# eriklindernoren/PyTorch-GAN

Measured on NVIDIA H100. Metric: DCGAN 64x64 images/sec (full G+D step), higher is better.
Workload: dtype tf32 (fp32 storage, fp32 accumulate)

## Files before the change

### include/b200gan.h

```cpp
#ifndef B200GAN_H
#define B200GAN_H

#include <stddef.h>
#include <stdint.h>

#ifdef __cplusplus
extern "C" {
#endif

#define B200GAN_VERSION 100

enum {
  B200GAN_OK = 0,
  B200GAN_E_UNSUPPORTED = -1,
  B200GAN_E_BAD_ARG = -2,
  B200GAN_E_CUDA = -3,
  B200GAN_E_ARCH = -4
};

enum { B200GAN_ACT_NONE = 0, B200GAN_ACT_LRELU = 1, B200GAN_ACT_RELU = 2, B200GAN_ACT_TANH = 3,
       B200GAN_ACT_SIGMOID = 4 };

enum { B200GAN_ALGO_AUTO = 0,
       B200GAN_ALGO_SIMT = 1,
       B200GAN_ALGO_TC = 2 };

enum { B200GAN_PAD_ZERO = 0, B200GAN_PAD_REFLECT = 1 };

enum {
  B200GAN_PACK_SIMT_FPROP = 0,
  B200GAN_PACK_SIMT_DGRAD = 1,
  B200GAN_PACK_TC_FPROP = 2,
  B200GAN_PACK_TC_DGRAD = 3,
  B200GAN_PACK_TC_FPROP_UP2 = 4,
  B200GAN_PACK_TC_DGRAD_UP2 = 5
};

typedef struct b200gan_conv_geom {
  int32_t N, H, W, C;
  int32_t K;
  int32_t R, S;
  int32_t stride;
  int32_t pad_t, pad_l, pad_b, pad_r;
  int32_t pad_mode;
  int32_t up;
  int32_t transposed;
  int32_t P, Q;
} b200gan_conv_geom;

typedef struct b200gan_epilogue {
  const float *bias;
  int32_t act;
  float slope;
  const float *chan_scale;
  double *stats;
  int32_t stats_per_sample;
  int32_t round_tf32;
} b200gan_epilogue;

int b200gan_version(void);
const char *b200gan_last_error(void);
int b200gan_check_device(void);

size_t b200gan_packed_weight_floats(const b200gan_conv_geom *g, int pack);
int b200gan_pack_weights(const b200gan_conv_geom *g, int pack, const float *w, float *packed,
                         void *stream);

typedef struct b200gan_pack_job {
  const float *w;
  float *packed;
  b200gan_conv_geom geom;
  int32_t pack;
} b200gan_pack_job;
int b200gan_pack_weights_multi(const b200gan_pack_job *jobs, int32_t count, void *stream);

int b200gan_conv2d_supported(const b200gan_conv_geom *g, int pass, int algo);

int b200gan_conv2d_fprop(const b200gan_conv_geom *g, const b200gan_epilogue *ep, const float *x,
                         const float *packed, float *y, int algo, void *stream);

size_t b200gan_conv2d_dgrad_workspace_floats(const b200gan_conv_geom *g, int algo);
int b200gan_conv2d_dgrad(const b200gan_conv_geom *g, const float *dy, const float *packed,
                         float *dx, float *workspace, int algo, void *stream);

size_t b200gan_conv2d_wgrad_workspace_floats(const b200gan_conv_geom *g, int algo);
int b200gan_conv2d_wgrad(const b200gan_conv_geom *g, const float *x, const float *dy, float *dw,
                         float *db, float *workspace, int algo, void *stream);

int b200gan_epilogue_bwd(const float *dy, const float *y, const float *chan_scale, int32_t act,
                         float slope, int64_t n, int32_t K, int64_t PQ, int32_t round_tf32,
                         float *dz, void *stream);

int b200gan_bias_grad(const float *dy, const float *y, const float *chan_scale, int32_t act, float slope,
                      int64_t rows, int32_t K, int64_t PQ, float *db, void *stream);

typedef struct b200gan_norm_desc {
  int32_t N, HW, C;
  int32_t per_sample;
  float eps;
  float momentum;
  int32_t act;
  float slope;
  int32_t round_tf32;
} b200gan_norm_desc;

int b200gan_norm_stats(const b200gan_norm_desc *d, const float *x, double *stats, void *stream);
int b200gan_norm_finalize(const b200gan_norm_desc *d, double *stats, const float *gamma,
                          const float *beta, float *mean_rstd, float *scale_shift,
                          float *running_mean, float *running_var, int64_t *num_batches_tracked,
                          void *stream);
int b200gan_norm_apply(const b200gan_norm_desc *d, const float *x, const float *scale_shift,
                       float *y, void *stream);
int b200gan_norm_bwd(const b200gan_norm_desc *d, const float *dy, const float *x, const float *y,
                     const float *mean_rstd, const float *scale_shift, const float *gamma, double *sums, float *dx,
                     float *dgamma_dbeta, void *stream);

typedef struct b200gan_tail_desc {
  int32_t N, H, W, C;
  int32_t K;
  int32_t act_mid;
  float slope;
  int32_t act_out;
} b200gan_tail_desc;
int b200gan_tail_supported(const b200gan_tail_desc *d);
int b200gan_tail_fprop(const b200gan_tail_desc *d, const float *a, const float *scale_shift, const float *w,
                       const float *bias, float *out, void *stream);
size_t b200gan_tail_bwd_workspace_bytes(const b200gan_tail_desc *d);
int b200gan_tail_bwd(const b200gan_tail_desc *d, const float *a, const float *mean_rstd, const float *scale_shift,
                     const float *w, const float *g, void *workspace, float *da, float *dgamma_dbeta, float *dw,
                     float *db, int32_t round_tf32, void *stream);

int b200gan_nchw_to_nhwc(const float *x, float *y, int32_t N, int32_t C, int32_t HW, void *stream);
int b200gan_nhwc_to_nchw(const float *x, float *y, int32_t N, int32_t C, int32_t HW, void *stream);
int b200gan_upsample2x_fwd(const float *x, float *y, int32_t N, int32_t H, int32_t W, int32_t C,
                           void *stream);
int b200gan_upsample2x_bwd(const float *dy, float *dx, int32_t N, int32_t H, int32_t W, int32_t C,
                           void *stream);
int b200gan_pad2d_fwd(const float *x, float *y, int32_t N, int32_t H, int32_t W, int32_t C,
                      int32_t pad_t, int32_t pad_l, int32_t pad_b, int32_t pad_r, int32_t mode,
                      int32_t round_tf32, void *stream);
int b200gan_pad2d_bwd(const float *dy, float *dx, int32_t N, int32_t H, int32_t W, int32_t C,
                      int32_t pad_t, int32_t pad_l, int32_t pad_b, int32_t pad_r, int32_t mode,
                      void *stream);
int b200gan_act_fwd(const float *x, const float *mask, int32_t mask_per_channel, int32_t act,
                    float slope, int64_t n, int32_t C, int64_t HW, float *y, void *stream);

typedef struct b200gan_mlp_critic_desc {
  int32_t N, Din, H1, H2;
  float slope;
} b200gan_mlp_critic_desc;
int b200gan_mlp_critic_fwd(const b200gan_mlp_critic_desc *d, const float *x, const float *W1,
                           const float *b1, const float *W2, const float *b2, const float *W3,
                           const float *b3, float *out, float *m1, float *a1, float *m2, float *a2,
                           void *stream);
size_t b200gan_mlp_critic_bwd_workspace_floats(const b200gan_mlp_critic_desc *d);
int b200gan_mlp_critic_bwd(const b200gan_mlp_critic_desc *d, const float *dout, const float *x,
                           const float *W1, const float *W2, const float *W3, const float *m1,
                           const float *a1, const float *m2, const float *a2, float *dx, float *dW1,
                           float *db1, float *dW2, float *db2, float *dW3, float *db3, float *U1,
                           float *U2, float *workspace, void *stream);
size_t b200gan_mlp_critic_dbwd_workspace_floats(const b200gan_mlp_critic_desc *d);
int b200gan_mlp_critic_dbwd(const b200gan_mlp_critic_desc *d, const float *u, const float *dout,
                            const float *U1, const float *U2, const float *m1, const float *m2,
                            const float *W1, const float *W2, const float *W3, float *dW1, float *dW2,
                            float *dW3, float *ddout, float *workspace, void *stream);
size_t b200gan_critic_step_workspace_floats(const b200gan_mlp_critic_desc *d);
int b200gan_critic_step_mlp(const b200gan_mlp_critic_desc *d, float lambda_gp, const float *real, const float *fake,
                            const float *alpha, const float *W1, const float *b1, const float *W2, const float *b2,
                            const float *W3, const float *b3, float *losses, float *dW1, float *db1, float *dW2,
                            float *db2, float *dW3, float *db3, float *workspace, void *stream);

#define B200GAN_MLP_GEN_MAX_LAYERS 8
#define B200GAN_MLP_GEN_MAX_WIDTH 8192
#define B200GAN_MLP_GEN_MAX_N 8192
typedef struct b200gan_mlp_gen_desc {
  int32_t L, N;
  int32_t width[B200GAN_MLP_GEN_MAX_LAYERS + 1];
  int32_t has_norm[B200GAN_MLP_GEN_MAX_LAYERS];
  float slope, eps, momentum;
  const float *W[B200GAN_MLP_GEN_MAX_LAYERS], *b[B200GAN_MLP_GEN_MAX_LAYERS];
  const float *gamma[B200GAN_MLP_GEN_MAX_LAYERS], *beta[B200GAN_MLP_GEN_MAX_LAYERS];
  float *running_mean[B200GAN_MLP_GEN_MAX_LAYERS], *running_var[B200GAN_MLP_GEN_MAX_LAYERS];
  int64_t *num_batches_tracked[B200GAN_MLP_GEN_MAX_LAYERS];
} b200gan_mlp_gen_desc;
typedef struct b200gan_mlp_gen_grads {
  float *dW[B200GAN_MLP_GEN_MAX_LAYERS], *db[B200GAN_MLP_GEN_MAX_LAYERS];
  float *dgamma[B200GAN_MLP_GEN_MAX_LAYERS], *dbeta[B200GAN_MLP_GEN_MAX_LAYERS];
} b200gan_mlp_gen_grads;
size_t b200gan_mlp_gen_saved_floats(const b200gan_mlp_gen_desc *d);
size_t b200gan_mlp_gen_workspace_floats(const b200gan_mlp_gen_desc *d);
int b200gan_mlp_gen_fwd(const b200gan_mlp_gen_desc *d, const float *z, float *out, float *saved, float *workspace,
                        void *stream);
int b200gan_mlp_gen_bwd(const b200gan_mlp_gen_desc *d, const float *dout, const float *z, const float *out,
                        const float *saved, float *dz, const b200gan_mlp_gen_grads *grads, float *workspace,
                        void *stream);

typedef struct b200gan_nb_bn {
  const double *stats;
// ... 49 lines not shown
```

### pytorch-gan_b200/b200gan/_lib.py

```python
import ctypes
import os

_HERE = os.path.dirname(os.path.abspath(__file__))
LIB_PATH = os.path.join(_HERE, "libb200gan.so")

c_i32, c_i64, c_f32, c_f64 = ctypes.c_int32, ctypes.c_int64, ctypes.c_float, ctypes.c_double
c_vp, c_sz = ctypes.c_void_p, ctypes.c_size_t

ACT_NONE, ACT_LRELU, ACT_RELU, ACT_TANH, ACT_SIGMOID = 0, 1, 2, 3, 4
ALGO_AUTO, ALGO_SIMT, ALGO_TC = 0, 1, 2
PAD_ZERO, PAD_REFLECT = 0, 1
PACK_SIMT_FPROP, PACK_SIMT_DGRAD, PACK_TC_FPROP, PACK_TC_DGRAD, PACK_TC_FPROP_UP2, PACK_TC_DGRAD_UP2 = range(6)


class ConvGeom(ctypes.Structure):
    _fields_ = [(n, c_i32) for n in (
        "N", "H", "W", "C", "K", "R", "S", "stride", "pad_t", "pad_l", "pad_b", "pad_r",
        "pad_mode", "up", "transposed", "P", "Q")]

    def key(self):
        return tuple(getattr(self, n) for n, _ in self._fields_)


class Epilogue(ctypes.Structure):
    _fields_ = [("bias", c_vp), ("act", c_i32), ("slope", c_f32), ("chan_scale", c_vp),
                ("stats", c_vp), ("stats_per_sample", c_i32), ("round_tf32", c_i32)]


class NormDesc(ctypes.Structure):
    _fields_ = [("N", c_i32), ("HW", c_i32), ("C", c_i32), ("per_sample", c_i32), ("eps", c_f32),
                ("momentum", c_f32), ("act", c_i32), ("slope", c_f32), ("round_tf32", c_i32)]


class MlpCriticDesc(ctypes.Structure):
    _fields_ = [("N", c_i32), ("Din", c_i32), ("H1", c_i32), ("H2", c_i32), ("slope", c_f32)]


MLP_GEN_MAX_LAYERS, MLP_GEN_MAX_WIDTH, MLP_GEN_MAX_N = 8, 8192, 8192


class MlpGenDesc(ctypes.Structure):
    _fields_ = [("L", c_i32), ("N", c_i32), ("width", c_i32 * (MLP_GEN_MAX_LAYERS + 1)),
                ("has_norm", c_i32 * MLP_GEN_MAX_LAYERS), ("slope", c_f32), ("eps", c_f32), ("momentum", c_f32)] + [
        (n, c_vp * MLP_GEN_MAX_LAYERS)
        for n in ("W", "b", "gamma", "beta", "running_mean", "running_var", "num_batches_tracked")]


class MlpGenGrads(ctypes.Structure):
    _fields_ = [(n, c_vp * MLP_GEN_MAX_LAYERS) for n in ("dW", "db", "dgamma", "dbeta")]


class PackJob(ctypes.Structure):
    _fields_ = [("w", c_vp), ("packed", c_vp), ("geom", ConvGeom), ("pack", c_i32)]


class NbBn(ctypes.Structure):
    _fields_ = [("stats", c_vp), ("gamma", c_vp), ("beta", c_vp), ("eps", c_f32), ("count", c_f64), ("groups", c_i32),
                ("reserved", c_i32)]


class TailDesc(ctypes.Structure):
    _fields_ = [("N", c_i32), ("H", c_i32), ("W", c_i32), ("C", c_i32), ("K", c_i32), ("act_mid", c_i32),
                ("slope", c_f32), ("act_out", c_i32)]


class AdamTensor(ctypes.Structure):
    _fields_ = [("p", c_vp), ("g", c_vp), ("m", c_vp), ("v", c_vp), ("n", c_i64)]


_P = ctypes.POINTER
SIGNATURES = {
    "b200gan_version": (c_i32, []),
    "b200gan_last_error": (ctypes.c_char_p, []),
    "b200gan_check_device": (c_i32, []),
    "b200gan_packed_weight_floats": (c_sz, [_P(ConvGeom), c_i32]),
    "b200gan_pack_weights": (c_i32, [_P(ConvGeom), c_i32, c_vp, c_vp, c_vp]),
    "b200gan_pack_weights_multi": (c_i32, [_P(PackJob), c_i32, c_vp]),
    "b200gan_conv2d_supported": (c_i32, [_P(ConvGeom), c_i32, c_i32]),
    "b200gan_conv2d_fprop": (c_i32, [_P(ConvGeom), _P(Epilogue), c_vp, c_vp, c_vp, c_i32, c_vp]),
    "b200gan_conv2d_dgrad_workspace_floats": (c_sz, [_P(ConvGeom), c_i32]),
    "b200gan_conv2d_dgrad": (c_i32, [_P(ConvGeom), c_vp, c_vp, c_vp, c_vp, c_i32, c_vp]),
    "b200gan_conv2d_wgrad_workspace_floats": (c_sz, [_P(ConvGeom), c_i32]),
    "b200gan_conv2d_wgrad": (c_i32, [_P(ConvGeom), c_vp, c_vp, c_vp, c_vp, c_vp, c_i32, c_vp]),
    "b200gan_epilogue_bwd": (c_i32, [c_vp, c_vp, c_vp, c_i32, c_f32, c_i64, c_i32, c_i64, c_i32, c_vp, c_vp]),
    "b200gan_bias_grad": (c_i32, [c_vp, c_vp, c_vp, c_i32, c_f32, c_i64, c_i32, c_i64, c_vp, c_vp]),
    "b200gan_norm_stats": (c_i32, [_P(NormDesc), c_vp, c_vp, c_vp]),
    "b200gan_norm_finalize": (c_i32, [_P(NormDesc), c_vp, c_vp, c_vp, c_vp, c_vp, c_vp, c_vp, c_vp, c_vp]),
    "b200gan_norm_apply": (c_i32, [_P(NormDesc), c_vp, c_vp, c_vp, c_vp]),
    "b200gan_norm_bwd": (c_i32, [_P(NormDesc), c_vp, c_vp, c_vp, c_vp, c_vp, c_vp, c_vp, c_vp, c_vp, c_vp]),
    "b200gan_tail_supported": (c_i32, [_P(TailDesc)]),
    "b200gan_tail_fprop": (c_i32, [_P(TailDesc), c_vp, c_vp, c_vp, c_vp, c_vp, c_vp]),
    "b200gan_tail_bwd_workspace_bytes": (c_sz, [_P(TailDesc)]),
    "b200gan_tail_bwd": (c_i32, [_P(TailDesc)] + [c_vp] * 10 + [c_i32, c_vp]),
    "b200gan_nchw_to_nhwc": (c_i32, [c_vp, c_vp, c_i32, c_i32, c_i32, c_vp]),
    "b200gan_nhwc_to_nchw": (c_i32, [c_vp, c_vp, c_i32, c_i32, c_i32, c_vp]),
    "b200gan_upsample2x_fwd": (c_i32, [c_vp, c_vp, c_i32, c_i32, c_i32, c_i32, c_vp]),
    "b200gan_upsample2x_bwd": (c_i32, [c_vp, c_vp, c_i32, c_i32, c_i32, c_i32, c_vp]),
    "b200gan_pad2d_fwd": (c_i32, [c_vp, c_vp] + [c_i32] * 10 + [c_vp]),
    "b200gan_pad2d_bwd": (c_i32, [c_vp, c_vp] + [c_i32] * 9 + [c_vp]),
    "b200gan_act_fwd": (c_i32, [c_vp, c_vp, c_i32, c_i32, c_f32, c_i64, c_i32, c_i64, c_vp, c_vp]),
    "b200gan_mlp_critic_fwd": (c_i32, [_P(MlpCriticDesc)] + [c_vp] * 13),
    "b200gan_mlp_critic_bwd_workspace_floats": (c_sz, [_P(MlpCriticDesc)]),
    "b200gan_mlp_critic_bwd": (c_i32, [_P(MlpCriticDesc)] + [c_vp] * 20),
    "b200gan_mlp_critic_dbwd_workspace_floats": (c_sz, [_P(MlpCriticDesc)]),
    "b200gan_mlp_critic_dbwd": (c_i32, [_P(MlpCriticDesc)] + [c_vp] * 15),
    "b200gan_critic_step_workspace_floats": (c_sz, [_P(MlpCriticDesc)]),
    "b200gan_critic_step_mlp": (c_i32, [_P(MlpCriticDesc), c_f32] + [c_vp] * 18),
    "b200gan_mlp_gen_saved_floats": (c_sz, [_P(MlpGenDesc)]),
    "b200gan_mlp_gen_workspace_floats": (c_sz, [_P(MlpGenDesc)]),
    "b200gan_mlp_gen_fwd": (c_i32, [_P(MlpGenDesc)] + [c_vp] * 5),
    "b200gan_mlp_gen_bwd": (c_i32, [_P(MlpGenDesc)] + [c_vp] * 5 + [_P(MlpGenGrads), c_vp, c_vp]),
    "b200gan_nb_supported": (c_i32, [_P(ConvGeom)]),
    "b200gan_nb_groups_supported": (c_i32, [_P(ConvGeom), c_i32]),
    "b200gan_nb_fprop": (c_i32, [_P(ConvGeom), _P(NbBn), c_vp, c_vp, c_vp, c_f32, c_vp, c_vp, c_vp, c_i32, c_f32, c_vp,
                                 c_vp, c_vp, c_i32, c_vp]),
    "b200gan_nb_dz": (c_i32, [c_i32, c_i64, c_i32, c_vp, c_vp, c_vp, c_i32, c_f32, _P(NbBn), c_vp, c_vp, c_vp, c_vp]),
    "b200gan_nb_wgrad_workspace_floats": (c_sz, [_P(ConvGeom)]),
    "b200gan_nb_wgrad": (c_i32, [_P(ConvGeom), _P(NbBn), c_vp, c_vp, c_vp, c_vp, c_vp]),
    "b200gan_nb_dgrad": (c_i32, [_P(ConvGeom), c_vp, c_vp, _P(NbBn), c_vp, c_vp, c_vp, c_vp]),
    "b200gan_nb_tail_fwd": (c_i32, [c_i32, c_i32, c_i32, _P(NbBn), c_vp, c_vp, c_vp, c_f32, c_vp, c_vp, c_i32, c_vp]),
    "b200gan_nb_tail_bwd": (c_i32, [c_i32, c_i32, c_i32, _P(NbBn), c_vp, c_vp, c_i32, c_vp, c_vp, c_vp]),
    "b200gan_linear1_fwd": (c_i32, [c_vp, c_vp, c_vp, c_vp, c_i32, c_i32, c_i32, c_vp]),
    "b200gan_linear1_bwd": (c_i32, [c_vp] * 7 + [c_i32, c_i32, c_i32, c_vp]),
    "b200gan_bce_fwd": (c_i32, [c_vp, c_vp, c_vp, c_i64, c_vp]),
    "b200gan_bce_bwd": (c_i32, [c_vp, c_vp, c_vp, c_vp, c_i64, c_vp]),
    "b200gan_adam_multi": (c_i32, [_P(AdamTensor), c_i32, c_f64, c_f64, c_f64, c_f64, c_f32, c_vp, c_vp]),
}

_lib = None


def load():
    global _lib
    if _lib is not None:
        return _lib
    if not os.path.exists(LIB_PATH):
        raise RuntimeError(
            f"{LIB_PATH} is missing: run `python pytorch-gan_b200/build.py` (or __graft_entry__.build()). "
            "b200gan has no CPU / cuDNN fallback.")
    lib = ctypes.CDLL(LIB_PATH)
    for name, (res, args) in SIGNATURES.items():
        fn = getattr(lib, name)
        fn.restype = res
        fn.argtypes = args
    _lib = lib
    return lib


CALLS = 0


def check(rc, what=""):
    global CALLS
    CALLS += 1
    if rc != 0:
        msg = load().b200gan_last_error().decode("utf-8", "replace")
        raise RuntimeError(f"libb200gan {what} failed (code {rc}): {msg}")
```

### pytorch-gan_b200/b200gan/functional.py

```python
import weakref
from dataclasses import dataclass
from typing import Optional, Tuple

import torch

from . import ops
from ._lib import ConvGeom
from ._lib import (ACT_LRELU, ACT_NONE, ACT_RELU, ACT_SIGMOID, ACT_TANH, ALGO_SIMT,
                   PACK_SIMT_DGRAD, PACK_SIMT_FPROP, PAD_ZERO)


@dataclass(frozen=True)
class ConvSpec:
    stride: int = 1
    pads: Tuple[int, int, int, int] = (0, 0, 0, 0)
    pad_mode: int = PAD_ZERO
    up: int = 1
    transposed: bool = False
    act: int = ACT_NONE
    slope: float = 0.0
    stats: Optional[bool] = None
    rtf_out: bool = False
    rtf_dz: bool = False

# ... 142 lines not shown
    @staticmethod
    @torch.autograd.function.once_differentiable
    def backward(ctx, u):
        dz, weight = ctx.saved_tensors
        g, u = ctx.g, _as_cl(u)
        ddz = _plain_fprop(g, u, weight.detach()) if ctx.needs_input_grad[0] else None
        dw = _plain_wgrad(g, u, _as_cl(dz.detach()), tuple(weight.shape)) if ctx.needs_input_grad[1] else None
        return ddz, dw, None


class ConvWgradFn(torch.autograd.Function):
    @staticmethod
    def forward(ctx, x, dz, g, wshape):
        ctx.g = g
        ctx.save_for_backward(x, dz)
        return _plain_wgrad(g, _as_cl(x.detach()), _as_cl(dz.detach()), wshape)

    @staticmethod
    @torch.autograd.function.once_differentiable
    def backward(ctx, v):
        x, dz = ctx.saved_tensors
        g, v = ctx.g, v.contiguous()
        dx = _plain_dgrad(g, _as_cl(dz.detach()), v) if ctx.needs_input_grad[0] else None
        ddz = _plain_fprop(g, _as_cl(x.detach()), v) if ctx.needs_input_grad[1] else None
        return dx, ddz, None, None


def _conv_backward_differentiable(ctx, dy):
    x, weight, y, chan_scale = ctx.saved_tensors
    act, slope, g = ctx.spec.act, ctx.spec.slope, ctx.g
    if chan_scale is not None and act in (ACT_TANH, ACT_SIGMOID):
        raise NotImplementedError("b200gan: double backward through Dropout2d fused with tanh / sigmoid")
    dz = dy
    if act == ACT_LRELU:
        dz = dz * torch.where(y > 0, 1.0, slope)
    elif act == ACT_RELU:
        dz = dz * (y > 0).to(dy.dtype)
    elif act == ACT_TANH:
        dz = dz * (1 - y * y)
    elif act == ACT_SIGMOID:
        dz = dz * (y * (1 - y))
    if chan_scale is not None:
        dz = dz * chan_scale.view(chan_scale.shape[0], chan_scale.shape[1], 1, 1)
    dx = ConvDgradFn.apply(dz, weight, g) if ctx.needs_input_grad[0] else None
    dw = ConvWgradFn.apply(x, dz, g, tuple(weight.shape)) if ctx.needs_input_grad[1] else None
    db = dz.sum((0, 2, 3)) if (ctx.has_bias and ctx.needs_input_grad[2]) else None
    return dx, dw, db



class NormFn(torch.autograd.Function):

    @staticmethod
    def forward(ctx, x, gamma, beta, stats, running_mean, running_var, nbt, spec: NormSpec):
        ops._require_cuda(x, "norm input")
        x = _as_cl(x)
        y, mean_rstd, scale_shift = ops.norm_forward(
            x, None if gamma is None else gamma.detach(), None if beta is None else beta.detach(), running_mean,
            running_var, nbt, spec.per_sample, spec.eps, spec.momentum, spec.act, spec.slope, stats, spec.rtf_out,
            return_scale_shift=True)
        ctx.spec = spec
        mask_from_x = spec.act in (ACT_LRELU, ACT_RELU)
        need_y = spec.act != ACT_NONE and not mask_from_x
        ctx.save_for_backward(x, y if need_y else None, mean_rstd, gamma, scale_shift if mask_from_x else None)
        return y

    @staticmethod
    @torch.autograd.function.once_differentiable
    def backward(ctx, dy):
        x, y, mean_rstd, gamma, scale_shift = ctx.saved_tensors
        spec = ctx.spec
        dy = _as_cl(dy)
        need_params = gamma is not None and (ctx.needs_input_grad[1] or ctx.needs_input_grad[2])
        dx, dgb = ops.norm_backward(dy, x, y, mean_rstd, None if gamma is None else gamma.detach(), spec.per_sample,
                                    spec.eps, spec.act, spec.slope, need_params, spec.rtf_dx, scale_shift)
        dgamma = dbeta = None
        if need_params:
            n, c = x.shape[0], x.shape[1]
            groups = dgb.numel() // 2
            dgamma, dbeta = dgb[:groups], dgb[groups:]
            if spec.per_sample:
                dgamma, dbeta = dgamma.view(n, c).sum(0), dbeta.view(n, c).sum(0)
        return dx, dgamma, dbeta, None, None, None, None, None


@dataclass(frozen=True)
class TailSpec:
    eps: float = 1e-5
    momentum: float = 0.0
    act_mid: int = ACT_NONE
    slope: float = 0.0
    act_out: int = ACT_NONE
    rtf_dx: bool = False


class TailFn(torch.autograd.Function):

    @staticmethod
    def forward(ctx, a, stats, gamma, beta, running_mean, running_var, nbt, weight, bias, spec: TailSpec):
        ops._require_cuda(a, "tail input")
        a = _as_cl(a)
        if stats is None:
            stats = ops.norm_stats(a, False)
        mean_rstd, scale_shift = ops.norm_finalize(
            tuple(a.shape), stats, None if gamma is None else gamma.detach(), None if beta is None else beta.detach(),
            running_mean, running_var, nbt, False, spec.eps, spec.momentum, a.device)
        d = ops.tail_desc(tuple(a.shape), weight.shape[0], spec.act_mid, spec.slope, spec.act_out)
        w = weight.detach().contiguous()
        out = ops.tail_fprop(d, a, scale_shift, w, None if bias is None else bias.detach())
        ctx.spec, ctx.d = spec, d
        ctx.has_affine, ctx.has_bias = gamma is not None, bias is not None
        ctx.save_for_backward(a, mean_rstd, scale_shift, weight, out if spec.act_out != ACT_NONE else None)
        return out

    @staticmethod
    @torch.autograd.function.once_differentiable
    def backward(ctx, dout):
        a, mean_rstd, scale_shift, weight, out = ctx.saved_tensors
        spec = ctx.spec
        dout = _as_cl(dout)
        g = ops.epilogue_bwd(dout, out, None, spec.act_out, 0.0) if spec.act_out != ACT_NONE else dout
        need_affine = ctx.has_affine and (ctx.needs_input_grad[2] or ctx.needs_input_grad[3])
        need_bias = ctx.has_bias and ctx.needs_input_grad[8]
        da, dgb, dw, db = ops.tail_bwd(ctx.d, a, mean_rstd, scale_shift, weight.detach().contiguous(), g, need_affine,
                                       need_bias, spec.rtf_dx)
        c = a.shape[1]
        dgamma = dgb[:c] if need_affine else None
        dbeta = dgb[c:] if need_affine else None
        return da, None, dgamma, dbeta, None, None, None, dw, db, None


class AffineActFn(torch.autograd.Function):

    @staticmethod
    def forward(ctx, x, scale_shift, act, slope):
        x = _as_cl(x)
        y = ops.norm_apply_affine(x, scale_shift, False, act, slope)
        ctx.act, ctx.slope = act, slope
        ctx.save_for_backward(y, scale_shift)
        return y

    @staticmethod
    @torch.autograd.function.once_differentiable
    def backward(ctx, dy):
        y, scale_shift = ctx.saved_tensors
        dy = _as_cl(dy)
        dz = ops.epilogue_bwd(dy, y, None, ctx.act, ctx.slope) if ctx.act != ACT_NONE else dy
        c = y.shape[1]
        zero = torch.zeros_like(scale_shift)
        zero[:c] = scale_shift[:c]
        return ops.norm_apply_affine(dz, zero, False), None, None, None


class ToChannelsLastFn(torch.autograd.Function):

    @staticmethod
    def forward(ctx, x):
        return ops.to_cl(x)

    @staticmethod
    def backward(ctx, dy):
        if torch.is_grad_enabled() and dy.requires_grad:
            return ToContiguousFn.apply(dy)
        return ops.to_nchw(dy.detach())


# ... 377 lines not shown
```

### pytorch-gan_b200/b200gan/nn.py

```python
import torch
import torch.nn as tnn

from . import _lib
from . import functional as F
from . import ops
from ._lib import (ACT_LRELU, ACT_NONE, ACT_RELU, ACT_SIGMOID, ACT_TANH, PAD_REFLECT, PAD_ZERO)
from .functional import ConvSpec, NormSpec, PackCache

_T = {
    n: getattr(tnn, n) for n in (
        "Conv2d", "ConvTranspose2d", "BatchNorm2d", "InstanceNorm2d", "LeakyReLU", "ReLU", "Tanh", "Sigmoid",
        "Upsample", "ZeroPad2d", "ReflectionPad2d", "Dropout", "Dropout2d", "Sequential", "Linear", "BCELoss",
        "BatchNorm1d")
}


def _pair_same(v, what):
    if isinstance(v, (tuple, list)):
        if len(v) != 2 or v[0] != v[1]:
            raise NotImplementedError(f"b200gan: {what}={v} (h != w) is not supported")
        return int(v[0])
    return int(v)


def _act_of(m):
    if isinstance(m, _T["LeakyReLU"]):
        if m.negative_slope < 0:
            raise NotImplementedError(f"b200gan: {m} (negative_slope < 0)")
        return ACT_LRELU, float(m.negative_slope)
    if isinstance(m, _T["ReLU"]):
        return ACT_RELU, 0.0
    if isinstance(m, _T["Tanh"]):
        return ACT_TANH, 0.0
    if isinstance(m, _T["Sigmoid"]):
        return ACT_SIGMOID, 0.0
    return None


def _is_up2(m):
    if not isinstance(m, _T["Upsample"]):
        return False
    sf = m.scale_factor
    if isinstance(sf, (tuple, list)):
        sf = sf[0] if len(set(sf)) == 1 else None
    return m.size is None and sf is not None and float(sf) == 2.0 and m.mode == "nearest"


def _pads_of(m):
    p = m.padding
    if isinstance(p, int):
        p = (p, p, p, p)
    l, r, t, b = p
    return (int(t), int(l), int(b), int(r))


def _conv_ok(m):
    if isinstance(m.padding, str) or m.padding_mode != "zeros":
        return False
    if tuple(m.dilation) != (1, 1) or m.groups != 1:
        return False
    if len(set(m.stride)) != 1 or len(set(m.padding)) != 1:
        return False
    if isinstance(m, _T["ConvTranspose2d"]) and tuple(m.output_padding) != (0, 0):
        return False
    return True


def _tc_like(conv, up, full=False):
    if ops.Config.algo == "simt":
        return False
    if up == 2:
        return (not isinstance(conv, _T["ConvTranspose2d"]) and conv.stride[0] == 1 and conv.in_channels % 32 == 0
                and conv.out_channels % 64 == 0)
    if conv.stride[0] in (1, 2) and conv.in_channels % 32 == 0 and conv.out_channels % 32 == 0:
        return True
    return (full is False and not isinstance(conv, _T["ConvTranspose2d"]) and conv.stride[0] == 1
            and conv.in_channels % 32 == 0 and conv.out_channels < 32)


def _no_groups(what):
    if ops.bn_groups.active > 1:
        raise RuntimeError(f"b200gan: ops.bn_groups({ops.bn_groups.active}) is active but {what} would treat the batch "
                           "as one pass; run the passes separately")


def _dropout2d_scale(x_shape, p, device):
    n, c = x_shape[0], x_shape[1]
    noise = torch.empty((n, c, 1, 1), device=device, dtype=torch.float32)
    if p >= 1.0:
        return noise.zero_().view(n, c)
    return noise.bernoulli_(1.0 - p).div_(1.0 - p).view(n, c)


def _run_conv(conv, x, up=1, extra_pads=(0, 0, 0, 0), pad_mode=PAD_ZERO, act=ACT_NONE, slope=0.0, chan_scale=None,
              stats=None, rtf_out=False, rtf_dz=False):
    if not _conv_ok(conv):
        raise NotImplementedError(f"b200gan: unsupported convolution configuration: {conv}")
    transposed = isinstance(conv, _T["ConvTranspose2d"])
    pad = int(conv.padding[0])
    if pad_mode == PAD_REFLECT and pad != 0:
        raise NotImplementedError("b200gan: reflection padding in front of a zero-padded conv")
    if pad_mode == PAD_REFLECT and up == 1 and _tc_like(conv, 1):
        x = F.PadFn.apply(x, tuple(extra_pads), PAD_REFLECT, True)
        extra_pads, pad_mode = (0, 0, 0, 0), PAD_ZERO
    pads = tuple(e + pad for e in extra_pads)
    spec = ConvSpec(stride=int(conv.stride[0]), pads=pads, pad_mode=pad_mode, up=up, transposed=transposed, act=act,
                    slope=slope, stats=stats, rtf_out=rtf_out, rtf_dz=rtf_dz)
    cache = conv.__dict__.get("_b200_cache")
    if cache is None:
        cache = PackCache()
        conv.__dict__["_b200_cache"] = cache
    return F.conv_block(x, conv.weight, conv.bias, chan_scale, spec, cache)


def _run_norm(norm, x, act=ACT_NONE, slope=0.0, stats=None, rtf_out=False, rtf_dx=False):
    per_sample = isinstance(norm, _T["InstanceNorm2d"])
    if per_sample and norm.track_running_stats:
        raise NotImplementedError("b200gan: InstanceNorm2d(track_running_stats=True)")
    if x.dim() != 4:
        raise ValueError(f"expected 4D input (got {x.dim()}D input)")
    if per_sample and x.shape[2] * x.shape[3] == 1 and norm.training:
        raise ValueError(f"Expected more than 1 spatial element when training, got input size {tuple(x.shape)}")
    use_batch_stats = per_sample or norm.training or norm.running_mean is None
    if use_batch_stats and not per_sample:
        _no_groups("a stand-alone BatchNorm2d")
    if use_batch_stats:
        rm = rv = nbt = None
        momentum = 0.0
        if not per_sample and norm.training and norm.track_running_stats:
            if norm.momentum is None:
                raise NotImplementedError("b200gan: BatchNorm2d(momentum=None)")
            rm, rv, nbt, momentum = norm.running_mean, norm.running_var, norm.num_batches_tracked, float(norm.momentum)
        spec = NormSpec(per_sample=per_sample, eps=float(norm.eps), momentum=momentum, act=act, slope=slope,
                        rtf_out=rtf_out, rtf_dx=rtf_dx)
        return F.norm_block(x, norm.weight, norm.bias, stats, rm, rv, nbt, spec)
    rstd = torch.rsqrt(norm.running_var + norm.eps)
    scale = rstd if norm.weight is None else norm.weight * rstd
    shift = -norm.running_mean * scale if norm.bias is None else norm.bias - norm.running_mean * scale
    return F.AffineActFn.apply(x, torch.cat([scale, shift]).detach(), act, slope)


def _on_device(x):
    return x.is_cuda


def _gpu4d(x):
    return x.dim() == 4 and _on_device(x)


class Conv2d(_T["Conv2d"]):
    def forward(self, x):
        return _run_conv(self, x)


class ConvTranspose2d(_T["ConvTranspose2d"]):
    def forward(self, x, output_size=None):
        if output_size is not None:
            raise NotImplementedError("b200gan: ConvTranspose2d(output_size=...)")
        return _run_conv(self, x)


class BatchNorm2d(_T["BatchNorm2d"]):
    def forward(self, x):
        return _run_norm(self, x)


class InstanceNorm2d(_T["InstanceNorm2d"]):
    def forward(self, x):
        return _run_norm(self, x)


class _Act:
    def forward(self, x):
        if not _gpu4d(x):
            return super().forward(x)
        act, slope = _act_of(self)
        return F.ActFn.apply(x, act, slope, None, False)


class LeakyReLU(_Act, _T["LeakyReLU"]):
    pass


class ReLU(_Act, _T["ReLU"]):
    pass


class Tanh(_Act, _T["Tanh"]):
    pass


class Sigmoid(_Act, _T["Sigmoid"]):
    pass


class Upsample(_T["Upsample"]):
    def forward(self, x):
        if _gpu4d(x) and _is_up2(self):
            return F.UpsampleFn.apply(x)
        if _gpu4d(x):
            raise NotImplementedError(f"b200gan: {self} (only nearest x2 is on the hot path)")
        return super().forward(x)


class ZeroPad2d(_T["ZeroPad2d"]):
    def forward(self, x):
        if not _gpu4d(x):
            return super().forward(x)
        return F.PadFn.apply(x, _pads_of(self), PAD_ZERO)


class ReflectionPad2d(_T["ReflectionPad2d"]):
    def forward(self, x):
        if not _gpu4d(x):
            return super().forward(x)
        return F.PadFn.apply(x, _pads_of(self), PAD_REFLECT)


class Dropout2d(_T["Dropout2d"]):
    def forward(self, x):
        if not _gpu4d(x):
            return super().forward(x)
        if not self.training or self.p == 0.0:
            return x
        _no_groups("a stand-alone Dropout2d")
        return F.ActFn.apply(x, ACT_NONE, 0.0, _dropout2d_scale(x.shape, self.p, x.device), True)


class Dropout(_T["Dropout"]):
    def forward(self, x):
        if not _gpu4d(x):
            return super().forward(x)
        if not self.training or self.p == 0.0:
            return x
        _no_groups("a stand-alone Dropout")
        xc = x if ops.is_cl(x) else ops.to_cl(x)
        mask = torch.empty_like(xc, memory_format=torch.channels_last)
        if self.p >= 1.0:
            mask.zero_()
        else:
            mask.bernoulli_(1.0 - self.p).div_(1.0 - self.p)
        return F.ActFn.apply(xc, ACT_NONE, 0.0, mask, False)


def _gpu2d_f32(x):
    return torch.is_tensor(x) and x.dim() == 2 and x.is_cuda and x.dtype == torch.float32


class Linear(_T["Linear"]):

    def forward(self, x):
        if _gpu2d_f32(x) and self.out_features >= 8192 and ops.Config.algo != "simt":
            return F.LinearWideFn.apply(x, self.weight, self.bias)
        return super().forward(x)


class BatchNorm1d(_T["BatchNorm1d"]):
    """nn.BatchNorm1d, same state_dict.  Inside the MLP generator pattern of a Sequential (mlp_generator_layers,
    wgan_gp.py:42-65, gan.py:38-61) it runs in the fused generator kernels; anywhere else, and on the CPU, it is the stock
    module."""


class BCELoss(_T["BCELoss"]):
    def forward(self, input, target):
        if (input.is_cuda and input.dtype == torch.float32 and self.reduction == "mean" and self.weight is None
                and target.shape == input.shape and target.dtype == torch.float32 and not target.requires_grad):
            return F.BCEMeanFn.apply(input, target)
        return super().forward(input, target)


class _ConvStep:
    def __init__(self, conv, up, extra_pads, pad_mode, act, slope, dropout2d, stats):
        self.conv, self.up, self.extra_pads, self.pad_mode = conv, up, extra_pads, pad_mode
        self.act, self.slope, self.dropout2d, self.stats = act, slope, dropout2d, stats
        self.rtf_out = False
        self.rtf_dz = False
        self.next_norm = None

    def tc_like(self, full=False):
        if self.pad_mode == PAD_REFLECT and self.up != 1:
            return False
        return _tc_like(self.conv, self.up, full)


class _NormStep:
    def __init__(self, norm, act, slope, takes_stats):
        self.norm, self.act, self.slope, self.takes_stats = norm, act, slope, takes_stats
        self.rtf_out = False
        self.rtf_dx = False


class _LeafStep:
    def __init__(self, mod):
        self.mod = mod


class _TailStep:

    def __init__(self, norm_step, conv_step):
        self.norm_step, self.conv_step = norm_step, conv_step


def _chain_plan(chain, shape):
    plan = []
    for cs, ns in chain.layers:
        conv = cs.conv
        if shape[1] != conv.in_channels or not _conv_ok(conv):
            return None
        g, oshape = ops.make_geom(shape, tuple(conv.weight.shape), int(conv.stride[0]), (int(conv.padding[0]),) * 4)
        macs = float(oshape[0]) * oshape[2] * oshape[3] * conv.out_channels * conv.in_channels * g.R * g.S
        if macs > _ChainStep.MAX_MACS or not ops.nb_supported(g) or oshape[2] * oshape[3] < 1:
            return None
        if ns is not None:
            norm = ns.norm
            if not (norm.training and norm.num_features == conv.out_channels):
                return None
            if norm.track_running_stats and norm.momentum is None:
                return None
        plan.append((cs, ns, oshape))
        shape = oshape
    return plan


def groups_eligible(seq, x_shape, groups):
    if not isinstance(seq, Sequential) or not ops.Config.fuse_narrow_chain or x_shape[0] % groups != 0:
        return False
    steps = seq._plan()
    if not steps or not all(isinstance(st, _ChainStep) for st in steps):
        return False
    shape = tuple(x_shape)
    with ops.bn_groups(groups):
        for st in steps:
            plan = _chain_plan(st, shape)
            if plan is None:
                return False
            shape = plan[-1][2]
    return True


class _ChainStep:

    MAX_MACS = 6.0e8

    def __init__(self, steps):
        self.steps = steps
        self.layers = []
        i = 0
        while i < len(steps):
            ns = steps[i + 1] if i + 1 < len(steps) and isinstance(steps[i + 1], _NormStep) else None
            self.layers.append((steps[i], ns))
            i += 2 if ns is not None else 1


def _chain_conv_candidate(cs):
    if not isinstance(cs, _ConvStep):
        return False
    conv = cs.conv
    if isinstance(conv, _T["ConvTranspose2d"]) or cs.up != 1 or cs.extra_pads != (0, 0, 0, 0) or cs.pad_mode != PAD_ZERO:
        return False
    if cs.act not in (ACT_NONE, ACT_LRELU, ACT_RELU):
        return False
    k, c = conv.out_channels, conv.in_channels
    if not (4 <= k <= 128 and (k & (k - 1)) == 0 and 1 <= c <= 128 and (c == 1 or c % 4 == 0)):
        return False
    return tuple(conv.kernel_size) in ((3, 3), (4, 4)) and conv.stride[0] in (1, 2)


def _chain_norm_candidate(ns):
    return isinstance(ns, _NormStep) and isinstance(ns.norm, _T["BatchNorm2d"]) and ns.act == ACT_NONE


def _fuse_chains(steps):
    out, i, n = [], 0, len(steps)
    while i < n:
        j, convs = i, 0
        while j < n and _chain_conv_candidate(steps[j]):
            convs += 1
            j += 1
            if j < n and steps[j - 1].stats is False and _chain_norm_candidate(steps[j]):
                j += 1
            elif steps[j - 1].stats is not None:
                j -= 1
                convs -= 1
# ... 208 lines not shown
                norm = ns.norm
                edge = ops.BnEdge(stats, None if norm.weight is None else norm.weight.detach(),
                                  None if norm.bias is None else norm.bias.detach(), norm.eps,
                                  oshape[0] // groups * oshape[2] * oshape[3], groups)
                out_box.append(edge)
                prev_norm = norm
            else:
                x, edge, prev_norm = res, None, None
        if edge is not None:
            norm = prev_norm
            rm = rv = nbt = None
            momentum = 0.0
            if norm.track_running_stats and norm.running_mean is not None:
                rm, rv, nbt, momentum = norm.running_mean, norm.running_var, norm.num_batches_tracked, float(norm.momentum)
            x = F.NbTailFn.apply(x, norm.weight, norm.bias, rm, rv, nbt, edge, momentum, bool(nchw_out))
        return x

    def _forward_2d(self, x):
        mods = list(self._modules.values())
        critic = mlp_critic_layers(mods, x.shape[1])
        if critic is not None and x.shape[0] >= 1:
            return F.mlp_critic(x, *critic)
        gen = mlp_generator_layers(mods, x.shape[1])
        if gen is not None and (x.shape[0] >= 2 or all(bn is None for _, bn in gen[0])) \
                and x.shape[0] <= _lib.MLP_GEN_MAX_N:
            return F.mlp_generator(x, *gen)
        i = 0
        while i < len(mods):
            m = mods[i]
            if (isinstance(m, _T["Linear"]) and m.out_features == 1 and _gpu2d_f32(x) and x.shape[0] <= 4096
                    and i + 1 < len(mods) and _act_of(mods[i + 1]) is not None
                    and _act_of(mods[i + 1])[0] in (ACT_SIGMOID, ACT_TANH)):
                x = F.Linear1Fn.apply(x, m.weight, m.bias, _act_of(mods[i + 1])[0])
                i += 2
            else:
                x = m(x)
                i += 1
        return x

    def forward(self, x):
        if _gpu2d_f32(x):
            return self._forward_2d(x)
        if not (torch.is_tensor(x) and x.dim() == 4 and _on_device(x) and x.dtype == torch.float32):
            return super().forward(x)
        steps = self._plan()
        if all(isinstance(s, _LeafStep) for s in steps):
            return _T["Sequential"].forward(self, x)
        want_contiguous = x.is_contiguous()
        stats = None
        queue = list(steps)
        while queue:
            s = queue.pop(0)
            if isinstance(s, _ChainStep):
                at_end = not queue
                res = self._run_chain(s, x, want_contiguous and at_end)
                if res is None:
                    _no_groups("a conv chain that does not qualify for the fused kernels")
                    queue[0:0] = s.steps
                else:
                    x, stats = res, None
                    if at_end and want_contiguous and x.is_contiguous():
                        return x
                continue
            if isinstance(s, _TailStep):
                ns, cs = s.norm_step, s.conv_step
                norm, conv = ns.norm, cs.conv
                _no_groups("the fused generator tail")
                if (norm.training and x.shape[1] == conv.in_channels and x.shape[1] == norm.num_features
                        and ops.tail_supported(tuple(x.shape), conv.out_channels, ns.act, ns.slope, cs.act)):
                    rm = rv = nbt = None
                    momentum = 0.0
                    if norm.track_running_stats and norm.running_mean is not None:
                        if norm.momentum is None:
                            raise NotImplementedError("b200gan: BatchNorm2d(momentum=None)")
                        rm, rv, nbt, momentum = norm.running_mean, norm.running_var, norm.num_batches_tracked, float(norm.momentum)
                    spec = F.TailSpec(eps=float(norm.eps), momentum=momentum, act_mid=ns.act, slope=ns.slope,
                                      act_out=cs.act, rtf_dx=ns.rtf_dx)
                    x = F.TailFn.apply(x, stats if ns.takes_stats else None, norm.weight, norm.bias, rm, rv, nbt,
                                       conv.weight, conv.bias, spec)
                    stats = None
                else:
                    queue[0:0] = [ns, cs]
                continue
            if isinstance(s, _ConvStep):
                cs = None
                if s.dropout2d is not None and s.dropout2d.training and s.dropout2d.p > 0.0:
                    _no_groups("a Dropout2d outside a fused chain")
                    n = x.shape[0]
                    cs = _dropout2d_scale((n, s.conv.out_channels), s.dropout2d.p, x.device)
                want = s.stats if (s.next_norm is not None and _uses_batch_stats(s.next_norm)) else None
                out = _run_conv(s.conv, x, s.up, s.extra_pads, s.pad_mode, s.act, s.slope, cs, want, s.rtf_out,
                                s.rtf_dz)
                if want is not None:
                    x, stats = out
                else:
                    x, stats = out, None
            elif isinstance(s, _NormStep):
                x = _run_norm(s.norm, x, s.act, s.slope, stats if s.takes_stats else None, s.rtf_out, s.rtf_dx)
                stats = None
            else:
                x = s.mod(x)
                stats = None
        if (want_contiguous and torch.is_tensor(x) and x.dim() == 4 and not x.is_contiguous()
                and x.shape[2] * x.shape[3] <= ops.Config.contiguous_hw_limit):
            x = F.ToContiguousFn.apply(x)
        return x


REPLACEMENTS = {
    "Conv2d": Conv2d, "ConvTranspose2d": ConvTranspose2d, "BatchNorm2d": BatchNorm2d,
    "InstanceNorm2d": InstanceNorm2d, "LeakyReLU": LeakyReLU, "ReLU": ReLU, "Tanh": Tanh, "Sigmoid": Sigmoid,
    "Upsample": Upsample, "ZeroPad2d": ZeroPad2d, "ReflectionPad2d": ReflectionPad2d, "Dropout": Dropout,
    "Dropout2d": Dropout2d, "Sequential": Sequential, "Linear": Linear, "BCELoss": BCELoss, "BatchNorm1d": BatchNorm1d,
}
for _n, _c in REPLACEMENTS.items():
    _c.__name__ = _n
    _c.__qualname__ = _n
```

### pytorch-gan_b200/b200gan/ops.py

```python
import ctypes
import os

import torch

from . import _lib
from ._lib import (ACT_NONE, ALGO_AUTO, ALGO_SIMT, ALGO_TC, PACK_SIMT_DGRAD, PACK_SIMT_FPROP, PACK_TC_DGRAD,
                   PACK_TC_DGRAD_UP2, PACK_TC_FPROP, PACK_TC_FPROP_UP2, PAD_REFLECT, PAD_ZERO, ConvGeom, Epilogue,
                   MlpCriticDesc, MlpGenDesc, MlpGenGrads, NbBn, NormDesc, TailDesc)

CL = torch.channels_last


class Config:
    algo = os.environ.get("B200GAN_ALGO", "auto")
    weight_cache = True
    contiguous_hw_limit = 64
    fuse_narrow_chain = os.environ.get("B200GAN_FUSE_CHAIN", "1") not in ("", "0")


def _stream():
    return torch.cuda.current_stream().cuda_stream


def _ptr(t):
# ... 53 lines not shown
    g = ConvGeom()
    g.N, g.H, g.W, g.C = n, h, w, c
    if transposed:
        cin, cout, r, s = weight_shape
    else:
        cout, cin, r, s = weight_shape
    if cin != c:
        raise RuntimeError(f"b200gan conv: input has {c} channels, weight expects {cin}")
    g.K, g.R, g.S, g.stride = cout, r, s, stride
    g.pad_t, g.pad_l, g.pad_b, g.pad_r = pads
    g.pad_mode, g.up, g.transposed = pad_mode, up, int(transposed)
    if transposed:
        g.P = (h - 1) * stride - 2 * pads[0] + r
        g.Q = (w - 1) * stride - 2 * pads[1] + s
    else:
        g.P = (h * up + pads[0] + pads[2] - r) // stride + 1
        g.Q = (w * up + pads[1] + pads[3] - s) // stride + 1
    return g, (n, cout, g.P, g.Q)


def tc_supported(g, pas):
    if Config.algo == "simt":
        return False
    return bool(_lib.load().b200gan_conv2d_supported(ctypes.byref(g), pas, ALGO_TC))


def conv_plan(g, pas, chan_scale=None):
    if pas == 2:
        return (ALGO_SIMT if Config.algo == "simt" else ALGO_AUTO), None
    tc = tc_supported(g, pas) and not (pas == 0 and g.K < 32 and chan_scale is not None)
    if not tc:
        return ALGO_SIMT, (PACK_SIMT_FPROP if pas == 0 else PACK_SIMT_DGRAD)
    if pas == 0:
        return ALGO_TC, (PACK_TC_FPROP_UP2 if g.up == 2 else PACK_TC_FPROP)
    return ALGO_TC, (PACK_TC_DGRAD_UP2 if g.up == 2 else PACK_TC_DGRAD)


def pack_weights(g, w, kind, out=None):
    lib = _lib.load()
    if out is None:
        n = lib.b200gan_packed_weight_floats(ctypes.byref(g), kind)
        out = torch.empty(n, device=w.device, dtype=torch.float32)
    _lib.check(lib.b200gan_pack_weights(ctypes.byref(g), kind, w.data_ptr(), out.data_ptr(), _stream()), "pack_weights")
    return out


def pack_weights_multi(jobs):
    table = (_lib.PackJob * len(jobs))()
    for i, (g, kind, w, packed) in enumerate(jobs):
        table[i].w, table[i].packed, table[i].geom, table[i].pack = w.data_ptr(), packed.data_ptr(), g, kind
    _lib.check(_lib.load().b200gan_pack_weights_multi(table, len(jobs), _stream()), "pack_weights_multi")


def conv_fprop(g, x, packed, algo, bias=None, act=ACT_NONE, slope=0.0, chan_scale=None, stats=None,
               stats_per_sample=False, round_tf32=False):
    y = empty_cl(g.N, g.K, g.P, g.Q, x.device)
    if g.N == 0:
        return y
    ep = Epilogue()
    ep.bias, ep.act, ep.slope = _ptr(bias), act, slope
    ep.chan_scale, ep.stats = _ptr(chan_scale), _ptr(stats)
    ep.stats_per_sample, ep.round_tf32 = int(stats_per_sample), int(round_tf32)
    _lib.check(_lib.load().b200gan_conv2d_fprop(ctypes.byref(g), ctypes.byref(ep), x.data_ptr(), packed.data_ptr(),
                                                y.data_ptr(), algo, _stream()), "conv2d_fprop")
    return y


def conv_dgrad(g, dy, packed, algo):
    lib = _lib.load()
    dx = empty_cl(g.N, g.C, g.H, g.W, dy.device)
    nws = lib.b200gan_conv2d_dgrad_workspace_floats(ctypes.byref(g), algo)
    ws = torch.empty(nws, device=dy.device, dtype=torch.float32) if nws else None
    _lib.check(lib.b200gan_conv2d_dgrad(ctypes.byref(g), dy.data_ptr(), packed.data_ptr(), dx.data_ptr(), _ptr(ws),
                                        algo, _stream()), "conv2d_dgrad")
    return dx


def conv_wgrad(g, x, dy, weight_shape, need_bias, algo):
    lib = _lib.load()
    dw = torch.empty(weight_shape, device=x.device, dtype=torch.float32)
    db = torch.empty(g.K, device=x.device, dtype=torch.float32) if need_bias else None
    nws = lib.b200gan_conv2d_wgrad_workspace_floats(ctypes.byref(g), algo)
    ws = torch.empty(nws, device=x.device, dtype=torch.float32) if nws else None
    _lib.check(lib.b200gan_conv2d_wgrad(ctypes.byref(g), x.data_ptr(), dy.data_ptr(), dw.data_ptr(), _ptr(db),
                                        _ptr(ws), algo, _stream()), "conv2d_wgrad")
    return dw, db


def epilogue_bwd(dy, y, chan_scale, act, slope, round_tf32=False):
    n, k, p, q = dy.shape
    dz = torch.empty_like(dy, memory_format=CL)
    _lib.check(_lib.load().b200gan_epilogue_bwd(dy.data_ptr(), _ptr(y), _ptr(chan_scale), act, slope, dy.numel(), k,
                                                p * q, int(round_tf32), dz.data_ptr(), _stream()), "epilogue_bwd")
    return dz


def bias_grad(dy, y, chan_scale, act, slope):
    n, k, p, q = dy.shape
    db = torch.empty(k, device=dy.device, dtype=torch.float32)
    _lib.check(_lib.load().b200gan_bias_grad(dy.data_ptr(), _ptr(y), _ptr(chan_scale), act, slope, n * p * q, k, p * q,
                                             db.data_ptr(), _stream()), "bias_grad")
    return db


def _norm_desc(shape, per_sample, eps, momentum, act, slope, round_tf32):
    n, c, h, w = shape
    d = NormDesc()
    d.N, d.HW, d.C, d.per_sample = n, h * w, c, int(per_sample)
    d.eps, d.momentum, d.act, d.slope, d.round_tf32 = eps, momentum, act, slope, int(round_tf32)
    return d


_zero_scratch = {}


def zero_scratch(device, numel):
    key = (device, numel)
    t = _zero_scratch.get(key)
    if t is None:
        t = torch.zeros(numel, device=device, dtype=torch.float64)
        _zero_scratch[key] = t
    return t


def reset_scratch():
    for t in _zero_scratch.values():
        t.zero_()


def new_stats(x, per_sample):
    n, c = x.shape[0], x.shape[1]
    return zero_scratch(x.device, 2 * (n * c if per_sample else c))


def norm_forward(x, gamma, beta, running_mean, running_var, nbt, per_sample, eps, momentum, act=ACT_NONE, slope=0.0,
                 stats=None, round_tf32=False, return_scale_shift=False):
    if stats is None:
        stats = norm_stats(x, per_sample)
    mean_rstd, scale_shift = norm_finalize(x.shape, stats, gamma, beta, running_mean, running_var, nbt, per_sample, eps,
                                           momentum, x.device)
    d = _norm_desc(x.shape, per_sample, eps, momentum, act, slope, round_tf32)
    y = torch.empty_like(x, memory_format=CL)
    _lib.check(_lib.load().b200gan_norm_apply(ctypes.byref(d), x.data_ptr(), scale_shift.data_ptr(), y.data_ptr(),
                                              _stream()), "norm_apply")
    if return_scale_shift:
        return y, mean_rstd, scale_shift
    return y, mean_rstd


def norm_finalize(x_shape, stats, gamma, beta, running_mean, running_var, nbt, per_sample, eps, momentum, device):
    d = _norm_desc(x_shape, per_sample, eps, momentum, ACT_NONE, 0.0, False)
    groups = stats.numel() // 2
    mean_rstd = torch.empty(2 * groups, device=device, dtype=torch.float32)
    scale_shift = torch.empty(2 * groups, device=device, dtype=torch.float32)
    _lib.check(_lib.load().b200gan_norm_finalize(ctypes.byref(d), stats.data_ptr(), _ptr(gamma), _ptr(beta),
                                                 mean_rstd.data_ptr(), scale_shift.data_ptr(), _ptr(running_mean),
                                                 _ptr(running_var), _ptr(nbt), _stream()), "norm_finalize")
    return mean_rstd, scale_shift


def norm_stats(x, per_sample):
    d = _norm_desc(x.shape, per_sample, 0.0, 0.0, ACT_NONE, 0.0, False)
    stats = new_stats(x, per_sample)
    _lib.check(_lib.load().b200gan_norm_stats(ctypes.byref(d), x.data_ptr(), stats.data_ptr(), _stream()), "norm_stats")
    return stats


def tail_desc(a_shape, k, act_mid, slope, act_out):
    n, c, h, w = a_shape
    d = TailDesc()
    d.N, d.H, d.W, d.C, d.K = n, h, w, c, k
    d.act_mid, d.slope, d.act_out = act_mid, slope, act_out
    return d


def tail_supported(a_shape, k, act_mid, slope, act_out):
    if Config.algo == "simt":
        return False
    return bool(_lib.load().b200gan_tail_supported(ctypes.byref(tail_desc(a_shape, k, act_mid, slope, act_out))))


def tail_fprop(d, a, scale_shift, w, bias):
    out = empty_cl(d.N, d.K, d.H, d.W, a.device)
    _lib.check(_lib.load().b200gan_tail_fprop(ctypes.byref(d), a.data_ptr(), scale_shift.data_ptr(), w.data_ptr(),
                                              _ptr(bias), out.data_ptr(), _stream()), "tail_fprop")
    return out


def tail_bwd(d, a, mean_rstd, scale_shift, w, g, need_affine, need_bias, round_tf32):
    lib = _lib.load()
    nws = lib.b200gan_tail_bwd_workspace_bytes(ctypes.byref(d))
    ws = torch.empty((nws + 7) // 8, device=a.device, dtype=torch.float64)
    da = torch.empty_like(a, memory_format=CL)
    dgb = torch.empty(2 * d.C, device=a.device, dtype=torch.float32) if need_affine else None
    dw = torch.empty((d.K, d.C, 3, 3), device=a.device, dtype=torch.float32)
    db = torch.empty(d.K, device=a.device, dtype=torch.float32) if need_bias else None
    _lib.check(lib.b200gan_tail_bwd(ctypes.byref(d), a.data_ptr(), mean_rstd.data_ptr(), scale_shift.data_ptr(),
                                    w.data_ptr(), g.data_ptr(), ws.data_ptr(), da.data_ptr(), _ptr(dgb), dw.data_ptr(),
                                    _ptr(db), int(round_tf32), _stream()), "tail_bwd")
    return da, dgb, dw, db


def norm_apply_affine(x, scale_shift, per_sample, act=ACT_NONE, slope=0.0):
    d = _norm_desc(x.shape, per_sample, 0.0, 0.0, act, slope, False)
    y = torch.empty_like(x, memory_format=CL)
    _lib.check(_lib.load().b200gan_norm_apply(ctypes.byref(d), x.data_ptr(), scale_shift.data_ptr(), y.data_ptr(),
                                              _stream()), "norm_apply")
    return y


def norm_backward(dy, x, y, mean_rstd, gamma, per_sample, eps, act=ACT_NONE, slope=0.0, need_params=False,
                  round_tf32=False, scale_shift=None):
    lib = _lib.load()
    d = _norm_desc(x.shape, per_sample, eps, 0.0, act, slope, round_tf32)
    groups = mean_rstd.numel() // 2
    sums = zero_scratch(x.device, 2 * groups)
    dx = torch.empty_like(x, memory_format=CL)
    dgb = torch.empty(2 * groups, device=x.device, dtype=torch.float32) if need_params else None
    _lib.check(lib.b200gan_norm_bwd(ctypes.byref(d), dy.data_ptr(), x.data_ptr(), _ptr(y), mean_rstd.data_ptr(),
                                    _ptr(scale_shift), _ptr(gamma), sums.data_ptr(), dx.data_ptr(), _ptr(dgb), _stream()),
               "norm_bwd")
    return dx, dgb


def upsample2x(x):
    n, c, h, w = x.shape
    y = empty_cl(n, c, 2 * h, 2 * w, x.device)
    _lib.check(_lib.load().b200gan_upsample2x_fwd(x.data_ptr(), y.data_ptr(), n, h, w, c, _stream()), "upsample2x_fwd")
    return y


def upsample2x_bwd(dy):
    n, c, h2, w2 = dy.shape
    dx = empty_cl(n, c, h2 // 2, w2 // 2, dy.device)
    _lib.check(_lib.load().b200gan_upsample2x_bwd(dy.data_ptr(), dx.data_ptr(), n, h2 // 2, w2 // 2, c, _stream()),
               "upsample2x_bwd")
    return dx


def pad2d(x, pads, mode, round_tf32=False):
    n, c, h, w = x.shape
    t, l, b, r = pads
    y = empty_cl(n, c, h + t + b, w + l + r, x.device)
    _lib.check(_lib.load().b200gan_pad2d_fwd(x.data_ptr(), y.data_ptr(), n, h, w, c, t, l, b, r, mode, int(round_tf32),
                                             _stream()), "pad2d_fwd")
    return y


def pad2d_bwd(dy, pads, mode):
    n, c, ho, wo = dy.shape
    t, l, b, r = pads
    h, w = ho - t - b, wo - l - r
    dx = empty_cl(n, c, h, w, dy.device)
    _lib.check(_lib.load().b200gan_pad2d_bwd(dy.data_ptr(), dx.data_ptr(), n, h, w, c, t, l, b, r, mode, _stream()),
               "pad2d_bwd")
    return dx


def act_forward(x, act, slope, mask=None, mask_per_channel=False):
    n, c, h, w = x.shape
    y = torch.empty_like(x, memory_format=CL)
    _lib.check(_lib.load().b200gan_act_fwd(x.data_ptr(), _ptr(mask), int(mask_per_channel), act, slope, x.numel(), c,
                                           h * w, y.data_ptr(), _stream()), "act_fwd")
    return y


class BnEdge:

    def __init__(self, stats, gamma, beta, eps, count, groups=1):
        self.stats, self.gamma, self.beta, self.eps, self.count = stats, gamma, beta, float(eps), float(count)
        self.groups = int(groups)
        self.sums = None

    def c_struct(self):
        b = NbBn()
        b.stats, b.gamma, b.beta = self.stats.data_ptr(), _ptr(self.gamma), _ptr(self.beta)
        b.eps, b.count, b.groups, b.reserved = self.eps, self.count, self.groups, 0
        return b


class bn_groups:

    active = 1

    def __init__(self, groups):
        self.groups = int(groups)

    def __enter__(self):
        self.prev = bn_groups.active
        bn_groups.active = self.groups
        return self

    def __exit__(self, *exc):
        bn_groups.active = self.prev


def nb_supported(g):
    if not Config.fuse_narrow_chain:
        return False
    lib = _lib.load()
    if bn_groups.active > 1:
        return bool(lib.b200gan_nb_groups_supported(ctypes.byref(g), bn_groups.active))
    return bool(lib.b200gan_nb_supported(ctypes.byref(g)))

# ... 243 lines not shown
```

### pytorch-gan_b200/csrc/conv_api.cu

```cuda
#include "common.cuh"
#include <atomic>
#include <mutex>
#include <string.h>
#include <stdlib.h>

namespace b200gan {

int simt_gather_gemm(int N, int H, int W, int C, int P, int Q, int K, int R, int S, int stride,
                     int pad_t, int pad_l, int pad_mode, int up, int mode,
                     const b200gan_epilogue *ep, const float *x, const float *wp, float *y,
                     cudaStream_t st);
int simt_wgrad(int N, int H, int W, int Cg, int P, int Q, int Cd, int R, int S, int stride,
               int pad_t, int pad_l, int pad_mode, int up, const float *xg, const float *dn,
               float *dw, cudaStream_t st);
int simt_colsum(const float *x, float *out, int64_t M, int C, cudaStream_t st);
bool nb_wgrad_ok(const b200gan_conv_geom *g);
int nb_wgrad_run(const b200gan_conv_geom *g, const b200gan_nb_bn *in_bn, const float *x, const float *dz, float *dw,
                 float *workspace, cudaStream_t st);
size_t nb_wgrad_workspace_floats(const b200gan_conv_geom *g);
bool nb_plain_fprop_ok(const b200gan_conv_geom *g);
int nb_plain_fprop(const b200gan_conv_geom *g, const b200gan_epilogue *ep, const float *x, const float *packed, float *y,
                   cudaStream_t st);
bool nb_plain_dgrad_ok(const b200gan_conv_geom *g);
int nb_plain_dgrad(const b200gan_conv_geom *g, const float *dy, const float *packed, float *dx, cudaStream_t st);
bool fewk_ok(const b200gan_conv_geom *g, int pas);
int fewk_fprop(const b200gan_conv_geom *g, const b200gan_epilogue *ep, const float *x, const float *packed, float *y,
               cudaStream_t st);
int fewk_dgrad(const b200gan_conv_geom *g, const float *dy, const float *packed, float *dx, cudaStream_t st);
int fewk_wgrad(const b200gan_conv_geom *g, const float *x, const float *dy, float *dw, float *workspace, cudaStream_t st);
size_t fewk_wgrad_workspace_floats(const b200gan_conv_geom *g);
int tc_supported(const b200gan_conv_geom *g, int pass);
int tc_fprop(const b200gan_conv_geom *g, const b200gan_epilogue *ep, const float *x,
             const float *packed, float *y, cudaStream_t st);
int tc_dgrad(const b200gan_conv_geom *g, const float *dy, const float *packed, float *dx,
             cudaStream_t st);
size_t tc_wgrad_workspace_floats(const b200gan_conv_geom *g);
int tc_wgrad(const b200gan_conv_geom *g, const float *x, const float *dy, float *dw, float *ws,
             cudaStream_t st);

static thread_local char g_err[512] = "";
void set_error(const char *fmt, ...) {
  va_list ap;
  va_start(ap, fmt);
  vsnprintf(g_err, sizeof(g_err), fmt, ap);
  va_end(ap);
}

int conv_stats_pass(const float *y, int N, int HW, int C, int per_sample, double *stats, cudaStream_t st) {
  b200gan_norm_desc nd;
  memset(&nd, 0, sizeof(nd));
  nd.N = N; nd.HW = HW; nd.C = C; nd.per_sample = per_sample;
  return b200gan_norm_stats(&nd, y, stats, st);
}

int num_sms() {
  static std::atomic<int> cache[64];
  int dev = 0;
  if (cudaGetDevice(&dev) != cudaSuccess || dev < 0 || dev >= 64) {
    cudaGetLastError();
    return 132;
  }
  int v = cache[dev].load(std::memory_order_relaxed);
  if (v > 0) return v;
  if (cudaDeviceGetAttribute(&v, cudaDevAttrMultiProcessorCount, dev) != cudaSuccess || v <= 0) {
    cudaGetLastError();
    return 132;
  }
  cache[dev].store(v, std::memory_order_relaxed);
  return v;
}

int validate_geom(const b200gan_conv_geom *g) {
  B2_CHECK_ARG(g != nullptr, "conv: null geometry");
  B2_CHECK_ARG(g->N >= 0 && g->H > 0 && g->W > 0 && g->C > 0 && g->K > 0 && g->R > 0 && g->S > 0,
               "conv: bad dims N=%d H=%d W=%d C=%d K=%d R=%d S=%d", g->N, g->H, g->W, g->C, g->K,
               g->R, g->S);
  B2_CHECK_ARG(g->stride >= 1, "conv: stride must be >= 1");
  B2_CHECK_ARG(g->up == 1 || g->up == 2, "conv: up must be 1 or 2");
  B2_CHECK_ARG(g->pad_t >= 0 && g->pad_l >= 0 && g->pad_b >= 0 && g->pad_r >= 0, "conv: negative padding");
  int P, Q;
  if (g->transposed) {
    B2_CHECK_ARG(g->up == 1 && g->pad_mode == B200GAN_PAD_ZERO,
                 "conv: ConvTranspose2d cannot fold upsample / reflection padding");
    B2_CHECK_ARG(g->pad_t == g->pad_b && g->pad_l == g->pad_r, "conv: ConvTranspose2d padding must be symmetric");
    P = (g->H - 1) * g->stride - 2 * g->pad_t + g->R;
    Q = (g->W - 1) * g->stride - 2 * g->pad_l + g->S;
  } else {
    int Hv = g->H * g->up, Wv = g->W * g->up;
    if (g->pad_mode == B200GAN_PAD_REFLECT)
      B2_CHECK_ARG(g->pad_t < Hv && g->pad_b < Hv && g->pad_l < Wv && g->pad_r < Wv,
                   "conv: reflection padding must be smaller than the input");
    int Hp = Hv + g->pad_t + g->pad_b, Wp = Wv + g->pad_l + g->pad_r;
    B2_CHECK_ARG(Hp >= g->R && Wp >= g->S, "conv: filter larger than padded input");
    P = (Hp - g->R) / g->stride + 1;
    Q = (Wp - g->S) / g->stride + 1;
  }
  B2_CHECK_ARG(P == g->P && Q == g->Q, "conv: output size mismatch: expected %dx%d, got %dx%d", P, Q,
               g->P, g->Q);
  B2_CHECK_ARG((int64_t)g->N * g->H * g->W * g->C < (1LL << 40) && (int64_t)g->N * P * Q * g->K < (1LL << 40),
               "conv: tensor too large");
  return B200GAN_OK;
}

__device__ __forceinline__ void up2_rset(int a, int d, int &lo, int &hi) {
  if (a == 0) { lo = d == 0 ? 0 : 1; hi = d == 0 ? 0 : 2; }
  else        { lo = d == 0 ? 0 : 2; hi = d == 0 ? 1 : 2; }
}

constexpr int PACK_MAX_JOBS = 24;
constexpr int PACK_CHUNK = 256 * 8;
struct PackJob {
  const float *src;
  float *dst;
  int R, S, Cin, Cout, transposed, kind;
  int tiles_ci;
  long long total;
};
constexpr int PACK_CO_T = 32, PACK_CI_T = 8, PACK_RS_MAX = 16;
struct PackTable {
  PackJob job[PACK_MAX_JOBS];
// ... 175 lines not shown
  return base;
}

extern "C" int b200gan_pack_weights(const b200gan_conv_geom *g, int pack, const float *w, float *packed,
                                    void *stream) {
  PackTable tb;
  tb.count = 0;
  tb.block_begin[0] = 0;
  if (int e = pack_table_add(tb, g, pack, w, packed)) return e;
  return pack_table_launch(tb, as_stream(stream));
}

extern "C" int b200gan_conv2d_supported(const b200gan_conv_geom *g, int pass, int algo) {
  if (validate_geom(g) != B200GAN_OK) return 0;
  if (algo == B200GAN_ALGO_SIMT) return 1;
  return tc_supported(g, pass);
}

extern "C" int b200gan_conv2d_fprop(const b200gan_conv_geom *g, const b200gan_epilogue *ep, const float *x,
                                    const float *packed, float *y, int algo, void *stream) {
  if (int e = validate_geom(g)) return e;
  B2_CHECK_ARG(x && packed && y, "conv2d_fprop: null pointer");
  B2_CHECK_ARG(algo != B200GAN_ALGO_AUTO, "conv2d_fprop: the packed layout fixes the algorithm; pass SIMT or TC");
  cudaStream_t st = as_stream(stream);
  if (algo == B200GAN_ALGO_TC) {
    if (!tc_supported(g, 0)) B2_UNSUPPORTED("conv2d_fprop: geometry not supported by the tensor-core path");
    return tc_fprop(g, ep, x, packed, y, st);
  }
  int rc;
  if (fewk_ok(g, 0) && !(ep && (ep->chan_scale || ep->round_tf32))) {
    b200gan_epilogue e2;
    if (ep) { e2 = *ep; e2.stats = nullptr; }
    rc = fewk_fprop(g, ep ? &e2 : nullptr, x, packed, y, st);
  } else if (nb_plain_fprop_ok(g)) {
    rc = nb_plain_fprop(g, ep, x, packed, y, st);
  } else {
    rc = simt_gather_gemm(g->N, g->H, g->W, g->C, g->P, g->Q, g->K, g->R, g->S, g->stride, g->pad_t, g->pad_l,
                          g->pad_mode, g->up, g->transposed ? 1 : 0, ep, x, packed, y, st);
  }
  if (rc) return rc;
  if (ep && ep->stats) return conv_stats_pass(y, g->N, g->P * g->Q, g->K, ep->stats_per_sample, ep->stats, st);
  return B200GAN_OK;
}

enum class DgradRoute { Tc, Transposed, Fewk, Staged, Virtual };

static DgradRoute dgrad_route(const b200gan_conv_geom *g, int algo) {
  if (algo == B200GAN_ALGO_AUTO ? tc_supported(g, 1) : algo == B200GAN_ALGO_TC) return DgradRoute::Tc;
  if (g->transposed) return DgradRoute::Transposed;
  if (fewk_ok(g, 1)) return DgradRoute::Fewk;
  if (nb_plain_dgrad_ok(g)) return DgradRoute::Staged;
  return DgradRoute::Virtual;
}

enum class WgradRoute { Tc, Fewk, Staged, Simt };

static WgradRoute wgrad_route(const b200gan_conv_geom *g, int algo) {
  if (algo == B200GAN_ALGO_AUTO ? tc_supported(g, 2) : algo == B200GAN_ALGO_TC) return WgradRoute::Tc;
  if (fewk_ok(g, 2)) return WgradRoute::Fewk;
  if (nb_wgrad_ok(g) && (int64_t)g->N * g->P * g->Q * g->K * g->C * g->R * g->S <= (int64_t)2e10)
    return WgradRoute::Staged;
  return WgradRoute::Simt;
}

extern "C" size_t b200gan_conv2d_dgrad_workspace_floats(const b200gan_conv_geom *g, int algo) {
  if (!g || dgrad_route(g, algo) != DgradRoute::Virtual) return 0;
  size_t n = 0;
  int Hv = g->H * g->up, Wv = g->W * g->up;
  if (g->pad_mode == B200GAN_PAD_REFLECT)
    n += (size_t)g->N * (Hv + g->pad_t + g->pad_b) * (Wv + g->pad_l + g->pad_r) * g->C;
  if (g->up == 2) n += (size_t)g->N * Hv * Wv * g->C;
  return n;
}

extern "C" int b200gan_conv2d_dgrad(const b200gan_conv_geom *g, const float *dy, const float *packed, float *dx,
                                    float *workspace, int algo, void *stream) {
  if (int e = validate_geom(g)) return e;
  B2_CHECK_ARG(dy && packed && dx, "conv2d_dgrad: null pointer");
  B2_CHECK_ARG(algo != B200GAN_ALGO_AUTO, "conv2d_dgrad: pass SIMT or TC explicitly");
  cudaStream_t st = as_stream(stream);
  switch (dgrad_route(g, algo)) {
    case DgradRoute::Tc:
      if (!tc_supported(g, 1)) B2_UNSUPPORTED("conv2d_dgrad: geometry not supported by the tensor-core path");
      return tc_dgrad(g, dy, packed, dx, st);
    case DgradRoute::Transposed:
      return simt_gather_gemm(g->N, g->P, g->Q, g->K, g->H, g->W, g->C, g->R, g->S, g->stride, g->pad_t, g->pad_l,
                              B200GAN_PAD_ZERO, 1, 0, nullptr, dy, packed, dx, st);
    case DgradRoute::Fewk:
      return fewk_dgrad(g, dy, packed, dx, st);
    case DgradRoute::Staged:
      return nb_plain_dgrad(g, dy, packed, dx, st);
    case DgradRoute::Virtual:
      break;
  }
  int Hv = g->H * g->up, Wv = g->W * g->up;
  bool reflect = g->pad_mode == B200GAN_PAD_REFLECT;
  B2_CHECK_ARG(!(reflect || g->up == 2) || workspace, "conv2d_dgrad: workspace required for reflect / upsample");
  float *ws_pad = nullptr, *ws_up = nullptr;
  if (reflect) {
    ws_pad = workspace;
    workspace += (size_t)g->N * (Hv + g->pad_t + g->pad_b) * (Wv + g->pad_l + g->pad_r) * g->C;
  }
  if (g->up == 2) ws_up = workspace;
  float *dvirt = reflect ? ws_pad : (g->up == 2 ? ws_up : dx);
  int oh = reflect ? Hv + g->pad_t + g->pad_b : Hv;
  int ow = reflect ? Wv + g->pad_l + g->pad_r : Wv;
  int rc;
  b200gan_conv_geom gv = *g;
  gv.H = oh; gv.W = ow; gv.up = 1; gv.pad_mode = B200GAN_PAD_ZERO;
  if (reflect) gv.pad_t = gv.pad_l = gv.pad_b = gv.pad_r = 0;
  if (reflect && g->up == 1 && fewk_ok(&gv, 1)) {
    rc = fewk_dgrad(&gv, dy, packed, dvirt, st);
  } else if (reflect && g->up == 1 && nb_plain_dgrad_ok(&gv)) {
    rc = nb_plain_dgrad(&gv, dy, packed, dvirt, st);
  } else {
    rc = simt_gather_gemm(g->N, g->P, g->Q, g->K, oh, ow, g->C, g->R, g->S, g->stride, reflect ? 0 : g->pad_t,
                          reflect ? 0 : g->pad_l, B200GAN_PAD_ZERO, 1, 1, nullptr, dy, packed, dvirt, st);
  }
  if (rc) return rc;
  if (reflect) {
    float *dst = g->up == 2 ? ws_up : dx;
    rc = b200gan_pad2d_bwd(ws_pad, dst, g->N, Hv, Wv, g->C, g->pad_t, g->pad_l, g->pad_b, g->pad_r,
                           B200GAN_PAD_REFLECT, stream);
    if (rc) return rc;
  }
  if (g->up == 2) return b200gan_upsample2x_bwd(ws_up, dx, g->N, g->H, g->W, g->C, stream);
  return B200GAN_OK;
}

extern "C" size_t b200gan_conv2d_wgrad_workspace_floats(const b200gan_conv_geom *g, int algo) {
  if (!g) return 0;
  switch (wgrad_route(g, algo)) {
    case WgradRoute::Tc: return tc_wgrad_workspace_floats(g);
    case WgradRoute::Fewk: return fewk_wgrad_workspace_floats(g);
    case WgradRoute::Staged: return nb_wgrad_workspace_floats(g);
    case WgradRoute::Simt: break;
  }
  return 0;
}

extern "C" int b200gan_conv2d_wgrad(const b200gan_conv_geom *g, const float *x, const float *dy, float *dw,
                                    float *db, float *workspace, int algo, void *stream) {
  if (int e = validate_geom(g)) return e;
  B2_CHECK_ARG(x && dy && dw, "conv2d_wgrad: null pointer");
  cudaStream_t st = as_stream(stream);
  int rc = B200GAN_OK;
  switch (wgrad_route(g, algo)) {
    case WgradRoute::Tc:
      if (!tc_supported(g, 2)) B2_UNSUPPORTED("conv2d_wgrad: geometry not supported by the tensor-core path");
      rc = tc_wgrad(g, x, dy, dw, workspace, st);
      break;
    case WgradRoute::Fewk:
      rc = fewk_wgrad(g, x, dy, dw, workspace, st);
      break;
    case WgradRoute::Staged:
      rc = nb_wgrad_run(g, nullptr, x, dy, dw, workspace, st);
      break;
    case WgradRoute::Simt:
      if (g->transposed)
        rc = simt_wgrad(g->N, g->P, g->Q, g->K, g->H, g->W, g->C, g->R, g->S, g->stride, g->pad_t, g->pad_l,
                        B200GAN_PAD_ZERO, 1, dy, x, dw, st);
      else
        rc = simt_wgrad(g->N, g->H, g->W, g->C, g->P, g->Q, g->K, g->R, g->S, g->stride, g->pad_t, g->pad_l,
                        g->pad_mode, g->up, x, dy, dw, st);
      break;
  }
  if (rc) return rc;
  if (db) return simt_colsum(dy, db, (int64_t)g->N * g->P * g->Q, g->K, st);
  return B200GAN_OK;
}
```

### pytorch-gan_b200/csrc/conv_tc.cu

```cuda
#include "tc_common.cuh"
#include <mutex>
#include <stdlib.h>

namespace b200gan {

PFN_encodeTiled get_encode_tiled() {
  static PFN_encodeTiled fn = nullptr;
  static std::once_flag once;
  std::call_once(once, [] {
    void *p = nullptr;
    cudaDriverEntryPointQueryResult q;
    if (cudaGetDriverEntryPointByVersion("cuTensorMapEncodeTiled", &p, 12000, cudaEnableDefault, &q) == cudaSuccess &&
        q == cudaDriverEntryPointSuccess)
      fn = reinterpret_cast<PFN_encodeTiled>(p);
  });
  return fn;
}

int make_tmap_f32(CUtensorMap *map, const void *base, int rank, const uint64_t *dims, const uint64_t *strides_bytes,
                  const uint32_t *box) {
  PFN_encodeTiled enc = get_encode_tiled();
  if (!enc) {
    set_error("cuTensorMapEncodeTiled entry point not available");
    return B200GAN_E_CUDA;
  }
  cuuint64_t gd[5], gs[4];
  cuuint32_t bx[5], es[5];
  for (int i = 0; i < rank; ++i) {
    gd[i] = dims[i];
    bx[i] = box[i];
    es[i] = 1;
  }
  for (int i = 0; i < rank - 1; ++i) gs[i] = strides_bytes[i];
  CUresult r = enc(map, CU_TENSOR_MAP_DATA_TYPE_FLOAT32, (cuuint32_t)rank, const_cast<void *>(base), gd, gs, bx, es,
                   CU_TENSOR_MAP_INTERLEAVE_NONE, CU_TENSOR_MAP_SWIZZLE_128B,
                   CU_TENSOR_MAP_L2_PROMOTION_L2_256B,
                   CU_TENSOR_MAP_FLOAT_OOB_FILL_NONE);
  if (r != CUDA_SUCCESS) {
    set_error("cuTensorMapEncodeTiled failed (%d): rank %d dims [%llu %llu %llu %llu %llu] box [%u %u %u %u %u]", (int)r,
              rank, (unsigned long long)gd[0], (unsigned long long)(rank > 1 ? gd[1] : 0),
              (unsigned long long)(rank > 2 ? gd[2] : 0), (unsigned long long)(rank > 3 ? gd[3] : 0),
              (unsigned long long)(rank > 4 ? gd[4] : 0), bx[0], rank > 1 ? bx[1] : 0, rank > 2 ? bx[2] : 0,
              rank > 3 ? bx[3] : 0, rank > 4 ? bx[4] : 0);
    return B200GAN_E_CUDA;
  }
  return B200GAN_OK;
}

constexpr int TC_BM = 128;
constexpr int TC_BK = 32;
constexpr int TC_A_BYTES = TC_BM * TC_BK * 4;
constexpr int TC_MAX_TAPS = 52;
constexpr int TC_THREADS = 384;

struct TcTap {
  int16_t dc;
  int8_t dw, da, dh;
  int8_t bt;
  int8_t pad_[2];
};

struct TcParams {
  int32_t tap_begin[5];
  TcTap taps[TC_MAX_TAPS];
  int32_t kout_total;
  int32_t kchunks;
  int32_t bw_log2, bh_log2;
  int32_t tiles_w, tiles_h;
  int32_t N, Ho, Wo;
  int32_t out_dc[4], out_da[4];
  int32_t ldk;
  const float *bias;
  const float *chan_scale;
  double *stats;
  int32_t stats_groups;
  int32_t stats_per_sample;
  int32_t act;
  float slope;
  int32_t rtf;
  float *y;
  int32_t narrow_k;
  int32_t ksplit;
  long long *trace;
};

#define TC_TRACE(slot)                                                   \
  do {                                                                   \
    if (p.trace) p.trace[((size_t)blockIdx.z * gridDim.x + blockIdx.x) * 64 + (slot)] = clock64(); \
  } while (0)

template <int OFF>
__device__ __forceinline__ void colsum_step(float (&v)[32], int lane) {
  const bool upper = (lane & OFF) != 0;
#pragma unroll
  for (int i = 0; i < OFF; ++i) {
    float send = upper ? v[i] : v[i + OFF];
    float keep = upper ? v[i + OFF] : v[i];
    v[i] = keep + __shfl_xor_sync(0xffffffffu, send, OFF);
  }
}
__device__ __forceinline__ float warp_colsum32(float (&v)[32], int lane) {
  colsum_step<16>(v, lane);
  colsum_step<8>(v, lane);
  colsum_step<4>(v, lane);
  colsum_step<2>(v, lane);
  colsum_step<1>(v, lane);
  return v[0];
}

__device__ __forceinline__ void consumers_sync() { asm volatile("bar.sync 1, 256;" ::: "memory"); }

__device__ __forceinline__ void ld_row32(const uint8_t *chunk, int m, float (&v)[32]) {
  const uint8_t *row = chunk + m * 128;
#pragma unroll
  for (int j = 0; j < 8; ++j) {
    const float4 t = *reinterpret_cast<const float4 *>(row + ((j ^ (m & 7)) << 4));
    v[4 * j] = t.x; v[4 * j + 1] = t.y; v[4 * j + 2] = t.z; v[4 * j + 3] = t.w;
  }
}
__device__ __forceinline__ void st_row32(uint8_t *chunk, int m, const float (&v)[32]) {
  uint8_t *row = chunk + m * 128;
#pragma unroll
  for (int j = 0; j < 8; ++j)
    *reinterpret_cast<float4 *>(row + ((j ^ (m & 7)) << 4)) = make_float4(v[4 * j], v[4 * j + 1], v[4 * j + 2], v[4 * j + 3]);
}

__device__ __forceinline__ void epilogue_chunk(float (&v)[32], const float *bias, int narrow_k, int act, float slope,
                                               const float *cs, int rtf) {
  if (bias && narrow_k) {
#pragma unroll
    for (int j = 0; j < 32; ++j)
      if (j < narrow_k) v[j] += __ldg(bias + j);
  } else if (bias) {
    const float4 *b4 = reinterpret_cast<const float4 *>(bias);
#pragma unroll
    for (int j = 0; j < 8; ++j) {
      float4 b = __ldg(b4 + j);
      v[4 * j] += b.x; v[4 * j + 1] += b.y; v[4 * j + 2] += b.z; v[4 * j + 3] += b.w;
    }
  }
  if (act == B200GAN_ACT_LRELU) {
#pragma unroll
    for (int j = 0; j < 32; ++j) v[j] = v[j] > 0.f ? v[j] : v[j] * slope;
  } else if (act == B200GAN_ACT_RELU) {
#pragma unroll
    for (int j = 0; j < 32; ++j) v[j] = fmaxf(v[j], 0.f);
  } else if (act == B200GAN_ACT_TANH) {
#pragma unroll
    for (int j = 0; j < 32; ++j) v[j] = tanhf(v[j]);
  } else if (act == B200GAN_ACT_SIGMOID) {
#pragma unroll
    for (int j = 0; j < 32; ++j) v[j] = 1.f / (1.f + __expf(-v[j]));
  }
  if (cs) {
    const float4 *s4 = reinterpret_cast<const float4 *>(cs);
#pragma unroll
    for (int j = 0; j < 8; ++j) {
      float4 b = __ldg(s4 + j);
      v[4 * j] *= b.x; v[4 * j + 1] *= b.y; v[4 * j + 2] *= b.z; v[4 * j + 3] *= b.w;
    }
  }
  if (rtf) {
#pragma unroll
    for (int j = 0; j < 32; ++j) v[j] = round_tf32(v[j]);
  }
}

template <int BN, int STAGES>
struct TcSmem {
  static constexpr int STAGE_BYTES = TC_A_BYTES + BN * TC_BK * 4;
  static constexpr int RING = STAGES * STAGE_BYTES;
  static constexpr int STAGING = (BN / 32) * TC_A_BYTES;
  static constexpr int MAIN = RING > STAGING ? RING : STAGING;
  static constexpr int TOTAL = MAIN + 1024 + 256 + 4 * BN * 2 * 4;
};

template <int BN, int STAGES>
__global__ void __launch_bounds__(TC_THREADS, 1)
conv_tc_kernel(const __grid_constant__ CUtensorMap tmA, const __grid_constant__ CUtensorMap tmB,
               const __grid_constant__ CUtensorMap tmY, const __grid_constant__ TcParams p) {
  using L = TcSmem<BN, STAGES>;
  extern __shared__ uint8_t smem_raw[];
  uint8_t *smem = reinterpret_cast<uint8_t *>((reinterpret_cast<uintptr_t>(smem_raw) + 1023) & ~(uintptr_t)1023);
  uint64_t *full = reinterpret_cast<uint64_t *>(smem + L::MAIN);
  uint64_t *empty = full + STAGES;
  float *red = reinterpret_cast<float *>(smem + L::MAIN + 256);

  const int warp = threadIdx.x >> 5, lane = threadIdx.x & 31;
  const int ph = blockIdx.z / p.ksplit, ks = blockIdx.z % p.ksplit;
  const int ntile = blockIdx.y;
  const int BW = 1 << p.bw_log2, BH = 1 << p.bh_log2;
  int t = blockIdx.x;
  const int tw = t % p.tiles_w;
  t /= p.tiles_w;
  const int th = t % p.tiles_h;
  const int tn = t / p.tiles_h;
  const int w0 = tw << p.bw_log2, h0 = th << p.bh_log2;
  const int n0 = tn * (TC_BM >> (p.bw_log2 + p.bh_log2));
  const int tap0 = p.tap_begin[ph];
  const int iters_all = (p.tap_begin[ph + 1] - tap0) * p.kchunks;
  const int it0 = (int)((long long)iters_all * ks / p.ksplit), it1 = (int)((long long)iters_all * (ks + 1) / p.ksplit);
  const int iters = it1 - it0;

  if (threadIdx.x == 0) {
    TC_TRACE(0);
    tma_prefetch_desc(&tmA);
    tma_prefetch_desc(&tmB);
    tma_prefetch_desc(&tmY);
    for (int s = 0; s < STAGES; ++s) {
      mbar_init(&full[s], 1);
      mbar_init(&empty[s], 2);
    }
    fence_barrier_init();
  }
  __syncthreads();

  if (warp == 0) {
    if (lane == 0) {
      int stage = 0;
      uint32_t phase = 0;
      int tap = it0 / p.kchunks, kc = it0 % p.kchunks;
      for (int it = 0; it < iters; ++it) {
        mbar_wait(&empty[stage], phase ^ 1);
        uint8_t *sa = smem + stage * L::STAGE_BYTES;
        uint8_t *sb = sa + TC_A_BYTES;
        const TcTap tp = p.taps[tap0 + tap];
        if (it < 16) TC_TRACE(2 + it);
        mbar_arrive_expect_tx(&full[stage], L::STAGE_BYTES);
        tma_load_5d(sa, &tmA, &full[stage], tp.dc + kc * TC_BK, w0 + tp.dw, tp.da, h0 + tp.dh, n0);
        tma_load_3d(sb, &tmB, &full[stage], kc * TC_BK, ntile * BN, tp.bt);
        if (++kc == p.kchunks) {
          kc = 0;
          ++tap;
        }
        if (++stage == STAGES) {
          stage = 0;
          phase ^= 1;
        }
      }
    }
  } else if (warp >= 4) {
    const int ct = threadIdx.x - 128;
    const int half = ct >> 7;
    {
      float acc[BN / 2];
      int stage = 0, prev = 0;
      uint32_t phase = 0;
      for (int it = 0; it < iters; ++it) {
        mbar_wait(&full[stage], phase);
        if (ct == 0 && it < 16) TC_TRACE(20 + it);
        const uint32_t sa = smem_u32(smem + stage * L::STAGE_BYTES) + half * (TC_A_BYTES / 2);
        const uint32_t sb = smem_u32(smem + stage * L::STAGE_BYTES + TC_A_BYTES);
        wgmma_fence();
#pragma unroll
        for (int k = 0; k < TC_BK / 8; ++k)
          wgmma_tf32<BN>(acc, gmma_desc_sw128(sa + k * 32), gmma_desc_sw128(sb + k * 32), (it > 0 || k > 0) ? 1u : 0u);
        wgmma_commit();
        wgmma_wait<1>();
        if (it > 0 && (ct & 127) == 0) mbar_arrive(&empty[prev]);
        prev = stage;
        if (++stage == STAGES) {
          stage = 0;
          phase ^= 1;
        }
      }
      wgmma_wait<0>();
      wgmma_fence_regs<BN / 2>(acc);
      consumers_sync();
      store_acc_sw128<BN>(smem, acc, half * 64);
    }
    consumers_sync();
    const int q = (ct >> 5) & 3;
    const int m = ct & 127;
    const int lw = m & (BW - 1);
    const int lh = (m >> p.bw_log2) & (BH - 1);
    const int ln = m >> (p.bw_log2 + p.bh_log2);
    const int ow = w0 + lw, oh = h0 + lh, on = n0 + ln;
    const bool valid = (ow < p.Wo) && (oh < p.Ho) && (on < p.N);
    const float *cs = p.chan_scale && valid ? p.chan_scale + (int64_t)on * p.ldk + ntile * BN : nullptr;
    const bool partial = p.ksplit > 1;
    if (ct == 0) TC_TRACE(40);
#pragma unroll 1
    for (int c = half * 32; c < BN; c += 64) {
      float v[32];
      uint8_t *chunk = smem + (c >> 5) * TC_A_BYTES;
      ld_row32(chunk, m, v);
      epilogue_chunk(v, p.bias ? p.bias + (p.narrow_k ? 0 : ntile * BN + c) : nullptr, p.narrow_k, p.act, p.slope,
                     cs ? cs + c : nullptr, p.rtf);
      if (p.narrow_k) {
        if (valid) {
          float *dst = p.y + ((int64_t)(on * p.Ho + oh) * p.Wo + ow) * p.narrow_k;
#pragma unroll
          for (int j = 0; j < 32; ++j)
            if (j < p.narrow_k) dst[j] = v[j];
        }
      } else {
        st_row32(chunk, m, v);
      }
      if (p.stats) {
        float s2[32];
#pragma unroll
        for (int j = 0; j < 32; ++j) {
          v[j] = valid ? v[j] : 0.f;
          s2[j] = v[j] * v[j];
        }
        float cs1 = warp_colsum32(v, lane);
        float cs2 = warp_colsum32(s2, lane);
        red[(q * BN + c + lane) * 2 + 0] = cs1;
        red[(q * BN + c + lane) * 2 + 1] = cs2;
      }
    }
    fence_proxy_async();
    consumers_sync();
    if (ct == 0 && !p.narrow_k) {
      TC_TRACE(44);
#pragma unroll 1
      for (int c = 0; c < BN; c += 32) {
        if (partial)
          tma_reduce_add_5d(&tmY, smem + (c >> 5) * TC_A_BYTES, p.out_dc[ph] + ntile * BN + c, w0, p.out_da[ph], h0, n0);
        else
          tma_store_5d(&tmY, smem + (c >> 5) * TC_A_BYTES, p.out_dc[ph] + ntile * BN + c, w0, p.out_da[ph], h0, n0);
      }
      tma_store_commit_and_wait_read();
      TC_TRACE(45);
    }
    if (p.stats) {
      for (int e = ct; e < BN; e += 256) {
        float a = 0.f, b = 0.f;
#pragma unroll
        for (int qq = 0; qq < 4; ++qq) {
          a += red[(qq * BN + e) * 2 + 0];
          b += red[(qq * BN + e) * 2 + 1];
        }
        const int gidx = (p.stats_per_sample ? n0 * p.ldk : 0) + ntile * BN + e;
        atomicAdd(p.stats + gidx, (double)a);
        atomicAdd(p.stats + p.stats_groups + gidx, (double)b);
      }
    }
  }
  if (threadIdx.x == 128) TC_TRACE(42);
}

constexpr int MP_BN = 64;
constexpr int MP_STAGES = 6;
constexpr int MP_B_BYTES = MP_BN * TC_BK * 4;
constexpr int MP_MAX_USES = 2;
constexpr int MP_STEPS = 10;
constexpr int MP_STAGE_BYTES = TC_A_BYTES + MP_MAX_USES * MP_B_BYTES;
constexpr int MP_MAIN = MP_STAGES * MP_STAGE_BYTES;
static_assert(MP_MAIN >= 4 * 2 * TC_A_BYTES, "all-phase staging buffers");

struct MpStep {
  int8_t dw, dh, nb, pad_;
  int8_t acc[MP_MAX_USES];
  int8_t bt[MP_MAX_USES];
};

struct MpSchedule {
  MpStep s[MP_STEPS];
  int n;
};
__host__ __device__ constexpr MpSchedule mp_schedule() {
  MpSchedule r{};
  for (int dh = -1; dh <= 1; ++dh)
    for (int dw = -1; dw <= 1; ++dw) {
      int cur = -1;
      for (int a = 0; a < 2; ++a)
        for (int b = 0; b < 2; ++b) {
          const int dr = dh - a + 1, ds = dw - b + 1;
          if (dr < 0 || dr > 1 || ds < 0 || ds > 1) continue;
          if (cur < 0 || r.s[cur].nb == MP_MAX_USES) {
            cur = r.n++;
            r.s[cur].dw = (int8_t)dw;
            r.s[cur].dh = (int8_t)dh;
          }
          const int ph = a * 2 + b;
          r.s[cur].acc[r.s[cur].nb] = (int8_t)ph;
          r.s[cur].bt[r.s[cur].nb] = (int8_t)(ph * 4 + dr * 2 + ds);
          ++r.s[cur].nb;
        }
    }
  return r;
}
static_assert(mp_schedule().n == MP_STEPS, "all-phase step schedule");
__host__ __device__ constexpr bool mp_first_use(int S, int U) {
  const MpSchedule r = mp_schedule();
  for (int s = 0; s <= S; ++s)
// ... 131 lines not shown
      wgmma_fence_regs<BN / 2>(acc0);
      wgmma_fence_regs<BN / 2>(acc1);
      wgmma_fence_regs<BN / 2>(acc2);
      wgmma_fence_regs<BN / 2>(acc3);
    }
    consumers_sync();
    store_acc_sw128<BN>(smem + 0 * (2 * TC_A_BYTES), acc0, half * 64);
    store_acc_sw128<BN>(smem + 1 * (2 * TC_A_BYTES), acc1, half * 64);
    store_acc_sw128<BN>(smem + 2 * (2 * TC_A_BYTES), acc2, half * 64);
    store_acc_sw128<BN>(smem + 3 * (2 * TC_A_BYTES), acc3, half * 64);
    consumers_sync();
    const int q = (ct >> 5) & 3;
    const int m = ct & 127;
    const int c = half * 32;
    const int lw = m & (BW - 1);
    const int lh = (m >> p.bw_log2) & (BH - 1);
    const int ln = m >> (p.bw_log2 + p.bh_log2);
    const int ow = w0 + lw, oh = h0 + lh, on = n0 + ln;
    const bool valid = (ow < p.Wo) && (oh < p.Ho) && (on < p.N);
    const float *cs = p.chan_scale && valid ? p.chan_scale + (int64_t)on * p.ldk + ntile * BN + c : nullptr;
    const float *bias = p.bias ? p.bias + ntile * BN + c : nullptr;
    float st1 = 0.f, st2 = 0.f;
    if (ct == 0) TC_TRACE(40);
#pragma unroll 1
    for (int j = 0; j < 4; ++j) {
      uint8_t *buf = smem + j * (2 * TC_A_BYTES);
      float v[32];
      uint8_t *chunk = buf + half * TC_A_BYTES;
      ld_row32(chunk, m, v);
      epilogue_chunk(v, bias, 0, p.act, p.slope, cs, p.rtf);
      st_row32(chunk, m, v);
      if (p.stats) {
        float s2[32];
#pragma unroll
        for (int e = 0; e < 32; ++e) {
          v[e] = valid ? v[e] : 0.f;
          s2[e] = v[e] * v[e];
        }
        st1 += warp_colsum32(v, lane);
        st2 += warp_colsum32(s2, lane);
      }
      fence_proxy_async();
      consumers_sync();
      if (ct == 0) {
        TC_TRACE(50 + 3 * j);
#pragma unroll
        for (int cc = 0; cc < BN; cc += 32)
          tma_store_5d(&tmY, buf + (cc >> 5) * TC_A_BYTES, p.out_dc[j] + ntile * BN + cc, w0, p.out_da[j], h0, n0);
        asm volatile("cp.async.bulk.commit_group;" ::: "memory");
      }
    }
    if (ct == 0) {
      asm volatile("cp.async.bulk.wait_group.read 0;" ::: "memory");
      TC_TRACE(41);
    }
    if (p.stats) {
      red[(q * BN + c + lane) * 2 + 0] = st1;
      red[(q * BN + c + lane) * 2 + 1] = st2;
      consumers_sync();
      if (ct < BN) {
        float a = 0.f, b = 0.f;
#pragma unroll
        for (int qq = 0; qq < 4; ++qq) {
          a += red[(qq * BN + ct) * 2 + 0];
          b += red[(qq * BN + ct) * 2 + 1];
        }
        const int gidx = (p.stats_per_sample ? n0 * p.ldk : 0) + ntile * BN + ct;
        atomicAdd(p.stats + gidx, (double)a);
        atomicAdd(p.stats + p.stats_groups + gidx, (double)b);
      }
    }
  }
  if (threadIdx.x == 128) TC_TRACE(42);
}

int conv_stats_pass(const float *y, int N, int HW, int C, int per_sample, double *stats, cudaStream_t st);

static int ilog2_ceil(int v) {
  int l = 0;
  while ((1 << l) < v) ++l;
  return l;
}

template <class Params>
static int tc_setup(Params &p, int N, int Ho, int Wo, int ldk, const b200gan_epilogue *ep, double **deferred) {
  int bwl = ilog2_ceil(Wo);
  if (bwl > 7) bwl = 7;
  int bhl = ilog2_ceil(Ho);
  if (bhl > 7 - bwl) bhl = 7 - bwl;
  const int BNn = TC_BM / ((1 << bwl) * (1 << bhl));
  p.bw_log2 = bwl;
  p.bh_log2 = bhl;
  p.tiles_w = ceil_div(Wo, 1 << bwl);
  p.tiles_h = ceil_div(Ho, 1 << bhl);
  p.N = N;
  p.Ho = Ho;
  p.Wo = Wo;
  p.ldk = ldk;
  p.bias = ep ? ep->bias : nullptr;
  p.chan_scale = ep ? ep->chan_scale : nullptr;
  p.stats = ep ? ep->stats : nullptr;
  p.stats_per_sample = ep ? ep->stats_per_sample : 0;
  p.stats_groups = p.stats_per_sample ? N * ldk : ldk;
  p.act = ep ? ep->act : 0;
  p.slope = ep ? ep->slope : 0.f;
  p.rtf = ep ? ep->round_tf32 : 0;
  *deferred = nullptr;
  if (p.stats && p.stats_per_sample && BNn != 1) {
    *deferred = p.stats;
    p.stats = nullptr;
  }
  p.trace = nullptr;
  if (const char *tv = getenv("B200GAN_TC_TRACE")) p.trace = reinterpret_cast<long long *>(strtoull(tv, nullptr, 0));
  return BNn;
}

template <int BN, int STAGES>
static int launch_tc(const CUtensorMap &tmA, const CUtensorMap &tmB, const CUtensorMap &tmY, const TcParams &p, dim3 grid,
                     cudaStream_t st) {
  constexpr int SMEM = TcSmem<BN, STAGES>::TOTAL;
  static std::atomic<uint64_t> attr_done{0};
  if (int e = ensure_dynamic_smem(conv_tc_kernel<BN, STAGES>, SMEM, attr_done)) return e;
  conv_tc_kernel<BN, STAGES><<<grid, TC_THREADS, SMEM, st>>>(tmA, tmB, tmY, p);
  B2_LAUNCH_CHECK();
  return B200GAN_OK;
}

int tc_wgrad_supported(const b200gan_conv_geom *g);

static bool tc_is_gather(const b200gan_conv_geom *g, int pass) { return (pass == 0) != (g->transposed != 0); }

int tc_supported(const b200gan_conv_geom *g, int pass) {
  if (g->pad_mode != B200GAN_PAD_ZERO || g->N < 1) return 0;
  if (pass == 2) return tc_wgrad_supported(g);
  if (g->stride != 1 && g->stride != 2) return 0;
  const int cin = pass == 0 ? g->C : g->K;
  const int cout = pass == 0 ? g->K : g->C;
  const bool narrow = cout < 32 && pass == 0 && !g->transposed && g->up == 1 && g->stride == 1;
  if (cin % 32 != 0 || (cout % 32 != 0 && !narrow) || 2 * cin > 32767) return 0;
  if (g->R * g->S > 49 || g->R > 15 || g->S > 15 || g->pad_t > 15 || g->pad_l > 15) return 0;
  if (g->up == 2) {
    if (g->transposed || g->stride != 1) return 0;
    if (!(g->R == 3 && g->S == 3 && g->pad_t == 1 && g->pad_l == 1 && g->pad_b == 1 && g->pad_r == 1)) return 0;
    return cout % 64 == 0;
  }
  if (g->stride == 2) {
    const int Hf = g->transposed ? g->P : g->H, Wf = g->transposed ? g->Q : g->W;
    if ((Hf & 1) || (Wf & 1)) return 0;
    if (!tc_is_gather(g, pass)) {
      int taps = 0;
      for (int a = 0; a < 2; ++a)
        for (int b = 0; b < 2; ++b) {
          int nr = 0, ns = 0;
          for (int r = 0; r < g->R; ++r) nr += ((a + g->pad_t - r) % 2 == 0);
          for (int s2 = 0; s2 < g->S; ++s2) ns += ((b + g->pad_l - s2) % 2 == 0);
          taps += nr * ns;
        }
      if (taps > TC_MAX_TAPS) return 0;
    }
  }
  return 1;
}

static int run_tc(const float *in, int N, int Hi, int Wi, int Cc, bool phase_in, const float *packedB, int Kout,
                  int btaps, int nphase, const int *tap_begin, const TcTap *taps, int Ho, int Wo, bool phase_out,
                  const int *out_dc, const int *out_da, int ldk, const b200gan_epilogue *ep, float *y,
                  cudaStream_t st) {
  const int narrow_k = Kout < 32 ? Kout : 0;
  const int Kreal = Kout;
  if (narrow_k) Kout = 32;
  int BN = (Kout % 128 == 0) ? 128 : (Kout % 64 == 0 ? 64 : 32);
  TcParams p;
  memset(&p, 0, sizeof(p));
  const int total_taps = tap_begin[nphase];
  for (int i = 0; i <= 4; ++i) p.tap_begin[i] = tap_begin[i < nphase ? i : nphase];
  for (int i = 0; i < total_taps; ++i) p.taps[i] = taps[i];
  p.kout_total = Kout;
  p.kchunks = Cc / TC_BK;
  double *deferred_stats;
  const int BNn = tc_setup(p, N, Ho, Wo, ldk, ep, &deferred_stats);
  const int BW = 1 << p.bw_log2, BH = 1 << p.bh_log2;
  {
    const int64_t tiles = (int64_t)p.tiles_w * p.tiles_h * ceil_div(N, BNn) * nphase;
    if (Kout % 256 == 0 && tiles * (Kout / 256) >= num_sms()) BN = 256;
  }
  for (int i = 0; i < 4; ++i) {
    p.out_dc[i] = i < nphase ? out_dc[i] : 0;
    p.out_da[i] = i < nphase ? out_da[i] : 0;
  }
  p.y = y;
  p.narrow_k = narrow_k;
  if (narrow_k) {
    B2_CHECK_ARG(!phase_in && !phase_out && nphase == 1, "tensor-core conv: narrow output only in the plain gather form");
    B2_CHECK_ARG(!p.chan_scale, "tensor-core conv: Dropout2d scale with fewer than 32 output channels");
  }
  p.ksplit = 1;
  if (narrow_k && p.stats) {
    deferred_stats = p.stats;
    p.stats = nullptr;
  }
  {
    const bool plain = !p.bias && !p.chan_scale && p.act == B200GAN_ACT_NONE && !p.rtf;
    const int64_t ctas = (int64_t)p.tiles_w * p.tiles_h * ceil_div(N, BNn) * (Kout / BN) * nphase;
    int min_iters = 1 << 30;
    for (int z = 0; z < nphase; ++z) {
      const int it = (tap_begin[z + 1] - tap_begin[z]) * p.kchunks;
      if (it < min_iters) min_iters = it;
    }
    if (plain && !narrow_k && ctas < num_sms() && min_iters >= 16) {
      int ks = (int)((2 * num_sms() + ctas - 1) / ctas);
      if (ks > min_iters / 8) ks = min_iters / 8;
      if (ks > 32) ks = 32;
      if (ks >= 2) {
        p.ksplit = ks;
        if (p.stats) {
          deferred_stats = p.stats;
          p.stats = nullptr;
        }
      }
    }
  }
  B2_CHECK_ARG(((uintptr_t)in % 16 == 0) && ((uintptr_t)packedB % 16 == 0) && ((uintptr_t)y % 16 == 0),
               "tensor-core conv: pointers must be 16-byte aligned");
  if (p.ksplit > 1) {
    const int64_t out_elems = phase_out ? (int64_t)N * (2 * Ho) * (2 * Wo) * ldk : (int64_t)N * Ho * Wo * ldk;
    B2_CUDA(cudaMemsetAsync(y, 0, (size_t)out_elems * sizeof(float), st));
  }

  CUtensorMap tmA, tmB, tmY;
  if (!narrow_k) {
    uint64_t dims[5], strides[4];
    uint32_t box[5] = {TC_BK, (uint32_t)BW, 1, (uint32_t)BH, (uint32_t)BNn};
    const uint64_t L = (uint64_t)ldk;
    if (!phase_out) {
      dims[0] = L; dims[1] = Wo; dims[2] = 1; dims[3] = Ho; dims[4] = N;
      strides[0] = L * 4; strides[1] = (uint64_t)Wo * L * 4; strides[2] = (uint64_t)Wo * L * 4;
      strides[3] = (uint64_t)Ho * Wo * L * 4;
    } else {
      dims[0] = 2 * L; dims[1] = Wo; dims[2] = 2; dims[3] = Ho; dims[4] = N;
      strides[0] = 2 * L * 4; strides[1] = (uint64_t)2 * Wo * L * 4; strides[2] = (uint64_t)4 * Wo * L * 4;
      strides[3] = (uint64_t)4 * Ho * Wo * L * 4;
    }
    if (int e = make_tmap_f32(&tmY, y, 5, dims, strides, box)) return e;
  }
  {
    uint64_t dims[5], strides[4];
    uint32_t box[5] = {TC_BK, (uint32_t)BW, 1, (uint32_t)BH, (uint32_t)BNn};
    if (!phase_in) {
      dims[0] = Cc; dims[1] = Wi; dims[2] = 1; dims[3] = Hi; dims[4] = N;
      strides[0] = (uint64_t)Cc * 4;
      strides[1] = (uint64_t)Wi * Cc * 4;
      strides[2] = (uint64_t)Wi * Cc * 4;
      strides[3] = (uint64_t)Hi * Wi * Cc * 4;
    } else {
      dims[0] = 2 * (uint64_t)Cc; dims[1] = Wi / 2; dims[2] = 2; dims[3] = Hi / 2; dims[4] = N;
      strides[0] = (uint64_t)2 * Cc * 4;
      strides[1] = (uint64_t)Wi * Cc * 4;
      strides[2] = (uint64_t)2 * Wi * Cc * 4;
      strides[3] = (uint64_t)Hi * Wi * Cc * 4;
    }
    if (int e = make_tmap_f32(&tmA, in, 5, dims, strides, box)) return e;
  }
  if (narrow_k) tmY = tmA;
  {
    uint64_t dims[3] = {(uint64_t)Cc, (uint64_t)Kreal, (uint64_t)btaps};
    uint64_t strides[2] = {(uint64_t)Cc * 4, (uint64_t)Kreal * Cc * 4};
    uint32_t box[3] = {TC_BK, (uint32_t)BN, 1};
    if (int e = make_tmap_f32(&tmB, packedB, 3, dims, strides, box)) return e;
  }
  dim3 grid((unsigned)(p.tiles_w * p.tiles_h * ceil_div(N, BNn)), (unsigned)(Kout / BN), (unsigned)(nphase * p.ksplit));
  int rc;
  if (BN == 256) rc = launch_tc<256, 4>(tmA, tmB, tmY, p, grid, st);
  else if (BN == 128) rc = launch_tc<128, 6>(tmA, tmB, tmY, p, grid, st);
  else if (BN == 64) rc = launch_tc<64, 8>(tmA, tmB, tmY, p, grid, st);
  else rc = launch_tc<32, 8>(tmA, tmB, tmY, p, grid, st);
  if (rc == B200GAN_OK && deferred_stats)
    rc = conv_stats_pass(y, N, phase_out ? 4 * Ho * Wo : Ho * Wo, ldk, p.stats_per_sample, deferred_stats, st);
  return rc;
}

static int run_up2_allphase(const float *x, int N, int H, int W, int C, const float *packed, int K,
                            const b200gan_epilogue *ep, float *y, cudaStream_t st) {
  MpParams p;
  memset(&p, 0, sizeof(p));
  constexpr MpSchedule sched = mp_schedule();
  for (int i = 0; i < MP_STEPS; ++i) p.steps[i] = sched.s[i];
  p.kout_total = K;
  p.kchunks = C / TC_BK;
  double *deferred_stats;
  const int BNn = tc_setup(p, N, H, W, K, ep, &deferred_stats);
  const int BW = 1 << p.bw_log2, BH = 1 << p.bh_log2;
  for (int ph = 0; ph < 4; ++ph) {
    p.out_dc[ph] = (ph & 1) * K;
    p.out_da[ph] = ph >> 1;
  }
  B2_CHECK_ARG(((uintptr_t)x % 16 == 0) && ((uintptr_t)packed % 16 == 0) && ((uintptr_t)y % 16 == 0),
               "tensor-core conv: pointers must be 16-byte aligned");
  CUtensorMap tmA, tmB, tmY;
  uint32_t box[5] = {TC_BK, (uint32_t)BW, 1, (uint32_t)BH, (uint32_t)BNn};
  {
    const uint64_t L = (uint64_t)K;
    uint64_t dims[5] = {2 * L, (uint64_t)W, 2, (uint64_t)H, (uint64_t)N};
    uint64_t strides[4] = {2 * L * 4, (uint64_t)2 * W * L * 4, (uint64_t)4 * W * L * 4, (uint64_t)4 * H * W * L * 4};
    if (int e = make_tmap_f32(&tmY, y, 5, dims, strides, box)) return e;
  }
  {
    uint64_t dims[5] = {(uint64_t)C, (uint64_t)W, 1, (uint64_t)H, (uint64_t)N};
    uint64_t strides[4] = {(uint64_t)C * 4, (uint64_t)W * C * 4, (uint64_t)W * C * 4, (uint64_t)H * W * C * 4};
    if (int e = make_tmap_f32(&tmA, x, 5, dims, strides, box)) return e;
  }
  {
    uint64_t dims[2] = {(uint64_t)C, (uint64_t)16 * K};
    uint64_t strides[1] = {(uint64_t)C * 4};
    uint32_t bbox[2] = {TC_BK, (uint32_t)MP_BN};
    if (int e = make_tmap_f32(&tmB, packed, 2, dims, strides, bbox)) return e;
  }
  constexpr int SMEM = MP_MAIN + 1024 + 256 + 4 * MP_BN * 2 * 4;
  static std::atomic<uint64_t> attr_done{0};
  if (int e = ensure_dynamic_smem(conv_tc_up2_allphase_kernel, SMEM, attr_done)) return e;
  dim3 grid((unsigned)(p.tiles_w * p.tiles_h * ceil_div(N, BNn)), (unsigned)(K / MP_BN), 1);
  conv_tc_up2_allphase_kernel<<<grid, TC_THREADS, SMEM, st>>>(tmA, tmB, tmY, p);
  B2_LAUNCH_CHECK();
  if (deferred_stats) return conv_stats_pass(y, N, 4 * H * W, K, p.stats_per_sample, deferred_stats, st);
  return B200GAN_OK;
}

static inline int floordiv2(int v) { return v >= 0 ? v / 2 : -((-v + 1) / 2); }

static int tc_gather(const float *in, int N, int Hi, int Wi, int Cc, int R, int S, int stride, int pad_t, int pad_l,
                     const float *packedB, int Kout, int Po, int Qo, const b200gan_epilogue *ep, float *out,
                     cudaStream_t st) {
  TcTap taps[TC_MAX_TAPS];
  memset(taps, 0, sizeof(taps));
  int tap_begin[5] = {0, 0, 0, 0, 0};
  int out_dc[4] = {0, 0, 0, 0}, out_da[4] = {0, 0, 0, 0};
  int nt = 0;
  for (int r = 0; r < R; ++r)
    for (int s = 0; s < S; ++s) {
      TcTap &t = taps[nt];
      const int eh = r - pad_t, ew = s - pad_l;
      if (stride == 1) {
        t.dc = 0; t.dw = (int8_t)ew; t.da = 0; t.dh = (int8_t)eh;
      } else {
        t.dh = (int8_t)floordiv2(eh); t.da = (int8_t)(eh & 1);
        t.dw = (int8_t)floordiv2(ew); t.dc = (int16_t)((ew & 1) * Cc);
      }
      t.bt = (int8_t)nt;
      ++nt;
    }
  tap_begin[1] = nt;
  return run_tc(in, N, Hi, Wi, Cc, stride == 2, packedB, Kout, R * S, 1, tap_begin, taps, Po, Qo, false, out_dc, out_da,
                Kout, ep, out, st);
}

static int tc_scatter(const float *in, int N, int Pi, int Qi, int Cc, int R, int S, int stride, int pad_t, int pad_l,
                      const float *packedB, int Kout, int Ho, int Wo, const b200gan_epilogue *ep, float *out,
                      cudaStream_t st) {
  TcTap taps[TC_MAX_TAPS];
  memset(taps, 0, sizeof(taps));
  int tap_begin[5] = {0, 0, 0, 0, 0};
  int out_dc[4] = {0, 0, 0, 0}, out_da[4] = {0, 0, 0, 0};
  if (stride == 1) {
    int nt = 0;
    for (int r = 0; r < R; ++r)
      for (int s = 0; s < S; ++s) {
        TcTap &t = taps[nt];
        t.dc = 0; t.dw = (int8_t)(pad_l - s); t.da = 0; t.dh = (int8_t)(pad_t - r); t.bt = (int8_t)nt;
        ++nt;
      }
    tap_begin[1] = nt;
    return run_tc(in, N, Pi, Qi, Cc, false, packedB, Kout, R * S, 1, tap_begin, taps, Ho, Wo, false, out_dc, out_da, Kout,
                  ep, out, st);
  }
  int nt = 0;
  for (int ph = 0; ph < 4; ++ph) {
    const int a = ph >> 1, b = ph & 1;
    tap_begin[ph] = nt;
    for (int r = 0; r < R; ++r) {
      if ((a + pad_t - r) % 2 != 0) continue;
      for (int s = 0; s < S; ++s) {
        if ((b + pad_l - s) % 2 != 0) continue;
        TcTap &t = taps[nt++];
        t.dc = 0; t.da = 0;
        t.dh = (int8_t)((a + pad_t - r) / 2);
        t.dw = (int8_t)((b + pad_l - s) / 2);
        t.bt = (int8_t)(r * S + s);
      }
    }
    out_dc[ph] = b * Kout;
    out_da[ph] = a;
  }
  tap_begin[4] = nt;
  return run_tc(in, N, Pi, Qi, Cc, false, packedB, Kout, R * S, 4, tap_begin, taps, Ho / 2, Wo / 2, true, out_dc, out_da,
                Kout, ep, out, st);
}

int tc_fprop(const b200gan_conv_geom *g, const b200gan_epilogue *ep, const float *x, const float *packed, float *y,
             cudaStream_t st) {
  b200gan_epilogue e2;
  if (ep) e2 = *ep;
  const b200gan_epilogue *e = ep ? &e2 : nullptr;
  if (g->up == 2) {
    if (g->K % 128 != 0 && g->K % 64 == 0)
      return run_up2_allphase(x, g->N, g->H, g->W, g->C, packed, g->K, e, y, st);
    TcTap taps[TC_MAX_TAPS];
    memset(taps, 0, sizeof(taps));
    int tap_begin[5] = {0, 4, 8, 12, 16};
    int out_dc[4], out_da[4];
    for (int ph = 0; ph < 4; ++ph) {
      int a = ph >> 1, b = ph & 1;
      for (int tp = 0; tp < 4; ++tp) {
        int dr = tp >> 1, ds = tp & 1;
        TcTap &t = taps[ph * 4 + tp];
        t.dc = 0; t.dw = (int8_t)(b - 1 + ds); t.da = 0; t.dh = (int8_t)(a - 1 + dr); t.bt = (int8_t)(ph * 4 + tp);
      }
      out_dc[ph] = b * g->K;
      out_da[ph] = a;
    }
    return run_tc(x, g->N, g->H, g->W, g->C, false, packed, g->K, 16, 4, tap_begin, taps, g->H, g->W, true, out_dc, out_da,
                  g->K, e, y, st);
  }
  if (g->transposed)
    return tc_scatter(x, g->N, g->H, g->W, g->C, g->R, g->S, g->stride, g->pad_t, g->pad_l, packed, g->K, g->P, g->Q, e, y,
                      st);
  return tc_gather(x, g->N, g->H, g->W, g->C, g->R, g->S, g->stride, g->pad_t, g->pad_l, packed, g->K, g->P, g->Q, e, y, st);
}

int tc_dgrad(const b200gan_conv_geom *g, const float *dy, const float *packed, float *dx, cudaStream_t st) {
  if (g->up == 2) {
    TcTap taps[TC_MAX_TAPS];
    memset(taps, 0, sizeof(taps));
    int tap_begin[5] = {0, 16, 16, 16, 16};
    int out_dc[4] = {0, 0, 0, 0}, out_da[4] = {0, 0, 0, 0};
    for (int ph = 0; ph < 4; ++ph) {
      int a = ph >> 1, b = ph & 1;
      for (int tp = 0; tp < 4; ++tp) {
        int dr = tp >> 1, ds = tp & 1;
        TcTap &t = taps[ph * 4 + tp];
        t.dc = (int16_t)(b * g->K); t.dw = (int8_t)(-(b - 1 + ds)); t.da = (int8_t)a; t.dh = (int8_t)(-(a - 1 + dr));
        t.bt = (int8_t)(ph * 4 + tp);
      }
    }
    return run_tc(dy, g->N, g->P, g->Q, g->K, true, packed, g->C, 16, 1, tap_begin, taps, g->H, g->W, false, out_dc, out_da,
                  g->C, nullptr, dx, st);
  }
  if (g->transposed)
    return tc_gather(dy, g->N, g->P, g->Q, g->K, g->R, g->S, g->stride, g->pad_t, g->pad_l, packed, g->C, g->H, g->W, nullptr,
                     dx, st);
  return tc_scatter(dy, g->N, g->P, g->Q, g->K, g->R, g->S, g->stride, g->pad_t, g->pad_l, packed, g->C, g->H, g->W, nullptr,
                    dx, st);
}

}
```

### pytorch-gan_b200/csrc/norm.cu

```cuda
#include "common.cuh"
#include <initializer_list>
#include <stdlib.h>

namespace b200gan {

__global__ void __launch_bounds__(256)
norm_stats_kernel(const float *__restrict__ x, double *__restrict__ stats, int C, int64_t rows,
                  int64_t rows_per_block, int G, int per_sample) {
  __shared__ float s1[8][33], s2[8][33];
  const int c = blockIdx.x * 32 + threadIdx.x;
  const int64_t base_row = per_sample ? (int64_t)blockIdx.z * rows : 0;
  int64_t r0 = (int64_t)blockIdx.y * rows_per_block;
  int64_t r1 = r0 + rows_per_block;
  if (r1 > rows) r1 = rows;
  float a = 0.f, b = 0.f;
  if (c < C) {
    const float *xp = x + (base_row + r0) * C + c;
    for (int64_t r = r0 + threadIdx.y; r < r1; r += 8) {
      float v = __ldg(xp + (r - r0) * C);
      a += v;
      b = fmaf(v, v, b);
    }
  }
  s1[threadIdx.y][threadIdx.x] = a;
// ... 181 lines not shown
  const bool from_x = scale_shift != nullptr && (act == B200GAN_ACT_LRELU || act == B200GAN_ACT_RELU);
  float mean[VEC], rstd[VEC], gr[VEC], m1[VEC], m2[VEC], sc[VEC], sh[VEC];
#pragma unroll
  for (int j = 0; j < VEC; ++j) {
    mean[j] = __ldg(mean_rstd + gbase + j);
    rstd[j] = __ldg(mean_rstd + G + gbase + j);
    gr[j] = (gamma ? __ldg(gamma + s.cv * VEC + j) : 1.f) * rstd[j];
    m1[j] = (float)sums[gbase + j] * inv_count;
    m2[j] = (float)sums[G + gbase + j] * inv_count;
    sc[j] = from_x ? __ldg(scale_shift + gbase + j) : 1.f;
    sh[j] = from_x ? __ldg(scale_shift + G + gbase + j) : 0.f;
  }
  const int64_t base = (gridDim.y > 1 ? (int64_t)blockIdx.y * rows : 0);
  const V *dyv = reinterpret_cast<const V *>(dy) + base * s.CV + s.cv;
  const V *xv = reinterpret_cast<const V *>(x) + base * s.CV + s.cv;
  const V *yv = reinterpret_cast<const V *>(y) + base * s.CV + s.cv;
  V *dxv = reinterpret_cast<V *>(dx) + base * s.CV + s.cv;
  const bool need_y = act != B200GAN_ACT_NONE && !from_x;
  const int CV = s.CV;
  const int64_t step = (int64_t)gridDim.x * s.rpb;
#pragma unroll 4
  for (int64_t r = s.first_row(rows); r < rows; r += step) {
    float dd[VEC], xx[VEC], yy[VEC], o[VEC];
    unpack(__ldg(dyv + r * CV), dd);
    unpack(__ldg(xv + r * CV), xx);
    unpack(need_y ? __ldg(yv + r * CV) : V{}, yy);
#pragma unroll
    for (int j = 0; j < VEC; ++j) {
      const float dz = dd[j] * norm_act_grad(xx[j], sc[j], sh[j], yy[j], from_x, act, slope);
      const float v = gr[j] * (dz - m1[j] - ((xx[j] - mean[j]) * rstd[j]) * m2[j]);
      o[j] = rtf ? round_tf32(v) : v;
    }
    dxv[r * CV] = pack(o);
  }
}

__global__ void norm_bwd_params_kernel(double *__restrict__ sums, float *__restrict__ dgb, int G) {
  int g = blockIdx.x * blockDim.x + threadIdx.x;
  if (g >= G) return;
  if (dgb) {
    dgb[g] = (float)sums[G + g];
    dgb[G + g] = (float)sums[g];
  }
  sums[g] = 0.0;
  sums[G + g] = 0.0;
}

static int vec_width(int C, std::initializer_list<const void *> streamed) {
  uintptr_t bits = 0;
  for (const void *p : streamed) bits |= (uintptr_t)p;
  return C % 4 == 0 && (bits & 15) == 0 ? 4 : 1;
}
static dim3 slice_grid(const b200gan_norm_desc *d, int vec, int64_t &rows) {
  rows = d->per_sample ? (int64_t)d->HW : (int64_t)d->N * d->HW;
  const int CV = d->C / vec;
  const int64_t ny = d->per_sample ? d->N : 1, nz = ceil_div(CV, 256);
  const int rpb = 256 / (CV < 256 ? CV : 256);
  int64_t want = (num_sms() * 8 + ny * nz - 1) / (ny * nz);
  int64_t maxb = ceil_div64(rows, (int64_t)rpb * 4);
  if (want > maxb) want = maxb;
  if (want < 1) want = 1;
  return dim3((unsigned)want, (unsigned)ny, (unsigned)nz);
}

static void reduce_grid(const b200gan_norm_desc *d, dim3 &grid, int64_t &rows, int64_t &rpb) {
  rows = d->per_sample ? (int64_t)d->HW : (int64_t)d->N * d->HW;
  int xb = ceil_div(d->C, 32);
  int zb = d->per_sample ? d->N : 1;
  int64_t want = (num_sms() * 8) / ((int64_t)xb * zb);
  if (want < 1) want = 1;
  rpb = ceil_div64(rows, want);
  if (rpb < 32) rpb = 32;
  int64_t yb = ceil_div64(rows, rpb);
  grid = dim3((unsigned)xb, (unsigned)yb, (unsigned)zb);
}

static int check_desc(const b200gan_norm_desc *d) {
  B2_CHECK_ARG(d != nullptr, "norm: null descriptor");
  B2_CHECK_ARG(d->N > 0 && d->HW > 0 && d->C > 0, "norm: bad dims N=%d HW=%d C=%d", d->N, d->HW, d->C);
  B2_CHECK_ARG(!d->per_sample || d->N <= 65535, "norm: N too large for per-sample grid");
  return B200GAN_OK;
}

}

using namespace b200gan;

extern "C" int b200gan_norm_stats(const b200gan_norm_desc *d, const float *x, double *stats,
                                  void *stream) {
  if (int e = check_desc(d)) return e;
  B2_CHECK_ARG(x && stats, "norm_stats: null pointer");
  dim3 grid;
  int64_t rows, rpb;
  reduce_grid(d, grid, rows, rpb);
  int G = d->per_sample ? d->N * d->C : d->C;
  norm_stats_kernel<<<grid, dim3(32, 8), 0, as_stream(stream)>>>(x, stats, d->C, rows, rpb, G,
                                                                 d->per_sample);
  B2_LAUNCH_CHECK();
  return B200GAN_OK;
}

extern "C" int b200gan_norm_finalize(const b200gan_norm_desc *d, double *stats,
                                     const float *gamma, const float *beta, float *mean_rstd,
                                     float *scale_shift, float *running_mean, float *running_var,
                                     int64_t *num_batches_tracked, void *stream) {
  if (int e = check_desc(d)) return e;
  B2_CHECK_ARG(stats && mean_rstd && scale_shift, "norm_finalize: null pointer");
  B2_CHECK_ARG(!(running_mean && d->per_sample), "norm_finalize: running stats with per-sample norm");
  B2_CHECK_ARG((running_mean == nullptr) == (running_var == nullptr),
               "norm_finalize: running_mean/var must both be given");
  int G = d->per_sample ? d->N * d->C : d->C;
  double count = d->per_sample ? (double)d->HW : (double)d->N * (double)d->HW;
  norm_finalize_kernel<<<ceil_div(G, 128), 128, 0, as_stream(stream)>>>(
      stats, gamma, beta, mean_rstd, scale_shift, running_mean, running_var, num_batches_tracked, G,
      d->C, count, d->eps, d->momentum);
  B2_LAUNCH_CHECK();
  return B200GAN_OK;
}

extern "C" int b200gan_norm_apply(const b200gan_norm_desc *d, const float *x,
                                  const float *scale_shift, float *y, void *stream) {
  if (int e = check_desc(d)) return e;
  B2_CHECK_ARG(x && scale_shift && y, "norm_apply: null pointer");
  const int G = d->per_sample ? d->N * d->C : d->C;
  const int vec = vec_width(d->C, {x, y, scale_shift});
  int64_t rows;
  const dim3 grid = slice_grid(d, vec, rows);
  auto kernel = vec == 4 ? norm_apply_kernel<4> : norm_apply_kernel<1>;
  kernel<<<grid, 256, 0, as_stream(stream)>>>(x, scale_shift, y, rows, d->C, G, d->act, d->slope, d->round_tf32);
  B2_LAUNCH_CHECK();
  return B200GAN_OK;
}

extern "C" int b200gan_norm_bwd(const b200gan_norm_desc *d, const float *dy, const float *x,
                                const float *y, const float *mean_rstd, const float *scale_shift,
                                const float *gamma, double *sums, float *dx, float *dgamma_dbeta, void *stream) {
  if (int e = check_desc(d)) return e;
  B2_CHECK_ARG(dy && x && mean_rstd && sums && dx, "norm_bwd: null pointer");
  const bool from_x = scale_shift && (d->act == B200GAN_ACT_LRELU || d->act == B200GAN_ACT_RELU);
  B2_CHECK_ARG(d->act == B200GAN_ACT_NONE || from_x || y != nullptr,
               "norm_bwd: fused activation needs the saved output y (or scale_shift for LeakyReLU / ReLU)");
  cudaStream_t st = as_stream(stream);
  const int G = d->per_sample ? d->N * d->C : d->C;
  const float *yy = y ? y : x;
  const int vec = vec_width(d->C, {dy, x, dx, yy});
  int64_t rows;
  const dim3 grid = slice_grid(d, vec, rows);
  auto reduce = vec == 4 ? norm_bwd_reduce_kernel<4> : norm_bwd_reduce_kernel<1>;
  reduce<<<grid, 256, 0, st>>>(dy, x, yy, mean_rstd, scale_shift, sums, rows, d->C, G, d->act, d->slope);
  B2_LAUNCH_CHECK();
  const float inv = (float)(1.0 / (d->per_sample ? (double)d->HW : (double)d->N * (double)d->HW));
  auto apply = vec == 4 ? norm_bwd_apply_kernel<4> : norm_bwd_apply_kernel<1>;
  apply<<<grid, 256, 0, st>>>(dy, x, yy, mean_rstd, scale_shift, gamma, sums, dx, rows, d->C, G, inv, d->act, d->slope,
                              d->round_tf32);
  B2_LAUNCH_CHECK();
  norm_bwd_params_kernel<<<ceil_div(G, 128), 128, 0, st>>>(sums, dgamma_dbeta, G);
  B2_LAUNCH_CHECK();
  return B200GAN_OK;
}
```

### pytorch-gan_b200/csrc/wgrad_tc.cu

```cuda
#include "tc_common.cuh"
#include <stdlib.h>

namespace b200gan {

constexpr int WG_THREADS = 384;
constexpr int WG_MAX_JOBS = 52;
constexpr int WG_PIX = 32;
constexpr int WG_CHUNK_BYTES = WG_PIX * 128;

struct WgJob {
  int16_t s_dc, d_dc;
  int8_t s_da, d_da;
  int8_t s_dw, s_dh;
};

struct WgParams {
  WgJob jobs[WG_MAX_JOBS];
  int32_t njobs;
  int32_t bw_log2, bh_log2;
  int32_t tiles_w, tiles_h, N;
  int32_t imgs_per_box;
  int32_t tiles_total, tiles_per_split;
  int32_t s_is_a;
  int32_t mtiles, ntiles;
  int32_t ldn;
  int32_t mtotal;
  float *partial;
};

template <int NB, int STAGES>
struct WgSmem {
  static constexpr int A_BYTES = 4 * WG_CHUNK_BYTES;
  static constexpr int B_BYTES = (NB / 32) * WG_CHUNK_BYTES;
  static constexpr int STAGE_BYTES = A_BYTES + B_BYTES;
  static constexpr int RING = STAGES * STAGE_BYTES;
  static constexpr int T_BYTES = NB * 128;
  static constexpr int STAGING = (NB / 32) * 16384;
  static constexpr int MAIN = RING + 2 * T_BYTES > STAGING ? RING + 2 * T_BYTES : STAGING;
  static constexpr int TOTAL = MAIN + 1024 + 256;
  static_assert(TOTAL <= 232448, "wgrad_tc_kernel: shared memory");
};

__device__ __forceinline__ void wg_consumers_sync() { asm volatile("bar.sync 1, 256;" ::: "memory"); }

__device__ __forceinline__ int wg_kpos(int p) { return (p & ~7) | ((p & 7) >> 1) | ((p & 1) << 2); }

template <int NB, int STAGES>
__global__ void __launch_bounds__(WG_THREADS, 1)
wgrad_tc_kernel(const __grid_constant__ CUtensorMap tmX, const __grid_constant__ CUtensorMap tmY,
                const __grid_constant__ CUtensorMap tmP, const __grid_constant__ WgParams p) {
  using L = WgSmem<NB, STAGES>;
  extern __shared__ uint8_t smem_raw[];
  uint8_t *smem = reinterpret_cast<uint8_t *>((reinterpret_cast<uintptr_t>(smem_raw) + 1023) & ~(uintptr_t)1023);
  uint64_t *full = reinterpret_cast<uint64_t *>(smem + L::MAIN);
  uint64_t *empty = full + STAGES;

  const int warp = threadIdx.x >> 5, lane = threadIdx.x & 31;
  const int split = blockIdx.x, job = blockIdx.y;
  const int mt = blockIdx.z / p.ntiles, nt = blockIdx.z % p.ntiles;
  const int t_begin = split * p.tiles_per_split;
  int t_end = t_begin + p.tiles_per_split;
  if (t_end > p.tiles_total) t_end = p.tiles_total;
  const int iters = t_end - t_begin;

  if (threadIdx.x == 0) {
    tma_prefetch_desc(&tmX);
    tma_prefetch_desc(&tmY);
    for (int s = 0; s < STAGES; ++s) {
      mbar_init(&full[s], 1);
      mbar_init(&empty[s], 256);
    }
    fence_barrier_init();
  }
  __syncthreads();

  if (warp < 4) {
    setmaxnreg_dec<40>();
    if (warp == 0 && lane == 0) {
      const WgJob jb = p.jobs[job];
      const CUtensorMap *mapA = p.s_is_a ? &tmX : &tmY;
      const CUtensorMap *mapB = p.s_is_a ? &tmY : &tmX;
      const int a_dc = p.s_is_a ? jb.s_dc : jb.d_dc, a_da = p.s_is_a ? jb.s_da : jb.d_da;
      const int a_dw = p.s_is_a ? jb.s_dw : 0, a_dh = p.s_is_a ? jb.s_dh : 0;
      const int b_dc = p.s_is_a ? jb.d_dc : jb.s_dc, b_da = p.s_is_a ? jb.d_da : jb.s_da;
      const int b_dw = p.s_is_a ? 0 : jb.s_dw, b_dh = p.s_is_a ? 0 : jb.s_dh;
      int stage = 0;
      uint32_t phase = 0;
      for (int it = 0; it < iters; ++it) {
        int t = t_begin + it;
        const int tw = t % p.tiles_w;
        t /= p.tiles_w;
        const int th = t % p.tiles_h;
        const int n = (t / p.tiles_h) * p.imgs_per_box;
        const int w0 = tw << p.bw_log2, h0 = th << p.bh_log2;
        mbar_wait(&empty[stage], phase ^ 1);
        uint8_t *sa = smem + stage * L::STAGE_BYTES;
        uint8_t *sb = sa + L::A_BYTES;
        mbar_arrive_expect_tx(&full[stage], L::STAGE_BYTES);
#pragma unroll
        for (int c = 0; c < 4; ++c)
          tma_load_5d(sa + c * WG_CHUNK_BYTES, mapA, &full[stage], a_dc + (mt * 4 + c) * 32, w0 + a_dw, a_da,
                      h0 + a_dh, n);
#pragma unroll
        for (int c = 0; c < NB / 32; ++c)
          tma_load_5d(sb + c * WG_CHUNK_BYTES, mapB, &full[stage], b_dc + (nt * (NB / 32) + c) * 32, w0 + b_dw, b_da,
                      h0 + b_dh, n);
        if (++stage == STAGES) {
          stage = 0;
          phase ^= 1;
        }
      }
    }
  } else {
    setmaxnreg_inc<232>();
    if (iters == 0) return;
    const int ct = threadIdx.x - 128;
    const int half = ct >> 7;
    const int tp = ct & 31, tq = ct >> 5;
    const int tk = wg_kpos(tp);
    const int wq = tq & 3;
    const int ac = 16 * (wq & 1) + (lane >> 2), ap = 2 * (lane & 3);
    const int abase = (2 * half + (wq >> 1)) * WG_CHUNK_BYTES + ap * 128 + (ac & 3) * 4;
    const uint32_t aoff[4] = {
        (uint32_t)(abase + ((((ac >> 2)) ^ ap) << 4)),
        (uint32_t)(abase + ((((ac >> 2) + 2) ^ ap) << 4)),
        (uint32_t)(abase + 128 + ((((ac >> 2)) ^ (ap + 1)) << 4)),
        (uint32_t)(abase + 128 + ((((ac >> 2) + 2) ^ (ap + 1)) << 4))};
    float acc[NB / 2];
    int stage = 0;
    uint32_t phase = 0;
    auto prepare = [&](int it, uint32_t(&fa)[16]) {
      uint8_t *tb = smem + L::RING + (it & 1) * L::T_BYTES;
      mbar_wait(&full[stage], phase);
      wg_consumers_sync();
      const uint8_t *src = smem + stage * L::STAGE_BYTES;
#pragma unroll
      for (int k = 0; k < WG_PIX / 8; ++k)
#pragma unroll
        for (int j = 0; j < 4; ++j) fa[4 * k + j] = *reinterpret_cast<const uint32_t *>(src + aoff[j] + k * 1024);
#pragma unroll
      for (int c = 0; c < NB / 32; ++c) {
        const float4 v = *reinterpret_cast<const float4 *>(src + L::A_BYTES + c * WG_CHUNK_BYTES + tp * 128 +
                                                           ((tq ^ (tp & 7)) << 4));
        const float e[4] = {v.x, v.y, v.z, v.w};
#pragma unroll
        for (int i = 0; i < 4; ++i) {
          const int r = c * 32 + tq * 4 + i;
          *reinterpret_cast<float *>(tb + r * 128 + (((tk >> 2) ^ (r & 7)) << 4) + (tk & 3) * 4) = e[i];
        }
      }
      mbar_arrive(&empty[stage]);
      fence_proxy_async();
      wg_consumers_sync();
      if (++stage == STAGES) {
        stage = 0;
        phase ^= 1;
      }
    };
    auto mma = [&](int it, const uint32_t(&fa)[16]) {
      const uint32_t sb = smem_u32(smem + L::RING + (it & 1) * L::T_BYTES);
      wgmma_fence();
#pragma unroll
      for (int k = 0; k < WG_PIX / 8; ++k)
        wgmma_tf32_rs<NB>(acc, fa + 4 * k, gmma_desc_sw128(sb + k * 32), (it > 0 || k > 0) ? 1u : 0u);
      wgmma_commit();
    };
    uint32_t fa0[16], fa1[16];
    prepare(0, fa0);
#pragma unroll 1
    for (int it = 0; it < iters; it += 2) {
      mma(it, fa0);
      if (it + 1 < iters) prepare(it + 1, fa1);
      wgmma_wait<0>();
      if (it + 1 < iters) {
        mma(it + 1, fa1);
        if (it + 2 < iters) prepare(it + 2, fa0);
        wgmma_wait<0>();
      }
    }
    wgmma_wait<0>();
    wgmma_fence_regs<NB / 2>(acc);
    wg_consumers_sync();
    store_acc_sw128<NB>(smem, acc, half * 64);
    fence_proxy_async();
    wg_consumers_sync();
    if (ct == 0) {
      const int row0 = job * p.mtotal + mt * 128;
#pragma unroll 1
      for (int c = 0; c < NB; c += 32) tma_reduce_add_2d(&tmP, smem + (c >> 5) * 16384, nt * NB + c, row0);
      tma_store_commit_and_wait_read();
    }
  }
}

struct WgReduceP {
  int32_t K, C, R, S, njobs, s_is_a, up2, transposed;
  int32_t mtotal, ldn;
};
__device__ __forceinline__ bool up2_contrib(int r, int a, int d) {
  if (a == 0) return d == 0 ? r == 0 : r >= 1;
  return d == 0 ? r <= 1 : r == 2;
}
__global__ void wgrad_reduce_kernel(const float *__restrict__ partial, float *__restrict__ dw, WgReduceP p) {
  int64_t total = (int64_t)p.K * p.C * p.R * p.S;
  for (int64_t i = (int64_t)blockIdx.x * blockDim.x + threadIdx.x; i < total;
       i += (int64_t)gridDim.x * blockDim.x) {
    int c = (int)(i % p.C);
    int64_t t = i / p.C;
    int k = (int)(t % p.K);
    t /= p.K;
    int s = (int)(t % p.S), r = (int)(t / p.S);
    const int sch = p.transposed ? k : c;
    const int dch = p.transposed ? c : k;
    int64_t elem = p.s_is_a ? (int64_t)sch * p.ldn + dch : (int64_t)dch * p.ldn + sch;
    int64_t job_stride = (int64_t)p.mtotal * p.ldn;
    const float *base = partial + elem;
    float acc = 0.f;
    if (!p.up2) {
      acc = __ldg(base + (int64_t)(r * p.S + s) * job_stride);
    } else {
      for (int j = 0; j < 16; ++j) {
        int ph = j >> 2, tp = j & 3;
        if (up2_contrib(r, ph >> 1, tp >> 1) && up2_contrib(s, ph & 1, tp & 1)) acc += __ldg(base + j * job_stride);
      }
    }
    const int64_t o = p.transposed ? (((int64_t)c * p.K + k) * p.R + r) * p.S + s
                                   : (((int64_t)k * p.C + c) * p.R + r) * p.S + s;
    dw[o] = acc;
  }
}


constexpr int WR_COL = 32, WR_ROW = 8, WR_TAPS = 16;
__global__ void __launch_bounds__(256)
wgrad_reduce_tile_kernel(const float *__restrict__ partial, float *__restrict__ dw, WgReduceP p) {
  __shared__ float s[WR_ROW][WR_COL][WR_TAPS + 1];
  const int RS = p.R * p.S;
  const int tin = p.up2 ? 16 : RS;
  const bool col_is_k = (p.s_is_a != 0) != (p.transposed != 0);
  const int ncol = col_is_k ? p.K : p.C, nrow = col_is_k ? p.C : p.K;
  const int tiles_col = (ncol + WR_COL - 1) / WR_COL;
  const int col0 = (blockIdx.x % tiles_col) * WR_COL, row0 = (blockIdx.x / tiles_col) * WR_ROW;
  const int64_t job_stride = (int64_t)p.mtotal * p.ldn;
  const int tid = threadIdx.x;
  for (int e = tid; e < WR_COL * WR_ROW * tin; e += 256) {
    const int cl = e % WR_COL, rw = (e / WR_COL) % WR_ROW, j = e / (WR_COL * WR_ROW);
    float v = 0.f;
    if (col0 + cl < ncol && row0 + rw < nrow) v = __ldg(partial + j * job_stride + (int64_t)(row0 + rw) * p.ldn + col0 + cl);
    s[rw][cl][j] = v;
  }
  __syncthreads();
  const bool col_is_b = col_is_k == (p.transposed != 0);
  const int nb = p.transposed ? p.K : p.C;
  for (int e = tid; e < WR_COL * WR_ROW * RS; e += 256) {
    const int t = e % RS;
    int cl, rw;
    if (col_is_b) { cl = (e / RS) % WR_COL; rw = e / (RS * WR_COL); }
    else          { rw = (e / RS) % WR_ROW; cl = e / (RS * WR_ROW); }
    const int col = col0 + cl, row = row0 + rw;
    if (col >= ncol || row >= nrow) continue;
    float acc;
    if (!p.up2) {
      acc = s[rw][cl][t];
    } else {
// ... 22 lines not shown
  int ipb;
};

static bool wg_plan(const b200gan_conv_geom *g, WgPlan &pl) {
  if (g->pad_mode != B200GAN_PAD_ZERO || g->N < 1) return false;
  if (g->stride != 1 && g->stride != 2) return false;
  if (g->C % 32 || g->K % 32 || 2 * g->C > 32767 || 2 * g->K > 32767) return false;
  const bool up2 = g->up == 2;
  if (up2 && (g->transposed || g->stride != 1 ||
              !(g->R == 3 && g->S == 3 && g->pad_t == 1 && g->pad_l == 1 && g->pad_b == 1 && g->pad_r == 1)))
    return false;
  if (g->R * g->S > WG_MAX_JOBS || g->R > 15 || g->S > 15 || g->pad_t > 15 || g->pad_l > 15) return false;
  pl.sch = g->transposed ? g->K : g->C;
  pl.dch = g->transposed ? g->C : g->K;
  if (g->stride == 2) {
    const int Hf = g->transposed ? g->P : g->H, Wf = g->transposed ? g->Q : g->W;
    if ((Hf & 1) || (Wf & 1)) return false;
  }
  if (pl.dch % 128 == 0) pl.s_is_a = 0;
  else if (pl.sch % 128 == 0) pl.s_is_a = 1;
  else return false;
  const int mch = pl.s_is_a ? pl.sch : pl.dch, nch = pl.s_is_a ? pl.dch : pl.sch;
  pl.NB = nch % 128 == 0 ? 128 : (nch % 64 == 0 ? 64 : 32);
  if (nch % 256 == 0) pl.NB = 256;
  pl.mtotal = mch;
  pl.ldn = nch;
  pl.mtiles = mch / 128;
  pl.ntiles = nch / pl.NB;
  pl.njobs = up2 ? 16 : g->R * g->S;
  pl.Ho = up2 ? g->H : (g->transposed ? g->H : g->P);
  pl.Wo = up2 ? g->W : (g->transposed ? g->W : g->Q);
  const int pl2 = 5;
  pl.bwl = ilog2c(pl.Wo);
  if (pl.bwl > pl2) pl.bwl = pl2;
  pl.bhl = ilog2c(pl.Ho);
  if (pl.bhl > pl2 - pl.bwl) pl.bhl = pl2 - pl.bwl;
  pl.tiles_w = ceil_div(pl.Wo, 1 << pl.bwl);
  pl.tiles_h = ceil_div(pl.Ho, 1 << pl.bhl);
  pl.ipb = WG_PIX >> (pl.bwl + pl.bhl);
  int64_t tt = (int64_t)ceil_div(g->N, pl.ipb) * pl.tiles_w * pl.tiles_h;
  if (tt > (1 << 30)) return false;
  pl.tiles_total = (int)tt;
  const int64_t ctas_per_split = (int64_t)pl.njobs * pl.mtiles * pl.ntiles;
  int max_ns = pl.tiles_total / 8;
  if (max_ns < 1) max_ns = 1;
  if (max_ns > 4 * num_sms()) max_ns = 4 * num_sms();
  int ns = 1;
  int64_t best = -1;
  for (int s = 1; s <= max_ns; ++s) {
    const int64_t waves = ceil_div64(s * ctas_per_split, num_sms());
    const int64_t cost = waves * (ceil_div(pl.tiles_total, s) + 8);
    if (best < 0 || cost < best) {
      best = cost;
      ns = s;
    }
  }
  pl.tps = ceil_div(pl.tiles_total, ns);
  pl.nsplits = ceil_div(pl.tiles_total, pl.tps);
  return true;
}

int tc_wgrad_supported(const b200gan_conv_geom *g) {
  WgPlan pl;
  return wg_plan(g, pl) ? 1 : 0;
}

size_t tc_wgrad_workspace_floats(const b200gan_conv_geom *g) {
  WgPlan pl;
  if (!wg_plan(g, pl)) return 0;
  return (size_t)pl.njobs * pl.mtotal * pl.ldn;
}

template <int NB, int STAGES>
static int launch_wg(const CUtensorMap &tmX, const CUtensorMap &tmY, const CUtensorMap &tmP, const WgParams &p, dim3 grid,
                     cudaStream_t st) {
  constexpr int SMEM = WgSmem<NB, STAGES>::TOTAL;
  static std::atomic<uint64_t> attr_done{0};
  if (int e = ensure_dynamic_smem(wgrad_tc_kernel<NB, STAGES>, SMEM, attr_done)) return e;
  wgrad_tc_kernel<NB, STAGES><<<grid, WG_THREADS, SMEM, st>>>(tmX, tmY, tmP, p);
  B2_LAUNCH_CHECK();
  return B200GAN_OK;
}

int tc_wgrad(const b200gan_conv_geom *g, const float *x, const float *dy, float *dw, float *ws, cudaStream_t st) {
  WgPlan pl;
  if (!wg_plan(g, pl)) B2_UNSUPPORTED("tensor-core wgrad: geometry not supported");
  B2_CHECK_ARG(ws != nullptr, "tensor-core wgrad: workspace required");
  B2_CHECK_ARG(((uintptr_t)x % 16 == 0) && ((uintptr_t)dy % 16 == 0) && ((uintptr_t)ws % 16 == 0),
               "tensor-core wgrad: pointers must be 16-byte aligned");
  const bool up2 = g->up == 2;
  const int st2 = g->stride == 2;
  WgParams p;
  memset(&p, 0, sizeof(p));
  p.njobs = pl.njobs;
  if (up2) {
    for (int ph = 0; ph < 4; ++ph)
      for (int tp = 0; tp < 4; ++tp) {
        int a = ph >> 1, b = ph & 1, dr = tp >> 1, ds = tp & 1;
        WgJob &j = p.jobs[ph * 4 + tp];
        j.d_dc = (int16_t)(b * g->K); j.d_da = (int8_t)a; j.s_dh = (int8_t)(a - 1 + dr); j.s_dw = (int8_t)(b - 1 + ds);
      }
  } else {
    for (int r = 0; r < g->R; ++r)
      for (int s2 = 0; s2 < g->S; ++s2) {
        WgJob &j = p.jobs[r * g->S + s2];
        const int eh = r - g->pad_t, ew = s2 - g->pad_l;
        if (!st2) {
          j.s_dh = (int8_t)eh; j.s_dw = (int8_t)ew;
        } else {
          j.s_dh = (int8_t)(eh >= 0 ? eh / 2 : -((-eh + 1) / 2)); j.s_da = (int8_t)(eh & 1);
          j.s_dw = (int8_t)(ew >= 0 ? ew / 2 : -((-ew + 1) / 2)); j.s_dc = (int16_t)((ew & 1) * pl.sch);
        }
      }
  }
  p.bw_log2 = pl.bwl; p.bh_log2 = pl.bhl;
  p.tiles_w = pl.tiles_w; p.tiles_h = pl.tiles_h; p.N = g->N; p.imgs_per_box = pl.ipb;
  p.tiles_total = pl.tiles_total; p.tiles_per_split = pl.tps;
  p.s_is_a = pl.s_is_a; p.mtiles = pl.mtiles; p.ntiles = pl.ntiles; p.ldn = pl.ldn; p.mtotal = pl.mtotal;
  p.partial = ws;

  const float *sptr = g->transposed ? dy : x, *dptr = g->transposed ? x : dy;
  const uint64_t Hs = g->transposed ? g->P : g->H, Ws = g->transposed ? g->Q : g->W, Cs = pl.sch;
  const uint64_t Hd = g->transposed ? g->H : g->P, Wd = g->transposed ? g->W : g->Q, Cd = pl.dch;
  CUtensorMap tmX, tmY;
  const uint32_t box[5] = {32, (uint32_t)(1 << pl.bwl), 1, (uint32_t)(1 << pl.bhl), (uint32_t)pl.ipb};
  {
    uint64_t dims[5], strides[4];
    if (!st2) {
      dims[0] = Cs; dims[1] = Ws; dims[2] = 1; dims[3] = Hs; dims[4] = g->N;
      strides[0] = Cs * 4; strides[1] = Ws * Cs * 4; strides[2] = Ws * Cs * 4; strides[3] = Hs * Ws * Cs * 4;
    } else {
      dims[0] = 2 * Cs; dims[1] = Ws / 2; dims[2] = 2; dims[3] = Hs / 2; dims[4] = g->N;
      strides[0] = 2 * Cs * 4; strides[1] = Ws * Cs * 4; strides[2] = 2 * Ws * Cs * 4; strides[3] = Hs * Ws * Cs * 4;
    }
    if (int e = make_tmap_f32(&tmX, sptr, 5, dims, strides, box)) return e;
  }
  {
    uint64_t dims[5], strides[4];
    if (!up2) {
      dims[0] = Cd; dims[1] = Wd; dims[2] = 1; dims[3] = Hd; dims[4] = g->N;
      strides[0] = Cd * 4; strides[1] = Wd * Cd * 4; strides[2] = Wd * Cd * 4; strides[3] = Hd * Wd * Cd * 4;
    } else {
      dims[0] = 2 * Cd; dims[1] = Wd / 2; dims[2] = 2; dims[3] = Hd / 2; dims[4] = g->N;
      strides[0] = 2 * Cd * 4; strides[1] = Wd * Cd * 4; strides[2] = 2 * Wd * Cd * 4; strides[3] = Hd * Wd * Cd * 4;
    }
    if (int e = make_tmap_f32(&tmY, dptr, 5, dims, strides, box)) return e;
  }
  CUtensorMap tmP;
  {
    uint64_t dims[2] = {(uint64_t)pl.ldn, (uint64_t)pl.njobs * pl.mtotal};
    uint64_t strides[1] = {(uint64_t)pl.ldn * 4};
    uint32_t pbox[2] = {32, 128};
    if (int e = make_tmap_f32(&tmP, ws, 2, dims, strides, pbox)) return e;
  }
  B2_CUDA(cudaMemsetAsync(ws, 0, (size_t)pl.njobs * pl.mtotal * pl.ldn * sizeof(float), st));
  dim3 grid((unsigned)pl.nsplits, (unsigned)pl.njobs, (unsigned)(pl.mtiles * pl.ntiles));
  int rc = pl.NB == 256 ? launch_wg<256, 3>(tmX, tmY, tmP, p, grid, st)
           : pl.NB == 128 ? launch_wg<128, 6>(tmX, tmY, tmP, p, grid, st)
           : pl.NB == 64 ? launch_wg<64, 8>(tmX, tmY, tmP, p, grid, st)
                         : launch_wg<32, 8>(tmX, tmY, tmP, p, grid, st);
  if (rc) return rc;
  WgReduceP rp;
  rp.K = g->K; rp.C = g->C; rp.R = g->R; rp.S = g->S; rp.njobs = pl.njobs;
  rp.s_is_a = pl.s_is_a; rp.up2 = up2 ? 1 : 0; rp.transposed = g->transposed ? 1 : 0; rp.mtotal = pl.mtotal; rp.ldn = pl.ldn;
  int64_t total = (int64_t)g->K * g->C * g->R * g->S;
  if (g->R * g->S <= WR_TAPS && g->K >= 32 && g->C >= 32) {
    const bool col_is_k = (pl.s_is_a != 0) != (g->transposed != 0);
    const int ncol = col_is_k ? g->K : g->C, nrow = col_is_k ? g->C : g->K;
    const unsigned tiles = (unsigned)(ceil_div(ncol, WR_COL) * ceil_div(nrow, WR_ROW));
    wgrad_reduce_tile_kernel<<<tiles, 256, 0, st>>>(ws, dw, rp);
    B2_LAUNCH_CHECK();
    return B200GAN_OK;
  }
  unsigned blocks = (unsigned)(ceil_div64(total, 256) > num_sms() * 16 ? num_sms() * 16 : ceil_div64(total, 256));
  wgrad_reduce_kernel<<<blocks, 256, 0, st>>>(ws, dw, rp);
  B2_LAUNCH_CHECK();
  return B200GAN_OK;
}

}
```

Baseline: 46960.

## Fuse BatchNorm backward reduction into conv dgrad and bias grad into wgrad

Adds a fused BatchNorm+Conv autograd path for stride-1 convs that follow a training BatchNorm. The tensor-core dgrad kernel accumulates the norm backward reduction sums in its epilogue, so the separate norm_bwd reduce pass over dy and x is skipped. The TC wgrad kernel also accumulates the bias gradient with atomics while streaming dy, replacing a separate bias reduction. This adds atomics and extra epilogue work, and there is a risk of slower kernels from register pressure.

```diff
diff --git a/include/b200gan.h b/include/b200gan.h
--- a/include/b200gan.h
+++ b/include/b200gan.h
@@ -86,6 +86,8 @@
 size_t b200gan_conv2d_wgrad_workspace_floats(const b200gan_conv_geom *g, int algo);
 int b200gan_conv2d_wgrad(const b200gan_conv_geom *g, const float *x, const float *dy, float *dw,
                          float *db, float *workspace, int algo, void *stream);
+int b200gan_conv2d_wgrad_fused_bias(const b200gan_conv_geom *g, const float *x, const float *dy, float *dw,
+                                    float *db, float *workspace, int algo, void *stream);
 
 int b200gan_epilogue_bwd(const float *dy, const float *y, const float *chan_scale, int32_t act,
                          float slope, int64_t n, int32_t K, int64_t PQ, int32_t round_tf32,
@@ -114,6 +116,14 @@
 int b200gan_norm_bwd(const b200gan_norm_desc *d, const float *dy, const float *x, const float *y,
                      const float *mean_rstd, const float *scale_shift, const float *gamma, double *sums, float *dx,
                      float *dgamma_dbeta, void *stream);
+
+int b200gan_conv2d_dgrad_norm_supported(const b200gan_conv_geom *g);
+int b200gan_conv2d_dgrad_norm(const b200gan_conv_geom *g, const b200gan_norm_desc *d, const float *dy,
+                              const float *packed, const float *x, const float *mean_rstd, const float *scale_shift,
+                              double *sums, float *dx, void *stream);
+int b200gan_norm_bwd_from_sums(const b200gan_norm_desc *d, const float *dy, const float *x, const float *mean_rstd,
+                               const float *scale_shift, const float *gamma, double *sums, float *dx,
+                               float *dgamma_dbeta, void *stream);
 
 typedef struct b200gan_tail_desc {
   int32_t N, H, W, C;
diff --git a/pytorch-gan_b200/b200gan/_lib.py b/pytorch-gan_b200/b200gan/_lib.py
--- a/pytorch-gan_b200/b200gan/_lib.py
+++ b/pytorch-gan_b200/b200gan/_lib.py
@@ -82,12 +82,16 @@
     "b200gan_conv2d_dgrad": (c_i32, [_P(ConvGeom), c_vp, c_vp, c_vp, c_vp, c_i32, c_vp]),
     "b200gan_conv2d_wgrad_workspace_floats": (c_sz, [_P(ConvGeom), c_i32]),
     "b200gan_conv2d_wgrad": (c_i32, [_P(ConvGeom), c_vp, c_vp, c_vp, c_vp, c_vp, c_i32, c_vp]),
+    "b200gan_conv2d_wgrad_fused_bias": (c_i32, [_P(ConvGeom), c_vp, c_vp, c_vp, c_vp, c_vp, c_i32, c_vp]),
     "b200gan_epilogue_bwd": (c_i32, [c_vp, c_vp, c_vp, c_i32, c_f32, c_i64, c_i32, c_i64, c_i32, c_vp, c_vp]),
     "b200gan_bias_grad": (c_i32, [c_vp, c_vp, c_vp, c_i32, c_f32, c_i64, c_i32, c_i64, c_vp, c_vp]),
     "b200gan_norm_stats": (c_i32, [_P(NormDesc), c_vp, c_vp, c_vp]),
     "b200gan_norm_finalize": (c_i32, [_P(NormDesc), c_vp, c_vp, c_vp, c_vp, c_vp, c_vp, c_vp, c_vp, c_vp]),
     "b200gan_norm_apply": (c_i32, [_P(NormDesc), c_vp, c_vp, c_vp, c_vp]),
     "b200gan_norm_bwd": (c_i32, [_P(NormDesc), c_vp, c_vp, c_vp, c_vp, c_vp, c_vp, c_vp, c_vp, c_vp, c_vp]),
+    "b200gan_conv2d_dgrad_norm_supported": (c_i32, [_P(ConvGeom)]),
+    "b200gan_conv2d_dgrad_norm": (c_i32, [_P(ConvGeom), _P(NormDesc)] + [c_vp] * 8),
+    "b200gan_norm_bwd_from_sums": (c_i32, [_P(NormDesc)] + [c_vp] * 9),
     "b200gan_tail_supported": (c_i32, [_P(TailDesc)]),
     "b200gan_tail_fprop": (c_i32, [_P(TailDesc), c_vp, c_vp, c_vp, c_vp, c_vp, c_vp]),
     "b200gan_tail_bwd_workspace_bytes": (c_sz, [_P(TailDesc)]),
diff --git a/pytorch-gan_b200/b200gan/functional.py b/pytorch-gan_b200/b200gan/functional.py
--- a/pytorch-gan_b200/b200gan/functional.py
+++ b/pytorch-gan_b200/b200gan/functional.py
@@ -248,6 +248,74 @@
             if spec.per_sample:
                 dgamma, dbeta = dgamma.view(n, c).sum(0), dbeta.view(n, c).sum(0)
         return dx, dgamma, dbeta, None, None, None, None, None
+
+
+class NormConvFn(torch.autograd.Function):
+
+    @staticmethod
+    def forward(ctx, x, gamma, beta, stats, running_mean, running_var, nbt, weight, bias, chan_scale, nspec: NormSpec,
+                cspec: ConvSpec, cache: PackCache):
+        ops._require_cuda(x, "norm input")
+        ops._require_cuda(weight, "conv weight")
+        x = _as_cl(x)
+        a, mean_rstd, scale_shift = ops.norm_forward(
+            x, None if gamma is None else gamma.detach(), None if beta is None else beta.detach(), running_mean,
+            running_var, nbt, False, nspec.eps, nspec.momentum, nspec.act, nspec.slope, stats, nspec.rtf_out,
+            return_scale_shift=True)
+        g, _ = ops.make_geom(tuple(a.shape), tuple(weight.shape), cspec.stride, cspec.pads, cspec.pad_mode, cspec.up)
+        algo, kind = ops.conv_plan(g, 0, chan_scale)
+        packed = cache.get(g, weight.detach(), kind)
+        out_stats = None
+        if cspec.stats is not None:
+            out_stats = ops.zero_scratch(x.device, 2 * (g.N * g.K if cspec.stats else g.K))
+        y = ops.conv_fprop(g, a, packed, algo, bias=None if bias is None else bias.detach(), act=cspec.act,
+                           slope=cspec.slope, chan_scale=chan_scale, stats=out_stats,
+                           stats_per_sample=bool(cspec.stats), round_tf32=cspec.rtf_out)
+        ctx.nspec, ctx.cspec, ctx.cache, ctx.g = nspec, cspec, cache, g
+        ctx.has_bias = bias is not None
+        ctx.save_for_backward(x, mean_rstd, scale_shift, gamma, a, weight, y if cspec.act != ACT_NONE else None,
+                              chan_scale)
+        if out_stats is not None:
+            ctx.mark_non_differentiable(out_stats)
+            ctx.set_materialize_grads(False)
+            return y, out_stats
+        return y
+
+    @staticmethod
+    @torch.autograd.function.once_differentiable
+    def backward(ctx, dy, *unused):
+        x, mean_rstd, scale_shift, gamma, a, weight, y, chan_scale = ctx.saved_tensors
+        nspec, cspec, g = ctx.nspec, ctx.cspec, ctx.g
+        dy = _as_cl(dy)
+        if cspec.act != ACT_NONE or chan_scale is not None:
+            dz = ops.epilogue_bwd(dy, y, chan_scale, cspec.act, cspec.slope, cspec.rtf_dz)
+        else:
+            dz = dy
+        nig = ctx.needs_input_grad
+        dx = dgamma = dbeta = dw = db = None
+        need_params = gamma is not None and (nig[1] or nig[2])
+        if nig[0] or need_params:
+            algo, kind = ops.conv_plan(g, 1)
+            da, sums = ops.conv_dgrad_norm(g, dz, ctx.cache.get(g, weight.detach(), kind), x, mean_rstd, scale_shift,
+                                           nspec.act, nspec.slope)
+            dx, dgb = ops.norm_backward_from_sums(da, x, mean_rstd, None if gamma is None else gamma.detach(), sums,
+                                                  nspec.eps, nspec.act, nspec.slope, need_params, nspec.rtf_dx,
+                                                  scale_shift)
+            if need_params:
+                c = x.shape[1]
+                dgamma, dbeta = dgb[:c], dgb[c:]
+            if not nig[0]:
+                dx = None
+        want_db = ctx.has_bias and nig[8]
+        if want_db and dz is not dy and cspec.rtf_dz:
+            db = ops.bias_grad(dy, y, chan_scale, cspec.act, cspec.slope)
+            want_db = False
+        if nig[7] or want_db:
+            dw, db2 = ops.conv_wgrad(g, a, dz, tuple(weight.shape), want_db, ops.conv_plan(g, 2)[0])
+            db = db2 if want_db else db
+            if not nig[7]:
+                dw = None
+        return dx, dgamma, dbeta, None, None, None, None, dw, db, None, None, None, None
 
 
 @dataclass(frozen=True)
diff --git a/pytorch-gan_b200/b200gan/nn.py b/pytorch-gan_b200/b200gan/nn.py
--- a/pytorch-gan_b200/b200gan/nn.py
+++ b/pytorch-gan_b200/b200gan/nn.py
@@ -90,6 +90,14 @@
     if p >= 1.0:
         return noise.zero_().view(n, c)
     return noise.bernoulli_(1.0 - p).div_(1.0 - p).view(n, c)
+
+
+def _conv_cache(conv):
+    cache = conv.__dict__.get("_b200_cache")
+    if cache is None:
+        cache = PackCache()
+        conv.__dict__["_b200_cache"] = cache
+    return cache
 
 
 def _run_conv(conv, x, up=1, extra_pads=(0, 0, 0, 0), pad_mode=PAD_ZERO, act=ACT_NONE, slope=0.0, chan_scale=None,
@@ -106,11 +114,19 @@
     pads = tuple(e + pad for e in extra_pads)
     spec = ConvSpec(stride=int(conv.stride[0]), pads=pads, pad_mode=pad_mode, up=up, transposed=transposed, act=act,
                     slope=slope, stats=stats, rtf_out=rtf_out, rtf_dz=rtf_dz)
-    cache = conv.__dict__.get("_b200_cache")
-    if cache is None:
-        cache = PackCache()
-        conv.__dict__["_b200_cache"] = cache
-    return F.conv_block(x, conv.weight, conv.bias, chan_scale, spec, cache)
+    return F.conv_block(x, conv.weight, conv.bias, chan_scale, spec, _conv_cache(conv))
+
+
+def _batch_norm_spec(norm, per_sample, act, slope, rtf_out, rtf_dx):
+    rm = rv = nbt = None
+    momentum = 0.0
+    if not per_sample and norm.training and norm.track_running_stats:
+        if norm.momentum is None:
+            raise NotImplementedError("b200gan: BatchNorm2d(momentum=None)")
+        rm, rv, nbt, momentum = norm.running_mean, norm.running_var, norm.num_batches_tracked, float(norm.momentum)
+    spec = NormSpec(per_sample=per_sample, eps=float(norm.eps), momentum=momentum, act=act, slope=slope,
+                    rtf_out=rtf_out, rtf_dx=rtf_dx)
+    return spec, rm, rv, nbt
 
 
 def _run_norm(norm, x, act=ACT_NONE, slope=0.0, stats=None, rtf_out=False, rtf_dx=False):
@@ -125,14 +141,7 @@
     if use_batch_stats and not per_sample:
         _no_groups("a stand-alone BatchNorm2d")
     if use_batch_stats:
-        rm = rv = nbt = None
-        momentum = 0.0
-        if not per_sample and norm.training and norm.track_running_stats:
-            if norm.momentum is None:
-                raise NotImplementedError("b200gan: BatchNorm2d(momentum=None)")
-            rm, rv, nbt, momentum = norm.running_mean, norm.running_var, norm.num_batches_tracked, float(norm.momentum)
-        spec = NormSpec(per_sample=per_sample, eps=float(norm.eps), momentum=momentum, act=act, slope=slope,
-                        rtf_out=rtf_out, rtf_dx=rtf_dx)
+        spec, rm, rv, nbt = _batch_norm_spec(norm, per_sample, act, slope, rtf_out, rtf_dx)
         return F.norm_block(x, norm.weight, norm.bias, stats, rm, rv, nbt, spec)
     rstd = torch.rsqrt(norm.running_var + norm.eps)
     scale = rstd if norm.weight is None else norm.weight * rstd
@@ -299,6 +308,29 @@
 
     def __init__(self, norm_step, conv_step):
         self.norm_step, self.conv_step = norm_step, conv_step
+
+
+def _no_hooks(m):
+    return not (m._forward_hooks or m._forward_pre_hooks or m._backward_hooks)
+
+
+def _norm_conv_fused(ns, cs, x_shape):
+    if not (isinstance(ns, _NormStep) and isinstance(cs, _ConvStep)):
+        return False
+    norm, conv = ns.norm, cs.conv
+    if not isinstance(norm, _T["BatchNorm2d"]) or ns.act not in (ACT_NONE, ACT_LRELU, ACT_RELU):
+        return False
+    if isinstance(conv, _T["ConvTranspose2d"]) or cs.pad_mode != PAD_ZERO or tuple(conv.stride) != (1, 1):
+        return False
+    if not (_no_hooks(norm) and _no_hooks(conv) and norm.training and ops.bn_groups.active <= 1):
+        return False
+    if norm.track_running_stats and norm.momentum is None:
+        return False
+    if not (len(x_shape) == 4 and x_shape[1] == norm.num_features == conv.in_channels):
+        return False
+    pads = tuple(e + int(conv.padding[0]) for e in cs.extra_pads)
+    g, _ = ops.make_geom(tuple(x_shape), tuple(conv.weight.shape), 1, pads, PAD_ZERO, cs.up)
+    return ops.conv_dgrad_norm_supported(g)
 
 
 def _chain_plan(chain, shape):
@@ -673,6 +705,20 @@
                 else:
                     queue[0:0] = [ns, cs]
                 continue
+            if queue and _norm_conv_fused(s, queue[0], tuple(x.shape)):
+                ns, cs = s, queue.pop(0)
+                scale = None
+                if cs.dropout2d is not None and cs.dropout2d.training and cs.dropout2d.p > 0.0:
+                    scale = _dropout2d_scale((x.shape[0], cs.conv.out_channels), cs.dropout2d.p, x.device)
+                want = cs.stats if (cs.next_norm is not None and _uses_batch_stats(cs.next_norm)) else None
+                norm, conv = ns.norm, cs.conv
+                nspec, rm, rv, nbt = _batch_norm_spec(norm, False, ns.act, ns.slope, ns.rtf_out, ns.rtf_dx)
+                cspec = ConvSpec(stride=1, pads=tuple(e + int(conv.padding[0]) for e in cs.extra_pads), up=cs.up,
+                                 act=cs.act, slope=cs.slope, stats=want, rtf_out=cs.rtf_out, rtf_dz=cs.rtf_dz)
+                out = F.NormConvFn.apply(x, norm.weight, norm.bias, stats if ns.takes_stats else None, rm, rv, nbt,
+                                         conv.weight, conv.bias, scale, nspec, cspec, _conv_cache(conv))
+                x, stats = out if want is not None else (out, None)
+                continue
             if isinstance(s, _ConvStep):
                 cs = None
                 if s.dropout2d is not None and s.dropout2d.training and s.dropout2d.p > 0.0:
diff --git a/pytorch-gan_b200/b200gan/ops.py b/pytorch-gan_b200/b200gan/ops.py
--- a/pytorch-gan_b200/b200gan/ops.py
+++ b/pytorch-gan_b200/b200gan/ops.py
@@ -159,8 +159,8 @@
     db = torch.empty(g.K, device=x.device, dtype=torch.float32) if need_bias else None
     nws = lib.b200gan_conv2d_wgrad_workspace_floats(ctypes.byref(g), algo)
     ws = torch.empty(nws, device=x.device, dtype=torch.float32) if nws else None
-    _lib.check(lib.b200gan_conv2d_wgrad(ctypes.byref(g), x.data_ptr(), dy.data_ptr(), dw.data_ptr(), _ptr(db),
-                                        _ptr(ws), algo, _stream()), "conv2d_wgrad")
+    _lib.check(lib.b200gan_conv2d_wgrad_fused_bias(ctypes.byref(g), x.data_ptr(), dy.data_ptr(), dw.data_ptr(),
+                                                   _ptr(db), _ptr(ws), algo, _stream()), "conv2d_wgrad")
     return dw, db
 
 
@@ -297,6 +297,33 @@
     _lib.check(lib.b200gan_norm_bwd(ctypes.byref(d), dy.data_ptr(), x.data_ptr(), _ptr(y), mean_rstd.data_ptr(),
                                     _ptr(scale_shift), _ptr(gamma), sums.data_ptr(), dx.data_ptr(), _ptr(dgb), _stream()),
                "norm_bwd")
+    return dx, dgb
+
+
+def conv_dgrad_norm_supported(g):
+    if Config.algo == "simt":
+        return False
+    return bool(_lib.load().b200gan_conv2d_dgrad_norm_supported(ctypes.byref(g)))
+
+
+def conv_dgrad_norm(g, dy, packed, x, mean_rstd, scale_shift, act, slope):
+    d = _norm_desc(x.shape, False, 0.0, 0.0, act, slope, False)
+    sums = zero_scratch(x.device, 2 * g.C)
+    dx = empty_cl(g.N, g.C, g.H, g.W, dy.device)
+    _lib.check(_lib.load().b200gan_conv2d_dgrad_norm(ctypes.byref(g), ctypes.byref(d), dy.data_ptr(), packed.data_ptr(),
+                                                     x.data_ptr(), mean_rstd.data_ptr(), scale_shift.data_ptr(),
+                                                     sums.data_ptr(), dx.data_ptr(), _stream()), "conv2d_dgrad_norm")
+    return dx, sums
+
+
+def norm_backward_from_sums(dy, x, mean_rstd, gamma, sums, eps, act=ACT_NONE, slope=0.0, need_params=False,
+                            round_tf32=False, scale_shift=None):
+    d = _norm_desc(x.shape, False, eps, 0.0, act, slope, round_tf32)
+    dx = torch.empty_like(x, memory_format=CL)
+    dgb = torch.empty(sums.numel(), device=x.device, dtype=torch.float32) if need_params else None
+    _lib.check(_lib.load().b200gan_norm_bwd_from_sums(ctypes.byref(d), dy.data_ptr(), x.data_ptr(), mean_rstd.data_ptr(),
+                                                      _ptr(scale_shift), _ptr(gamma), sums.data_ptr(), dx.data_ptr(),
+                                                      _ptr(dgb), _stream()), "norm_bwd_from_sums")
     return dx, dgb
 
 
diff --git a/pytorch-gan_b200/csrc/conv_api.cu b/pytorch-gan_b200/csrc/conv_api.cu
--- a/pytorch-gan_b200/csrc/conv_api.cu
+++ b/pytorch-gan_b200/csrc/conv_api.cu
@@ -32,10 +32,11 @@
 int tc_supported(const b200gan_conv_geom *g, int pass);
 int tc_fprop(const b200gan_conv_geom *g, const b200gan_epilogue *ep, const float *x,
              const float *packed, float *y, cudaStream_t st);
-int tc_dgrad(const b200gan_conv_geom *g, const float *dy, const float *packed, float *dx,
+struct TcNormBwd;
+int tc_dgrad(const b200gan_conv_geom *g, const float *dy, const float *packed, float *dx, const TcNormBwd *nb,
              cudaStream_t st);
 size_t tc_wgrad_workspace_floats(const b200gan_conv_geom *g);
-int tc_wgrad(const b200gan_conv_geom *g, const float *x, const float *dy, float *dw, float *ws,
+int tc_wgrad(const b200gan_conv_geom *g, const float *x, const float *dy, float *dw, float *db, float *ws,
              cudaStream_t st);
 
 static thread_local char g_err[512] = "";
@@ -377,7 +378,7 @@
   switch (dgrad_route(g, algo)) {
     case DgradRoute::Tc:
       if (!tc_supported(g, 1)) B2_UNSUPPORTED("conv2d_dgrad: geometry not supported by the tensor-core path");
-      return tc_dgrad(g, dy, packed, dx, st);
+      return tc_dgrad(g, dy, packed, dx, nullptr, st);
     case DgradRoute::Transposed:
       return simt_gather_gemm(g->N, g->P, g->Q, g->K, g->H, g->W, g->C, g->R, g->S, g->stride, g->pad_t, g->pad_l,
                               B200GAN_PAD_ZERO, 1, 0, nullptr, dy, packed, dx, st);
@@ -434,8 +435,8 @@
   return 0;
 }
 
-extern "C" int b200gan_conv2d_wgrad(const b200gan_conv_geom *g, const float *x, const float *dy, float *dw,
-                                    float *db, float *workspace, int algo, void *stream) {
+static int conv2d_wgrad(const b200gan_conv_geom *g, const float *x, const float *dy, float *dw, float *db,
+                        float *workspace, int algo, bool fuse_db, void *stream) {
   if (int e = validate_geom(g)) return e;
   B2_CHECK_ARG(x && dy && dw, "conv2d_wgrad: null pointer");
   cudaStream_t st = as_stream(stream);
@@ -443,7 +444,8 @@
   switch (wgrad_route(g, algo)) {
     case WgradRoute::Tc:
       if (!tc_supported(g, 2)) B2_UNSUPPORTED("conv2d_wgrad: geometry not supported by the tensor-core path");
-      rc = tc_wgrad(g, x, dy, dw, workspace, st);
+      if (fuse_db && !g->transposed) return tc_wgrad(g, x, dy, dw, db, workspace, st);
+      rc = tc_wgrad(g, x, dy, dw, nullptr, workspace, st);
       break;
     case WgradRoute::Fewk:
       rc = fewk_wgrad(g, x, dy, dw, workspace, st);
@@ -464,3 +466,13 @@
   if (db) return simt_colsum(dy, db, (int64_t)g->N * g->P * g->Q, g->K, st);
   return B200GAN_OK;
 }
+
+extern "C" int b200gan_conv2d_wgrad(const b200gan_conv_geom *g, const float *x, const float *dy, float *dw,
+                                    float *db, float *workspace, int algo, void *stream) {
+  return conv2d_wgrad(g, x, dy, dw, db, workspace, algo, false, stream);
+}
+
+extern "C" int b200gan_conv2d_wgrad_fused_bias(const b200gan_conv_geom *g, const float *x, const float *dy, float *dw,
+                                               float *db, float *workspace, int algo, void *stream) {
+  return conv2d_wgrad(g, x, dy, dw, db, workspace, algo, true, stream);
+}
diff --git a/pytorch-gan_b200/csrc/conv_tc.cu b/pytorch-gan_b200/csrc/conv_tc.cu
--- a/pytorch-gan_b200/csrc/conv_tc.cu
+++ b/pytorch-gan_b200/csrc/conv_tc.cu
@@ -81,7 +81,19 @@
   float *y;
   int32_t narrow_k;
   int32_t ksplit;
+  const float *nb_x;
+  const float *nb_mean_rstd;
+  const float *nb_scale_shift;
+  int32_t nb_act;
+  float nb_slope;
   long long *trace;
+};
+
+struct TcNormBwd {
+  const float *x, *mean_rstd, *scale_shift;
+  int32_t act;
+  float slope;
+  double *sums;
 };
 
 #define TC_TRACE(slot)                                                   \
@@ -163,6 +175,40 @@
   if (rtf) {
 #pragma unroll
     for (int j = 0; j < 32; ++j) v[j] = round_tf32(v[j]);
+  }
+}
+
+__device__ __forceinline__ void norm_bwd_terms(float (&v)[32], float (&s2)[32], const float *xrow, const float *mean_rstd,
+                                               const float *scale_shift, int ldk, int act, float slope) {
+  const bool masked = act != B200GAN_ACT_NONE;
+  const float lo = act == B200GAN_ACT_LRELU ? slope : 0.f;
+#pragma unroll
+  for (int g = 0; g < 4; ++g) {
+    float xx[8], mean[8], rstd[8], sc[8], sh[8];
+#pragma unroll
+    for (int h = 0; h < 2; ++h) {
+      const int o = 2 * g + h;
+      const float4 a = xrow ? __ldg(reinterpret_cast<const float4 *>(xrow) + o) : make_float4(0.f, 0.f, 0.f, 0.f);
+      const float4 m = __ldg(reinterpret_cast<const float4 *>(mean_rstd) + o);
+      const float4 r = __ldg(reinterpret_cast<const float4 *>(mean_rstd + ldk) + o);
+      const float4 s = __ldg(reinterpret_cast<const float4 *>(scale_shift) + o);
+      const float4 t = __ldg(reinterpret_cast<const float4 *>(scale_shift + ldk) + o);
+      xx[4 * h] = a.x; xx[4 * h + 1] = a.y; xx[4 * h + 2] = a.z; xx[4 * h + 3] = a.w;
+      mean[4 * h] = m.x; mean[4 * h + 1] = m.y; mean[4 * h + 2] = m.z; mean[4 * h + 3] = m.w;
+      rstd[4 * h] = r.x; rstd[4 * h + 1] = r.y; rstd[4 * h + 2] = r.z; rstd[4 * h + 3] = r.w;
+      sc[4 * h] = s.x; sc[4 * h + 1] = s.y; sc[4 * h + 2] = s.z; sc[4 * h + 3] = s.w;
+      sh[4 * h] = t.x; sh[4 * h + 1] = t.y; sh[4 * h + 2] = t.z; sh[4 * h + 3] = t.w;
+    }
+#pragma unroll
+    for (int e = 0; e < 8; ++e) {
+      const int j = 8 * g + e;
+      float dz = v[j];
+      if (masked && !(fmaf(xx[e], sc[e], sh[e]) > 0.f)) dz *= lo;
+      dz = xrow ? dz : 0.f;
+      v[j] = dz;
+      s2[j] = dz * ((xx[e] - mean[e]) * rstd[e]);
+    }
+    asm volatile("" ::: "memory");
   }
 }
 
@@ -299,10 +345,16 @@
       }
       if (p.stats) {
         float s2[32];
-#pragma unroll
-        for (int j = 0; j < 32; ++j) {
-          v[j] = valid ? v[j] : 0.f;
-          s2[j] = v[j] * v[j];
+        if (BN < 256 && p.nb_x) {
+          const int ch = ntile * BN + c;
+          norm_bwd_terms(v, s2, valid ? p.nb_x + ((int64_t)(on * p.Ho + oh) * p.Wo + ow) * p.ldk + ch : nullptr,
+                         p.nb_mean_rstd + ch, p.nb_scale_shift + ch, p.ldk, p.nb_act, p.nb_slope);
+        } else {
+#pragma unroll
+          for (int j = 0; j < 32; ++j) {
+            v[j] = valid ? v[j] : 0.f;
+            s2[j] = v[j] * v[j];
+          }
         }
         float cs1 = warp_colsum32(v, lane);
         float cs2 = warp_colsum32(s2, lane);
@@ -600,13 +652,37 @@
   return l;
 }
 
+static int tc_tile_shape(int Ho, int Wo, int &bwl, int &bhl) {
+  bwl = ilog2_ceil(Wo);
+  if (bwl > 7) bwl = 7;
+  bhl = ilog2_ceil(Ho);
+  if (bhl > 7 - bwl) bhl = 7 - bwl;
+  return TC_BM / ((1 << bwl) * (1 << bhl));
+}
+
+static int64_t tc_tiles(int N, int Ho, int Wo) {
+  int bwl, bhl;
+  const int BNn = tc_tile_shape(Ho, Wo, bwl, bhl);
+  return (int64_t)ceil_div(Wo, 1 << bwl) * ceil_div(Ho, 1 << bhl) * ceil_div(N, BNn);
+}
+
+static int tc_block_n(int Kout, int64_t tiles) {
+  if (Kout % 256 == 0 && tiles * (Kout / 256) >= num_sms()) return 256;
+  return (Kout % 128 == 0) ? 128 : (Kout % 64 == 0 ? 64 : 32);
+}
+
+static int tc_ksplit(int64_t ctas, int min_iters) {
+  if (ctas >= num_sms() || min_iters < 16) return 1;
+  int ks = (int)((2 * num_sms() + ctas - 1) / ctas);
+  if (ks > min_iters / 8) ks = min_iters / 8;
+  if (ks > 32) ks = 32;
+  return ks >= 2 ? ks : 1;
+}
+
 template <class Params>
 static int tc_setup(Params &p, int N, int Ho, int Wo, int ldk, const b200gan_epilogue *ep, double **deferred) {
-  int bwl = ilog2_ceil(Wo);
-  if (bwl > 7) bwl = 7;
-  int bhl = ilog2_ceil(Ho);
-  if (bhl > 7 - bwl) bhl = 7 - bwl;
-  const int BNn = TC_BM / ((1 << bwl) * (1 << bhl));
+  int bwl, bhl;
+  const int BNn = tc_tile_shape(Ho, Wo, bwl, bhl);
   p.bw_log2 = bwl;
   p.bh_log2 = bhl;
   p.tiles_w = ceil_div(Wo, 1 << bwl);
@@ -682,12 +758,11 @@
 
 static int run_tc(const float *in, int N, int Hi, int Wi, int Cc, bool phase_in, const float *packedB, int Kout,
                   int btaps, int nphase, const int *tap_begin, const TcTap *taps, int Ho, int Wo, bool phase_out,
-                  const int *out_dc, const int *out_da, int ldk, const b200gan_epilogue *ep, float *y,
-                  cudaStream_t st) {
+                  const int *out_dc, const int *out_da, int ldk, const b200gan_epilogue *ep, const TcNormBwd *nb,
+                  float *y, cudaStream_t st) {
   const int narrow_k = Kout < 32 ? Kout : 0;
   const int Kreal = Kout;
   if (narrow_k) Kout = 32;
-  int BN = (Kout % 128 == 0) ? 128 : (Kout % 64 == 0 ? 64 : 32);
   TcParams p;
   memset(&p, 0, sizeof(p));
   const int total_taps = tap_begin[nphase];
@@ -698,10 +773,8 @@
   double *deferred_stats;
   const int BNn = tc_setup(p, N, Ho, Wo, ldk, ep, &deferred_stats);
   const int BW = 1 << p.bw_log2, BH = 1 << p.bh_log2;
-  {
-    const int64_t tiles = (int64_t)p.tiles_w * p.tiles_h * ceil_div(N, BNn) * nphase;
-    if (Kout % 256 == 0 && tiles * (Kout / 256) >= num_sms()) BN = 256;
-  }
+  const int64_t tiles = (int64_t)p.tiles_w * p.tiles_h * ceil_div(N, BNn) * nphase;
+  const int BN = tc_block_n(Kout, tiles);
   for (int i = 0; i < 4; ++i) {
     p.out_dc[i] = i < nphase ? out_dc[i] : 0;
     p.out_da[i] = i < nphase ? out_da[i] : 0;
@@ -719,24 +792,32 @@
   }
   {
     const bool plain = !p.bias && !p.chan_scale && p.act == B200GAN_ACT_NONE && !p.rtf;
-    const int64_t ctas = (int64_t)p.tiles_w * p.tiles_h * ceil_div(N, BNn) * (Kout / BN) * nphase;
     int min_iters = 1 << 30;
     for (int z = 0; z < nphase; ++z) {
       const int it = (tap_begin[z + 1] - tap_begin[z]) * p.kchunks;
       if (it < min_iters) min_iters = it;
     }
-    if (plain && !narrow_k && ctas < num_sms() && min_iters >= 16) {
-      int ks = (int)((2 * num_sms() + ctas - 1) / ctas);
-      if (ks > min_iters / 8) ks = min_iters / 8;
-      if (ks > 32) ks = 32;
-      if (ks >= 2) {
-        p.ksplit = ks;
-        if (p.stats) {
-          deferred_stats = p.stats;
-          p.stats = nullptr;
-        }
-      }
-    }
+    const int ks = plain && !narrow_k ? tc_ksplit(tiles * (Kout / BN), min_iters) : 1;
+    if (ks >= 2) {
+      if (nb) B2_UNSUPPORTED("tensor-core dgrad with norm sums: the contraction of this geometry is split");
+      p.ksplit = ks;
+      if (p.stats) {
+        deferred_stats = p.stats;
+        p.stats = nullptr;
+      }
+    }
+  }
+  if (nb) {
+    B2_CHECK_ARG(!narrow_k && !phase_out && nphase == 1 && !p.stats && !deferred_stats,
+                 "tensor-core dgrad with norm sums: plain output without other statistics only");
+    p.stats = nb->sums;
+    p.stats_per_sample = 0;
+    p.stats_groups = ldk;
+    p.nb_x = nb->x;
+    p.nb_mean_rstd = nb->mean_rstd;
+    p.nb_scale_shift = nb->scale_shift;
+    p.nb_act = nb->act;
+    p.nb_slope = nb->slope;
   }
   B2_CHECK_ARG(((uintptr_t)in % 16 == 0) && ((uintptr_t)packedB % 16 == 0) && ((uintptr_t)y % 16 == 0),
                "tensor-core conv: pointers must be 16-byte aligned");
@@ -868,12 +949,12 @@
     }
   tap_begin[1] = nt;
   return run_tc(in, N, Hi, Wi, Cc, stride == 2, packedB, Kout, R * S, 1, tap_begin, taps, Po, Qo, false, out_dc, out_da,
-                Kout, ep, out, st);
+                Kout, ep, nullptr, out, st);
 }
 
 static int tc_scatter(const float *in, int N, int Pi, int Qi, int Cc, int R, int S, int stride, int pad_t, int pad_l,
-                      const float *packedB, int Kout, int Ho, int Wo, const b200gan_epilogue *ep, float *out,
-                      cudaStream_t st) {
+                      const float *packedB, int Kout, int Ho, int Wo, const b200gan_epilogue *ep, const TcNormBwd *nb,
+                      float *out, cudaStream_t st) {
   TcTap taps[TC_MAX_TAPS];
   memset(taps, 0, sizeof(taps));
   int tap_begin[5] = {0, 0, 0, 0, 0};
@@ -888,7 +969,7 @@
       }
     tap_begin[1] = nt;
     return run_tc(in, N, Pi, Qi, Cc, false, packedB, Kout, R * S, 1, tap_begin, taps, Ho, Wo, false, out_dc, out_da, Kout,
-                  ep, out, st);
+                  ep, nb, out, st);
   }
   int nt = 0;
   for (int ph = 0; ph < 4; ++ph) {
@@ -910,7 +991,7 @@
   }
   tap_begin[4] = nt;
   return run_tc(in, N, Pi, Qi, Cc, false, packedB, Kout, R * S, 4, tap_begin, taps, Ho / 2, Wo / 2, true, out_dc, out_da,
-                Kout, ep, out, st);
+                Kout, ep, nb, out, st);
 }
 
 int tc_fprop(const b200gan_conv_geom *g, const b200gan_epilogue *ep, const float *x, const float *packed, float *y,
@@ -936,15 +1017,25 @@
       out_da[ph] = a;
     }
     return run_tc(x, g->N, g->H, g->W, g->C, false, packed, g->K, 16, 4, tap_begin, taps, g->H, g->W, true, out_dc, out_da,
-                  g->K, e, y, st);
+                  g->K, e, nullptr, y, st);
   }
   if (g->transposed)
-    return tc_scatter(x, g->N, g->H, g->W, g->C, g->R, g->S, g->stride, g->pad_t, g->pad_l, packed, g->K, g->P, g->Q, e, y,
-                      st);
+    return tc_scatter(x, g->N, g->H, g->W, g->C, g->R, g->S, g->stride, g->pad_t, g->pad_l, packed, g->K, g->P, g->Q, e,
+                      nullptr, y, st);
   return tc_gather(x, g->N, g->H, g->W, g->C, g->R, g->S, g->stride, g->pad_t, g->pad_l, packed, g->K, g->P, g->Q, e, y, st);
 }
 
-int tc_dgrad(const b200gan_conv_geom *g, const float *dy, const float *packed, float *dx, cudaStream_t st) {
+int tc_dgrad_norm_supported(const b200gan_conv_geom *g) {
+  if (!tc_supported(g, 1) || g->transposed || g->stride != 1 || g->pad_mode != B200GAN_PAD_ZERO) return 0;
+  const int64_t tiles = tc_tiles(g->N, g->H, g->W);
+  const int taps = g->up == 2 ? 16 : g->R * g->S;
+  const int bn = tc_block_n(g->C, tiles);
+  return bn <= 128 && tc_ksplit(tiles * (g->C / bn), taps * (g->K / TC_BK)) == 1;
+}
+
+int tc_dgrad(const b200gan_conv_geom *g, const float *dy, const float *packed, float *dx, const TcNormBwd *nb,
+             cudaStream_t st) {
+  if (nb && !tc_dgrad_norm_supported(g)) B2_UNSUPPORTED("tensor-core dgrad with norm sums: geometry not supported");
   if (g->up == 2) {
     TcTap taps[TC_MAX_TAPS];
     memset(taps, 0, sizeof(taps));
@@ -960,13 +1051,36 @@
       }
     }
     return run_tc(dy, g->N, g->P, g->Q, g->K, true, packed, g->C, 16, 1, tap_begin, taps, g->H, g->W, false, out_dc, out_da,
-                  g->C, nullptr, dx, st);
+                  g->C, nullptr, nb, dx, st);
   }
   if (g->transposed)
     return tc_gather(dy, g->N, g->P, g->Q, g->K, g->R, g->S, g->stride, g->pad_t, g->pad_l, packed, g->C, g->H, g->W, nullptr,
                      dx, st);
   return tc_scatter(dy, g->N, g->P, g->Q, g->K, g->R, g->S, g->stride, g->pad_t, g->pad_l, packed, g->C, g->H, g->W, nullptr,
-                    dx, st);
-}
-
-}
+                    nb, dx, st);
+}
+
+}
+
+using namespace b200gan;
+
+extern "C" int b200gan_conv2d_dgrad_norm_supported(const b200gan_conv_geom *g) {
+  if (validate_geom(g) != B200GAN_OK) return 0;
+  return tc_dgrad_norm_supported(g);
+}
+
+extern "C" int b200gan_conv2d_dgrad_norm(const b200gan_conv_geom *g, const b200gan_norm_desc *d, const float *dy,
+                                         const float *packed, const float *x, const float *mean_rstd,
+                                         const float *scale_shift, double *sums, float *dx, void *stream) {
+  if (int e = validate_geom(g)) return e;
+  B2_CHECK_ARG(d && dy && packed && x && mean_rstd && sums && dx, "conv2d_dgrad_norm: null pointer");
+  if (d->per_sample) B2_UNSUPPORTED("conv2d_dgrad_norm: batch statistics only (per-sample norms are not supported)");
+  B2_CHECK_ARG(d->C == g->C && d->N == g->N && d->HW == g->H * g->W, "conv2d_dgrad_norm: norm and conv input differ");
+  B2_CHECK_ARG(d->act == B200GAN_ACT_NONE || d->act == B200GAN_ACT_LRELU || d->act == B200GAN_ACT_RELU,
+               "conv2d_dgrad_norm: the norm's activation must be none, LeakyReLU or ReLU");
+  B2_CHECK_ARG(scale_shift != nullptr, "conv2d_dgrad_norm: scale_shift required");
+  B2_CHECK_ARG(((uintptr_t)x | (uintptr_t)mean_rstd | (uintptr_t)scale_shift) % 16 == 0,
+               "conv2d_dgrad_norm: pointers must be 16-byte aligned");
+  const TcNormBwd nb{x, mean_rstd, scale_shift, d->act, d->slope, sums};
+  return tc_dgrad(g, dy, packed, dx, &nb, as_stream(stream));
+}
diff --git a/pytorch-gan_b200/csrc/norm.cu b/pytorch-gan_b200/csrc/norm.cu
--- a/pytorch-gan_b200/csrc/norm.cu
+++ b/pytorch-gan_b200/csrc/norm.cu
@@ -287,6 +287,20 @@
   return B200GAN_OK;
 }
 
+static int norm_bwd_apply_params(const b200gan_norm_desc *d, const float *dy, const float *x, const float *y,
+                                 const float *mean_rstd, const float *scale_shift, const float *gamma, double *sums,
+                                 float *dx, float *dgamma_dbeta, int vec, dim3 grid, int64_t rows, cudaStream_t st) {
+  const int G = d->per_sample ? d->N * d->C : d->C;
+  const float inv = (float)(1.0 / (d->per_sample ? (double)d->HW : (double)d->N * (double)d->HW));
+  auto apply = vec == 4 ? norm_bwd_apply_kernel<4> : norm_bwd_apply_kernel<1>;
+  apply<<<grid, 256, 0, st>>>(dy, x, y, mean_rstd, scale_shift, gamma, sums, dx, rows, d->C, G, inv, d->act, d->slope,
+                              d->round_tf32);
+  B2_LAUNCH_CHECK();
+  norm_bwd_params_kernel<<<ceil_div(G, 128), 128, 0, st>>>(sums, dgamma_dbeta, G);
+  B2_LAUNCH_CHECK();
+  return B200GAN_OK;
+}
+
 }
 
 using namespace b200gan;
@@ -354,12 +368,19 @@
   auto reduce = vec == 4 ? norm_bwd_reduce_kernel<4> : norm_bwd_reduce_kernel<1>;
   reduce<<<grid, 256, 0, st>>>(dy, x, yy, mean_rstd, scale_shift, sums, rows, d->C, G, d->act, d->slope);
   B2_LAUNCH_CHECK();
-  const float inv = (float)(1.0 / (d->per_sample ? (double)d->HW : (double)d->N * (double)d->HW));
-  auto apply = vec == 4 ? norm_bwd_apply_kernel<4> : norm_bwd_apply_kernel<1>;
-  apply<<<grid, 256, 0, st>>>(dy, x, yy, mean_rstd, scale_shift, gamma, sums, dx, rows, d->C, G, inv, d->act, d->slope,
-                              d->round_tf32);
-  B2_LAUNCH_CHECK();
-  norm_bwd_params_kernel<<<ceil_div(G, 128), 128, 0, st>>>(sums, dgamma_dbeta, G);
-  B2_LAUNCH_CHECK();
-  return B200GAN_OK;
-}
+  return norm_bwd_apply_params(d, dy, x, yy, mean_rstd, scale_shift, gamma, sums, dx, dgamma_dbeta, vec, grid, rows, st);
+}
+
+extern "C" int b200gan_norm_bwd_from_sums(const b200gan_norm_desc *d, const float *dy, const float *x,
+                                          const float *mean_rstd, const float *scale_shift, const float *gamma,
+                                          double *sums, float *dx, float *dgamma_dbeta, void *stream) {
+  if (int e = check_desc(d)) return e;
+  B2_CHECK_ARG(dy && x && mean_rstd && sums && dx, "norm_bwd_from_sums: null pointer");
+  B2_CHECK_ARG(d->act == B200GAN_ACT_NONE || ((d->act == B200GAN_ACT_LRELU || d->act == B200GAN_ACT_RELU) && scale_shift),
+               "norm_bwd_from_sums: activation must be none, or LeakyReLU / ReLU with scale_shift");
+  const int vec = vec_width(d->C, {dy, x, dx});
+  int64_t rows;
+  const dim3 grid = slice_grid(d, vec, rows);
+  return norm_bwd_apply_params(d, dy, x, x, mean_rstd, scale_shift, gamma, sums, dx, dgamma_dbeta, vec, grid, rows,
+                               as_stream(stream));
+}
diff --git a/pytorch-gan_b200/csrc/wgrad_tc.cu b/pytorch-gan_b200/csrc/wgrad_tc.cu
--- a/pytorch-gan_b200/csrc/wgrad_tc.cu
+++ b/pytorch-gan_b200/csrc/wgrad_tc.cu
@@ -12,6 +12,8 @@
   int16_t s_dc, d_dc;
   int8_t s_da, d_da;
   int8_t s_dw, s_dh;
+  int8_t db;
+  int8_t pad_;
 };
 
 struct WgParams {
@@ -26,6 +28,7 @@
   int32_t ldn;
   int32_t mtotal;
   float *partial;
+  float *db;
 };
 
 template <int NB, int STAGES>
@@ -127,6 +130,13 @@
         (uint32_t)(abase + 128 + ((((ac >> 2)) ^ (ap + 1)) << 4)),
         (uint32_t)(abase + 128 + ((((ac >> 2) + 2) ^ (ap + 1)) << 4))};
     float acc[NB / 2];
+    const bool db_job = p.db != nullptr && p.jobs[job].db;
+    const bool dbA = db_job && !p.s_is_a && nt == 0;
+    const bool dbB = db_job && p.s_is_a && mt == 0;
+    float dsa0 = 0.f, dsa1 = 0.f;
+    float dsb[NB <= 64 ? NB / 8 : 1];
+#pragma unroll
+    for (int i = 0; i < (NB <= 64 ? NB / 8 : 1); ++i) dsb[i] = 0.f;
     int stage = 0;
     uint32_t phase = 0;
     auto prepare = [&](int it, uint32_t(&fa)[16]) {
@@ -138,11 +148,24 @@
       for (int k = 0; k < WG_PIX / 8; ++k)
 #pragma unroll
         for (int j = 0; j < 4; ++j) fa[4 * k + j] = *reinterpret_cast<const uint32_t *>(src + aoff[j] + k * 1024);
+      if (dbA) {
+#pragma unroll
+        for (int k = 0; k < WG_PIX / 8; ++k) {
+          dsa0 += __uint_as_float(fa[4 * k]) + __uint_as_float(fa[4 * k + 2]);
+          dsa1 += __uint_as_float(fa[4 * k + 1]) + __uint_as_float(fa[4 * k + 3]);
+        }
+      }
 #pragma unroll
       for (int c = 0; c < NB / 32; ++c) {
         const float4 v = *reinterpret_cast<const float4 *>(src + L::A_BYTES + c * WG_CHUNK_BYTES + tp * 128 +
                                                            ((tq ^ (tp & 7)) << 4));
         const float e[4] = {v.x, v.y, v.z, v.w};
+        if constexpr (NB <= 64) {
+          if (dbB) {
+#pragma unroll
+            for (int i = 0; i < 4; ++i) dsb[4 * c + i] += e[i];
+          }
+        }
 #pragma unroll
         for (int i = 0; i < 4; ++i) {
           const int r = c * 32 + tq * 4 + i;
@@ -180,6 +203,28 @@
     }
     wgmma_wait<0>();
     wgmma_fence_regs<NB / 2>(acc);
+    if (dbA) {
+      dsa0 += __shfl_xor_sync(0xffffffffu, dsa0, 1);
+      dsa1 += __shfl_xor_sync(0xffffffffu, dsa1, 1);
+      dsa0 += __shfl_xor_sync(0xffffffffu, dsa0, 2);
+      dsa1 += __shfl_xor_sync(0xffffffffu, dsa1, 2);
+      if ((lane & 3) == 0) {
+        const int ch = (mt * 4 + 2 * half + (wq >> 1)) * 32 + ac;
+        atomicAdd(p.db + ch, dsa0);
+        atomicAdd(p.db + ch + 8, dsa1);
+      }
+    }
+    if constexpr (NB <= 64) {
+      if (dbB) {
+#pragma unroll
+        for (int i = 0; i < NB / 8; ++i) {
+          float s = dsb[i];
+#pragma unroll
+          for (int o = 16; o > 0; o >>= 1) s += __shfl_xor_sync(0xffffffffu, s, o);
+          if (lane == 0) atomicAdd(p.db + nt * NB + (i >> 2) * 32 + tq * 4 + (i & 3), s);
+        }
+      }
+    }
     wg_consumers_sync();
     store_acc_sw128<NB>(smem, acc, half * 64);
     fence_proxy_async();
@@ -368,10 +413,12 @@
   return B200GAN_OK;
 }
 
-int tc_wgrad(const b200gan_conv_geom *g, const float *x, const float *dy, float *dw, float *ws, cudaStream_t st) {
+int tc_wgrad(const b200gan_conv_geom *g, const float *x, const float *dy, float *dw, float *db, float *ws,
+             cudaStream_t st) {
   WgPlan pl;
   if (!wg_plan(g, pl)) B2_UNSUPPORTED("tensor-core wgrad: geometry not supported");
   B2_CHECK_ARG(ws != nullptr, "tensor-core wgrad: workspace required");
+  B2_CHECK_ARG(!(db && g->transposed), "tensor-core wgrad: bias gradient of a ConvTranspose2d is not fused");
   B2_CHECK_ARG(((uintptr_t)x % 16 == 0) && ((uintptr_t)dy % 16 == 0) && ((uintptr_t)ws % 16 == 0),
                "tensor-core wgrad: pointers must be 16-byte aligned");
   const bool up2 = g->up == 2;
@@ -385,8 +432,10 @@
         int a = ph >> 1, b = ph & 1, dr = tp >> 1, ds = tp & 1;
         WgJob &j = p.jobs[ph * 4 + tp];
         j.d_dc = (int16_t)(b * g->K); j.d_da = (int8_t)a; j.s_dh = (int8_t)(a - 1 + dr); j.s_dw = (int8_t)(b - 1 + ds);
+        j.db = tp == 0;
       }
   } else {
+    p.jobs[0].db = 1;
     for (int r = 0; r < g->R; ++r)
       for (int s2 = 0; s2 < g->S; ++s2) {
         WgJob &j = p.jobs[r * g->S + s2];
@@ -404,6 +453,7 @@
   p.tiles_total = pl.tiles_total; p.tiles_per_split = pl.tps;
   p.s_is_a = pl.s_is_a; p.mtiles = pl.mtiles; p.ntiles = pl.ntiles; p.ldn = pl.ldn; p.mtotal = pl.mtotal;
   p.partial = ws;
+  p.db = db;
 
   const float *sptr = g->transposed ? dy : x, *dptr = g->transposed ? x : dy;
   const uint64_t Hs = g->transposed ? g->P : g->H, Ws = g->transposed ? g->Q : g->W, Cs = pl.sch;
@@ -440,6 +490,7 @@
     if (int e = make_tmap_f32(&tmP, ws, 2, dims, strides, pbox)) return e;
   }
   B2_CUDA(cudaMemsetAsync(ws, 0, (size_t)pl.njobs * pl.mtotal * pl.ldn * sizeof(float), st));
+  if (db) B2_CUDA(cudaMemsetAsync(db, 0, (size_t)g->K * sizeof(float), st));
   dim3 grid((unsigned)pl.nsplits, (unsigned)pl.njobs, (unsigned)(pl.mtiles * pl.ntiles));
   int rc = pl.NB == 256 ? launch_wg<256, 3>(tmX, tmY, tmP, p, grid, st)
            : pl.NB == 128 ? launch_wg<128, 6>(tmX, tmY, tmP, p, grid, st)
```

Result: faster. 48880 (median of 6 runs) (+4.1%).
